# NoakLiu/FastFourierDiffusion

Measured on AMD Instinct MI355X. Metric: samples/sec at 1000 diffusion steps, ECG freq-domain, higher is better.
Workload: dtype f32; 1 GPU; ECG frequency-domain L=187 C=1, transformer d72/H12/NL10/F2048, VP beta[0.1,20], 1000-step sampler (BASELINE configs[1]); batch_per_gpu=512, global_batch=512, diffusion_steps=1000, cache=False, noise=philox on device

## Files before the change

### fastfourierdiffusion_amd/_native.py

```python
from __future__ import annotations

import ctypes as C
import os
from typing import Optional

_HERE = os.path.dirname(os.path.abspath(__file__))
LIB_PATH = os.path.join(_HERE, "libffd.so")

FFD_MODEL_TRANSFORMER, FFD_MODEL_LSTM, FFD_MODEL_MLP = 0, 1, 2
FFD_SDE_VP, FFD_SDE_VE = 0, 1
K_FFN, K_ATTN, K_OUTPROJ, K_LSTM_REC, K_LSTM_GATES, K_SDE, K_EMBED, K_UNEMBED = range(8)


class FFDError(RuntimeError):
    pass


class ModelDesc(C.Structure):
    _fields_ = [
        ("kind", C.c_int32), ("n_channels", C.c_int32), ("max_len", C.c_int32), ("d_model", C.c_int32),
        ("n_head", C.c_int32), ("num_layers", C.c_int32), ("dim_feedforward", C.c_int32), ("sde", C.c_int32),
        ("sde_a", C.c_double), ("sde_b", C.c_double), ("fourier_noise_scaling", C.c_int32), ("eps", C.c_double),
    ]


class SdeDesc(C.Structure):
    _fields_ = [("sde", C.c_int32), ("reserved", C.c_int32), ("a", C.c_double), ("b", C.c_double)]


class FrescaCfg(C.Structure):
    _fields_ = [("low_scale", C.c_float), ("high_scale", C.c_float), ("cutoff_ratio", C.c_double),
                ("strategy", C.c_int32), ("num_steps", C.c_int32)]


class CrfCaptureCfg(C.Structure):
    _fields_ = [("ring", C.c_void_p), ("n_slots", C.c_int32), ("every", C.c_int32), ("last", C.c_void_p),
                ("last_every", C.c_int32), ("reserved", C.c_int32)]


class CacheCfg(C.Structure):
    _fields_ = [("K", C.c_int32), ("R", C.c_int32)]


class CacheStats(C.Structure):
    _fields_ = [("recompute_count", C.c_int64), ("cache_hit_count", C.c_int64), ("current_step", C.c_int64),
                ("table_allocated", C.c_int32), ("reserved", C.c_int32)]


_P = C.c_void_p
_F = C.POINTER(C.c_float)

SIGNATURES = {
    "ffd_freq_decompose": (C.c_int, [_P, _P, _P, C.c_int, C.c_int, C.c_int, C.c_double, _P]),
    "ffd_hermite_predict": (C.c_int, [_P, C.POINTER(C.c_double), C.c_double, C.c_int, _P, C.c_int, C.c_size_t, _P]),
    "ffd_spectral_density": (C.c_int, [_P, _P, C.c_int, C.c_int, C.c_int, _P]),
    "ffd_w2_work_bytes": (C.c_size_t, [C.c_int, C.c_int, C.c_int, C.c_int, C.c_size_t]),
    "ffd_w2_sliced": (C.c_int, [_P, C.c_int, _P, C.c_int, C.c_int, _P, C.c_int, C.c_int, _P, _P, C.c_size_t, _P]),
    "ffd_w2_marginal": (C.c_int, [_P, C.c_int, _P, C.c_int, C.c_int, C.c_int, _P, _P, C.c_size_t, _P]),
    "ffd_w2_prepare": (C.c_int, [_P, C.c_int, C.c_int, _P, C.c_int, _P, _P, C.c_size_t, _P]),
    "ffd_w2_against_prepared": (C.c_int, [_P, C.c_int, _P, C.c_int, C.c_int, _P, C.c_int, C.c_int, _P, _P,
                                          C.c_size_t, _P]),
    "ffd_w2_summary": (C.c_int, [_P, C.c_int, _P, _P]),
    "ffd_col_mean_work_bytes": (C.c_size_t, [C.c_int, C.c_int]),
    "ffd_col_mean": (C.c_int, [_P, C.c_int, C.c_int, _P, _P, C.c_size_t, _P]),
    "ffd_w2_bench_kernels": (C.c_int, [_P, C.c_int, C.c_int, _P, C.c_int, _P, _P, _P, C.c_int, _P, C.c_int, _F, _P]),
    "ffd_sm_draw_times": (C.c_int, [_P, C.c_int, C.c_double, C.c_double, C.c_uint64, C.c_uint64, _P]),
    "ffd_sm_perturb": (C.c_int, [_P, _P, _P, _P, _P, _P, C.c_uint64, C.c_uint64, C.c_int, C.c_int, C.c_int, _P]),
    "ffd_sm_loss": (C.c_int, [_P, _P, _P, _P, C.c_uint64, C.c_uint64, C.c_int, C.c_int, _P, C.c_int, C.c_int, C.c_int, _P]),
    "ffd_sm_eval_batch": (C.c_int, [_P, _P, _P, _P, _P, _P, C.c_uint64, C.c_uint64, C.c_int, C.c_int, _P, C.c_int, _P]),
    "ffd_cache_crf_capture": (C.c_int, [_P, C.POINTER(CrfCaptureCfg)]),
    "ffd_create": (C.c_int, [C.POINTER(_P), C.POINTER(ModelDesc), C.c_int]),
    "ffd_destroy": (None, [_P]),
    "ffd_last_error": (C.c_char_p, [_P]),
    "ffd_version": (C.c_char_p, []),
    "ffd_load_weight": (C.c_int, [_P, C.c_char_p, _P, C.c_size_t]),
    "ffd_finalize_weights": (C.c_int, [_P]),
    "ffd_host_noise_scaling": (C.c_int, [C.c_int, C.c_int, _F]),
    "ffd_host_timesteps": (C.c_int, [C.c_int, C.c_double, _F, _F]),
    "ffd_host_gate": (C.c_int, [C.c_int, C.c_int, C.c_int, C.c_int]),
    "ffd_score_forward": (C.c_int, [_P, _P, C.c_float, _P, C.c_int, _P]),
    "ffd_score_forward_cached": (C.c_int, [_P, _P, C.c_float, _P, _P, C.c_int, C.c_int, _P]),
    "ffd_sde_step": (C.c_int, [C.POINTER(SdeDesc), _P, _P, _P, C.c_double, C.c_float, _P, C.c_uint64, C.c_uint64,
                               C.c_int, C.c_int, C.c_int, C.c_int, _P]),
    "ffd_prior": (C.c_int, [C.POINTER(SdeDesc), _P, _P, _P, C.c_uint64, C.c_uint64, C.c_int, C.c_int, C.c_int, _P]),
    "ffd_dft": (C.c_int, [_P, _P, C.c_int, C.c_int, C.c_int, _P]),
    "ffd_idft": (C.c_int, [_P, _P, C.c_int, C.c_int, C.c_int, _P]),
    "ffd_unstandardize_idft": (C.c_int, [_P, _P, _P, _P, C.c_int, C.c_int, C.c_int, _P]),
    "ffd_dft_standardize": (C.c_int, [_P, _P, _P, _P, C.c_int, C.c_int, C.c_int, _P]),
    "ffd_positional_encoding": (C.c_int, [_P, _P, _P, C.c_int, C.c_int, C.c_int, C.c_float, _P]),
    "ffd_time_encoding": (C.c_int, [_P, _P, _P, _P, _P, _P, _P, C.c_int, C.c_int, C.c_int, _P]),
    "ffd_fresca": (C.c_int, [_P, _P, _P, C.c_int, C.c_int, C.c_int, C.c_float, C.c_float, C.c_double, C.c_int, _P]),
    "ffd_lstm_trace": (C.c_int, [_P, C.POINTER(C.c_uint64), C.c_int, C.POINTER(C.c_int)]),
    "ffd_fresca2d": (C.c_int, [_P, _P, _P, C.c_int, C.c_int, C.c_int, C.c_int, C.c_float, C.c_float, C.c_double, C.c_int, _P]),
    "ffd_fresca_enable": (C.c_int, [_P, C.POINTER(FrescaCfg)]),
    "ffd_fresca_disable": (C.c_int, [_P]),
    "ffd_cache_enable": (C.c_int, [_P, C.POINTER(CacheCfg)]),
    "ffd_cache_disable": (C.c_int, [_P]),
    "ffd_cache_reset": (C.c_int, [_P]),
    "ffd_cache_stats_get": (C.c_int, [_P, C.POINTER(CacheStats)]),
    "ffd_cache_tables_read": (C.c_int, [_P, _P, _P, _P]),
    "ffd_sample_batch": (C.c_int, [_P, _P, C.c_int, _F, C.c_int, C.c_float, C.c_int, C.c_int, C.c_uint64,
                                   C.c_uint64, _P, C.c_int, C.c_int, _P]),
    "ffd_flops_per_sample_step": (C.c_double, [_P, C.c_int]),
    "ffd_ffn_flops_per_launch": (C.c_double, [_P, C.c_int]),
    "ffd_kernel_timing_begin": (C.c_int, [_P, C.c_uint32, C.c_int]),
    "ffd_kernel_timing_end": (C.c_int, [_P]),
    "ffd_kernel_timing_get": (C.c_int, [_P, C.c_int, _F, C.POINTER(C.c_int)]),
    "ffd_kernel_work": (C.c_char_p, [_P, C.c_int, C.c_int, C.c_int, C.POINTER(C.c_double), C.POINTER(C.c_double)]),
    "ffd_score_forward_ts": (C.c_int, [_P, _P, _P, _P, _P, C.c_int, C.c_int, _P]),
    "ffd_cache_configure": (C.c_int, [_P, C.POINTER(CacheCfg)]),
    "ffd_tune": (C.c_int, [C.c_char_p, C.c_int]),
    "ffd_tune_get": (C.c_int, [C.c_char_p, C.POINTER(C.c_int)]),
    "ffd_bench_ffn": (C.c_int, [_P, C.c_int, C.c_int, _F, _P]),
    "ffd_probe_ffn_clock": (C.c_int, [_P, C.c_int, C.c_double, C.POINTER(C.c_double), C.POINTER(C.c_double),
                                      C.POINTER(C.c_uint64), C.c_int, C.POINTER(C.c_int), _P]),
    "ffd_async_status": (C.c_int, [_P]),
    "ffd_probe_attn": (C.c_int, [_P, C.c_int, C.c_int, C.c_double, C.c_int, _F, C.POINTER(C.c_uint64), C.c_int,
                                 C.POINTER(C.c_int), _P]),
}

_lib: Optional[C.CDLL] = None


def lib() -> C.CDLL:
    global _lib
    if _lib is not None:
        return _lib
    if not os.path.exists(LIB_PATH):
        raise FFDError(
            f"{LIB_PATH} not found: build it with `python -c 'import __graft_entry__ as g; g.build()'` "
            "(or `make -C fastfourierdiffusion_amd/csrc`). There is no CPU / PyTorch fallback.")
    try:
        import torch
    except Exception:
        pass
    try:
        handle = C.CDLL(LIB_PATH, mode=C.RTLD_GLOBAL)
    except OSError as e:
        raise FFDError(f"failed to load {LIB_PATH}: {e}") from e
    for name, (res, args) in SIGNATURES.items():
        try:
            fn = getattr(handle, name)
        except AttributeError as e:
            raise FFDError(f"{LIB_PATH} does not export {name}") from e
        fn.restype = res
        fn.argtypes = args
    _lib = handle
    return handle


def check(rc: int, ctx=None, what: str = "") -> None:
    if rc == 0:
        return
    msg = ""
    if ctx:
        raw = lib().ffd_last_error(ctx)
        msg = raw.decode() if raw else ""
    exc = {-1: AssertionError, -2: NotImplementedError}.get(rc, FFDError)
    raise exc(f"libffd {what} failed (status {rc}): {msg}")


def current_stream_ptr(device) -> int:
    import torch

    return int(torch.cuda.current_stream(device).cuda_stream)


def require_gpu_tensor(t, name: str = "tensor"):
    import torch

    if not isinstance(t, torch.Tensor):
        raise TypeError(f"{name} must be a torch.Tensor")
    if t.device.type != "cuda":
        raise FFDError(
            f"{name} lives on {t.device}: fastfourierdiffusion_amd computes only on an MI355X (gfx950) device; "
            "move the model/tensors to cuda (there is no CPU fallback).")
    if t.dtype != torch.float32:
        raise AssertionError(f"{name} must be float32, got {t.dtype}")
    return t if t.is_contiguous() else t.contiguous()
```

### fastfourierdiffusion_amd/csrc/ffd_api.hip

```cpp
#include <math.h>
#include <stdarg.h>
#include <stdio.h>
#include <string.h>

#include <algorithm>
#include <string>
#include <vector>

#include "../../include/ffd.h"
#include "ffd_internal.h"

using namespace ffd;

namespace {

template <typename T>
struct Grow {
  T* p = nullptr;
  size_t cap = 0;
};

struct WeightSlot {
  std::string key;
  size_t n;
// ... 44 lines not shown
  std::vector<LstmLayer> lstm;
  std::vector<MlpLayer> mlp;
  float* G_dev = nullptr;
  std::vector<float> G_host;
  Grow<float> h0, h1, attn, score;
  Grow<float> qkv;
  Grow<float> temb_b;
  Grow<float> temb_tab, ts_dev;
  float* temb1 = nullptr;
  Grow<float> ffn_part;
  Grow<int> lstm_prog;
  Grow<float> lstm_state;
  std::vector<float> ts_host;
  long weight_epoch = 0, temb_epoch = -1;
  uint32_t time_mask = 0;
  std::vector<hipEvent_t> ev;
  std::vector<int> ev_cls;
  size_t ev_used = 0;
  float tm_ms[FFD_K_COUNT] = {0};
  int tm_n[FFD_K_COUNT] = {0};
  int* async_err = nullptr;
  unsigned long long* lstm_trace = nullptr;
  int lstm_trace_units = 0;
  bool fresca_on = false;
  bool crf_cap_on = false;
  ffd_crf_capture_cfg crf_cap{};
  ffd_fresca_cfg fcfg{};
  Grow<float> score2, fwork;
  Grow<float> sm_noisy;
  bool cache_enabled = false;
  ffd_cache_cfg ccfg{5, 10};
  float *kt = nullptr, *vt = nullptr;
  bool table_allocated = false;
  ffd_cache_stats stats{};

  int fail(int code, const char* fmt, ...) {
    char buf[512];
    va_list ap;
    va_start(ap, fmt);
    vsnprintf(buf, sizeof buf, fmt, ap);
    va_end(ap);
    err = buf;
    return code;
  }
  int d() const { return desc.d_model; }
  int hd() const { return desc.d_model / desc.n_head; }
  bool packs_made() const { return !layers.empty() && layers[0].in_wp != nullptr; }
  size_t table_floats() const { return (size_t)desc.num_layers * desc.n_head * desc.max_len * hd(); }
};

#define HIPCHECK(expr)                                                                          \
  do {                                                                                          \
    hipError_t e__ = (expr);                                                                    \
    if (e__ != hipSuccess)                                                                      \
      return ctx->fail(FFD_ERR_HIP, "%s failed: %s (%s:%d)", #expr, hipGetErrorString(e__), __FILE__, __LINE__); \
  } while (0)

namespace ffd {
#define FFD_KNOB_DEF(key, var, def, ...) thread_local int var = def;
FFD_KNOBS(FFD_KNOB_DEF, FFD_KNOB_DEF)
#undef FFD_KNOB_DEF
}

template <typename T>
static int dev_alloc(ffd_ctx* ctx, T** p, size_t n) {
  static_assert(sizeof(T) == sizeof(float), "the sizes in the messages are in floats");
  *p = nullptr;
  if (g_fail_alloc_after > 0 && --g_fail_alloc_after == 0)
    return ctx->fail(FFD_ERR_NOMEM, "hipMalloc(%zu floats) failed: injected by ffd_tune(\"fail_alloc_after\")", n);
  hipError_t e = hipMalloc((void**)p, n * sizeof(T) + 256);
  if (e != hipSuccess) return ctx->fail(FFD_ERR_NOMEM, "hipMalloc(%zu floats) failed: %s", n, hipGetErrorString(e));
  ctx->owned.push_back(*p);
  return FFD_OK;
}

template <typename T>
static int ensure(ffd_ctx* ctx, Grow<T>& b, size_t n) {
  if (n <= b.cap) return FFD_OK;
  T* old = b.p;
  b.cap = 0;
  b.p = nullptr;
  if (old) {
    (void)hipDeviceSynchronize();
    auto it = std::find(ctx->owned.begin(), ctx->owned.end(), (void*)old);
    if (it != ctx->owned.end()) ctx->owned.erase(it);
    (void)hipFree(old);
  }
  int rc = dev_alloc(ctx, &b.p, n);
  if (rc == FFD_OK) b.cap = n;
  return rc;
}

struct Timed {
  ffd_ctx* ctx;
  hipStream_t s;
  bool on;
  Timed(ffd_ctx* c, int cls, hipStream_t st) : ctx(c), s(st) {
    on = ((c->time_mask >> cls) & 1u) && c->ev_used + 2 <= c->ev.size();
    if (on) {
      (void)hipEventRecord(c->ev[c->ev_used], s);
      c->ev_cls.push_back(cls);
    }
  }
  ~Timed() {
    if (on) {
      (void)hipEventRecord(ctx->ev[ctx->ev_used + 1], s);
      ctx->ev_used += 2;
    }
  }
};
#define TIMED(cls, expr)      \
  do {                        \
    Timed tm__(ctx, cls, s);  \
    HIPCHECK(expr);           \
  } while (0)

static bool d_supported(int d) {
#define X(v) if (d == v) return true;
  FFD_D_LIST(X)
#undef X
  return false;
}
static bool hd_supported(int hd) {
#define X(v) if (hd == v) return true;
  FFD_HD_LIST(X)
#undef X
  return false;
}

namespace ffd {

CacheMode cache_mode(int n_rec, int L) {
  if (n_rec < 0) return CACHE_STD;
  if (n_rec == L) return CACHE_FULL;
  if ((double)n_rec > 0.8 * (double)L) return CACHE_STD;
  return n_rec == 0 ? CACHE_PURE : CACHE_MIXED;
}

LayerPlan plan_layer(const ffd_model_desc& m, int B, CacheMode mode, const PackSet& pk) {
  const int L = m.max_len, d = m.d_model, H = m.n_head, hd = d / H, F = m.dim_feedforward, M = B * L;
  LayerPlan p{};
  p.attn = g_attn_fused && pk.aw_full ? ATTN_FUSED : ATTN_TWO_KERNEL;
  p.hpw = 1;
  p.q_only = mode == CACHE_PURE;
  const int QT = cdiv(L, 32);
  if (p.attn == ATTN_FUSED) {
    p.kspl = qkv_attention_small_split(B, H, L);
    if (pk.aw_full2 && !p.kspl) p.hpw = qkv_attention_hpw(d, hd, L);
    if (g_attn_kvq && pk.aw_kvq && mode != CACHE_PURE && p.kspl) p.q_only = 2;
    p.qg = p.kspl                                               ? 1
           : p.hpw == 2                                         ? cdiv(QT, 2)
           : !p.q_only && (g_attn_qg == 1 || g_attn_qg == 2)    ? g_attn_qg
                                                                : attn_qg(QT, hd, true);
  } else {
    p.qg = QT == 1 ? 1 : g_attn_qg ? g_attn_qg : attn_qg(QT, hd, false);
  }
  const int hp = g_ffn_height && !g_ffn_split && !g_ffn_mb_override ? ffn_height_plan(M, d, F) : 0;
  int unf = 0;
  auto rows_nw = [&] { return g_ffn_rows_nw ? g_ffn_rows_nw : rows_waves(M); };
  if (g_ffn_split) {
    p.ffn = FFN_SPLIT;
  } else if (hp && g_ffn_height == 1) {
    p.ffn = FFN_LN_OPROJ, p.mb = hp;
  } else if (!(hp && g_small_wgs == 0) && (p.ns = small_path_splits(M, d, F))) {
    p.ffn = FFN_SMALL, p.part_floats = small_path_partial_floats(M, d, p.ns);
  } else if (pk.ring && !(hp && g_rows_slices == 0) && rows_slice_plan(M, d, F, &p.nw, &p.nslice, &unf)) {
    p.ffn = unf ? FFN_ROWS_SLICED : FFN_ROWS_SLICED_OPROJ, p.cps = 2, p.part_floats = rows_slice_floats(M, d, p.nslice);
  } else if ((p.nm = hp && g_mid_path == 1 ? 0 : mid_path_splits(M, d, F))) {
    p.ffn = FFN_MID, p.part_floats = small_path_partial_floats(cdiv(M, 64) * 64, d, p.nm);
  } else if (pk.ring && ffn_rows_fused_selected(M, d, F)) {
    p.ffn = FFN_ROWS_OPROJ, p.nw = rows_nw(), p.cps = 2;
  } else if (pk.ring && ffn_rows_selected(M, d, F)) {
    p.ffn = FFN_ROWS, p.nw = rows_nw(), p.cps = g_ffn_rows_cps == 1 && d == 72 ? 1 : 2;
  } else {
    p.ffn = FFN_LN;
    p.mb = g_ffn_mb_override >= 1 ? g_ffn_mb_override : cdiv(M, 64) >= 512 ? 4 : cdiv(M, 32) >= 512 ? 2 : 1;
    if (hp) p.mb = hp;
    p.persist = g_ffn_persist;
  }
  if (p.ffn == FFN_LN || p.ffn == FFN_LN_OPROJ) p.rem = g_ffn_rem && ffn_rem_rows(d, p.mb);
  p.oproj_separate = p.ffn >= FFN_ROWS_SLICED;
  p.swap = p.ffn == FFN_ROWS_SLICED_OPROJ || p.ffn == FFN_ROWS_OPROJ;
  return p;
}

LstmPlan plan_lstm(const ffd_model_desc& m, int B) {
  const int maxb = lstm_wave_max_batch(m.max_len, m.d_model);
  if (g_lstm_wave && m.d_model % 4 == 0 && m.d_model >= 16 && m.num_layers <= 64 && maxb >= 16)
    return {true, B < maxb ? B : maxb};
  return {false, B};
}

}

extern "C" {

int ffd_tune(const char* key, int value) {
  if (!key) return FFD_ERR_INVALID;
  if (!strcmp(key, "reset")) {
#define FFD_KNOB_RESET(k, var, def, ...) var = def;
    FFD_KNOBS(FFD_KNOB_RESET, FFD_KNOB_RESET)
#undef FFD_KNOB_RESET
    return FFD_OK;
  }
  const int v = value;
#define FFD_KNOB_SET(k, var, def, ok) \
  if (!strcmp(key, k)) {              \
    if (!(ok)) return FFD_ERR_INVALID; \
    var = v;                          \
    return FFD_OK;                    \
  }
#define FFD_KNOB_SET_BOOL(k, var, def) \
  if (!strcmp(key, k)) {               \
    var = v ? 1 : 0;                   \
    return FFD_OK;                     \
  }
  FFD_KNOBS(FFD_KNOB_SET, FFD_KNOB_SET_BOOL)
#undef FFD_KNOB_SET
#undef FFD_KNOB_SET_BOOL
  return FFD_ERR_INVALID;
}

int ffd_tune_get(const char* key, int* value) {
  if (!key || !value) return FFD_ERR_INVALID;
#define FFD_KNOB_GET(k, var, ...) \
  if (!strcmp(key, k)) {          \
    *value = var;                 \
    return FFD_OK;                \
  }
  FFD_KNOBS(FFD_KNOB_GET, FFD_KNOB_GET)
#undef FFD_KNOB_GET
  return FFD_ERR_INVALID;
}

const char* ffd_version(void) { return "libffd 0.1 (gfx950, fp32 MFMA 16x16x4, wave64)"; }

const char* ffd_last_error(const ffd_ctx* ctx) { return ctx ? ctx->err.c_str() : "null context"; }

int ffd_host_noise_scaling(int max_len, int fourier_noise_scaling, float* G) {
  if (max_len < 1 || !G) return FFD_ERR_INVALID;
  for (int i = 0; i < max_len; ++i) G[i] = 1.0f;
  if (fourier_noise_scaling) {
    const float c = (float)(1.0 / sqrt(2.0));
    const float s2 = (float)sqrt(2.0);
    for (int i = 0; i < max_len; ++i) G[i] = c * G[i];
    G[0] = G[0] * s2;
    if (max_len % 2 == 0) G[max_len / 2] = G[max_len / 2] * s2;
  }
  return FFD_OK;
}

int ffd_host_timesteps(int n, double eps, float* ts, float* step_size) {
  if (n < 2 || !ts) return FFD_ERR_INVALID;
  const float start = 1.0f, end = (float)eps;
  const float step = (end - start) / (float)(n - 1);
  const int half = n / 2;
  for (int i = 0; i < n; ++i) {
    volatile float prod = (i < half) ? step * (float)i : step * (float)(n - i - 1);
    ts[i] = (i < half) ? start + prod : end - prod;
  }
  if (step_size) *step_size = ts[0] - ts[1];
  return FFD_OK;
}

int ffd_host_gate(int step, int max_len, int K, int R) {
  if (step == 0) return max_len;
  const int interval = (R < 100) ? 500 : R;
  const int k_tokens = K < max_len ? K : max_len;
  if (step % interval == 0) {
    int n = 2 * k_tokens;
    if (n > max_len) n = max_len;
    return n < 0 ? 0 : n;
  }
  return 0;
}

static void bind_weights(ffd_ctx* ctx) {
  const ffd_model_desc& m = ctx->desc;
  const int NL = std::max(m.num_layers, 0);
  const size_t d = m.d_model, C = m.n_channels, L = m.max_len, F = m.dim_feedforward;
  auto bind = [&](const std::string& key, size_t n, const float** field) { ctx->weights.push_back({key, n, field}); };
  ModelWeights& w = ctx->model;
  if (m.kind == FFD_MODEL_TRANSFORMER) bind("pos_encoder.embedding.weight", L * d, &w.pos);
  bind("time_encoder.W", (d + 1) / 2, &w.time_W);
  bind("time_encoder.dense.weight", d * d, &w.time_dense_w);
  bind("time_encoder.dense.bias", d, &w.time_dense_b);
  const size_t io = m.kind == FFD_MODEL_MLP ? L * C : C;
  bind("embedder.weight", d * io, &w.embed_w);
  bind("embedder.bias", d, &w.embed_b);
  bind("unembedder.weight", io * d, &w.unembed_w);
  bind("unembedder.bias", io, &w.unembed_b);
  if (m.kind == FFD_MODEL_TRANSFORMER) ctx->layers.resize(NL);
  else if (m.kind == FFD_MODEL_MLP) ctx->mlp.resize(NL);
  else ctx->lstm.resize(NL);
  for (int i = 0; i < NL; ++i) {
    const std::string s = (m.kind == FFD_MODEL_TRANSFORMER ? "backbone.layers." : "backbone.") + std::to_string(i) + ".";
    if (m.kind == FFD_MODEL_TRANSFORMER) {
      LayerWeights& l = ctx->layers[i];
      bind(s + "self_attn.in_proj_weight", 3 * d * d, &l.in_w);
      bind(s + "self_attn.in_proj_bias", 3 * d, &l.in_b);
      bind(s + "self_attn.out_proj.weight", d * d, &l.out_w);
      bind(s + "self_attn.out_proj.bias", d, &l.out_b);
      bind(s + "linear1.weight", F * d, &l.w1);
      bind(s + "linear1.bias", F, &l.b1);
      bind(s + "linear2.weight", d * F, &l.w2);
      bind(s + "linear2.bias", d, &l.b2);
      bind(s + "norm1.weight", d, &l.n1w);
      bind(s + "norm1.bias", d, &l.n1b);
      bind(s + "norm2.weight", d, &l.n2w);
      bind(s + "norm2.bias", d, &l.n2b);
    } else if (m.kind == FFD_MODEL_MLP) {
      MlpLayer& l = ctx->mlp[i];
      bind(s + "0.weight", F * d, &l.w0);
      bind(s + "0.bias", F, &l.b0);
      bind(s + "3.weight", d * F, &l.w3);
      bind(s + "3.bias", d, &l.b3);
    } else {
      LstmLayer& l = ctx->lstm[i];
      bind(s + "weight_ih_l0", 4 * d * d, &l.wih);
      bind(s + "weight_hh_l0", 4 * d * d, &l.whh);
      bind(s + "bias_ih_l0", 4 * d, &l.bih);
      bind(s + "bias_hh_l0", 4 * d, &l.bhh);
    }
  }
}

int ffd_create(ffd_ctx** out, const ffd_model_desc* desc, int device) {
  if (!out || !desc) return FFD_ERR_INVALID;
  *out = nullptr;
  ffd_ctx* ctx = new ffd_ctx();
  ctx->desc = *desc;
  ctx->device = device;
  *out = ctx;
  const ffd_model_desc& m = ctx->desc;
  bind_weights(ctx);
  if (m.n_channels < 1 || m.max_len < 1 || m.num_layers < 1)
    return ctx->fail(FFD_ERR_INVALID, "bad shape: C=%d L=%d NL=%d", m.n_channels, m.max_len, m.num_layers);
  if (m.kind == FFD_MODEL_MLP) {
    if (m.d_model < 1 || m.dim_feedforward < 1)
      return ctx->fail(FFD_ERR_INVALID, "mlp: d_model=%d d_mlp=%d", m.d_model, m.dim_feedforward);
  } else if (!d_supported(m.d_model)) {
    return ctx->fail(FFD_ERR_UNSUPPORTED, "d_model=%d: this build has kernels for d_model in {8, 16, 24, 32, 48, 60, 64, 72}", m.d_model);
  }
  if (m.kind == FFD_MODEL_TRANSFORMER) {
    if (m.n_head < 1 || m.d_model % m.n_head != 0)
      return ctx->fail(FFD_ERR_INVALID, "d_model=%d not divisible by n_head=%d", m.d_model, m.n_head);
    if (!hd_supported(m.d_model / m.n_head))
      return ctx->fail(FFD_ERR_UNSUPPORTED, "head_dim=%d: supported head dims are 2, 3, 4, 5, 6, 8", m.d_model / m.n_head);
    if (m.dim_feedforward < 64 || m.dim_feedforward % 64 != 0)
      return ctx->fail(FFD_ERR_UNSUPPORTED, "dim_feedforward=%d must be a positive multiple of 64", m.dim_feedforward);
    if (m.max_len > 512) return ctx->fail(FFD_ERR_UNSUPPORTED, "max_len=%d > 512 (attention kernel limit)", m.max_len);
  } else if (m.kind != FFD_MODEL_LSTM && m.kind != FFD_MODEL_MLP) {
    return ctx->fail(FFD_ERR_UNSUPPORTED, "model kind %d", m.kind);
  }
  if (m.sde != FFD_SDE_VP && m.sde != FFD_SDE_VE) return ctx->fail(FFD_ERR_UNSUPPORTED, "sde kind %d", m.sde);
  int ndev = 0;
  hipError_t e = hipGetDeviceCount(&ndev);
  if (e != hipSuccess || ndev <= 0)
    return ctx->fail(FFD_ERR_HIP, "no HIP device available (%s): libffd has no CPU path",
                     e == hipSuccess ? "device count 0" : hipGetErrorString(e));
  if (device < 0 || device >= ndev) return ctx->fail(FFD_ERR_INVALID, "device %d out of range [0,%d)", device, ndev);
  HIPCHECK(hipSetDevice(device));
  hipDeviceProp_t prop;
  HIPCHECK(hipGetDeviceProperties(&prop, device));
  if (strncmp(prop.gcnArchName, "gfx950", 6) != 0)
    return ctx->fail(FFD_ERR_UNSUPPORTED, "device %d is %s; libffd is built for gfx950 only", device, prop.gcnArchName);
  ctx->G_host.resize(m.max_len);
  ffd_host_noise_scaling(m.max_len, m.fourier_noise_scaling, ctx->G_host.data());
  int rc = dev_alloc(ctx, &ctx->G_dev, m.max_len);
  if (rc) return rc;
  HIPCHECK(hipMemcpy(ctx->G_dev, ctx->G_host.data(), sizeof(float) * m.max_len, hipMemcpyHostToDevice));
  rc = dev_alloc(ctx, &ctx->temb1, m.d_model);
  if (rc) return rc;
  HIPCHECK(hipHostMalloc((void**)&ctx->async_err, 64, hipHostMallocMapped));
  memset(ctx->async_err, 0, 64);
  return FFD_OK;
}

void ffd_destroy(ffd_ctx* ctx) {
  if (!ctx) return;
  (void)hipSetDevice(ctx->device);
  for (WeightSlot& w : ctx->weights) (void)hipFree(w.dev);
  for (void* p : ctx->owned) (void)hipFree(p);
  for (hipEvent_t e : ctx->ev) (void)hipEventDestroy(e);
  if (ctx->async_err) (void)hipHostFree(ctx->async_err);
  delete ctx;
}

int ffd_load_weight(ffd_ctx* ctx, const char* name, const float* data, size_t n) {
  if (!ctx) return FFD_ERR_INVALID;
  if (!name || !data) return ctx->fail(FFD_ERR_INVALID, "ffd_load_weight: null argument");
  auto w = std::find_if(ctx->weights.begin(), ctx->weights.end(), [&](const WeightSlot& v) { return v.key == name; });
  if (w == ctx->weights.end()) return ctx->fail(FFD_ERR_INVALID, "unexpected parameter '%s' for this model", name);
  if (w->n != n) return ctx->fail(FFD_ERR_INVALID, "parameter '%s': got %zu floats, expected %zu", name, n, w->n);
  HIPCHECK(hipSetDevice(ctx->device));
  if (!w->dev) {
    hipError_t e = hipMalloc((void**)&w->dev, n * sizeof(float) + 256);
    if (e != hipSuccess) return ctx->fail(FFD_ERR_NOMEM, "hipMalloc for '%s' failed: %s", name, hipGetErrorString(e));
    *w->field = w->dev;
  }
  HIPCHECK(hipMemcpy(w->dev, data, n * sizeof(float), hipMemcpyDefault));
  ctx->finalized = false;
  return FFD_OK;
}

int ffd_finalize_weights(ffd_ctx* ctx) {
  if (!ctx) return FFD_ERR_INVALID;
  const ffd_model_desc& m = ctx->desc;
  for (const WeightSlot& w : ctx->weights)
    if (!w.dev) return ctx->fail(FFD_ERR_STATE, "missing parameter '%s'", w.key.c_str());
  HIPCHECK(hipSetDevice(ctx->device));
  const int d = m.d_model, F = m.dim_feedforward;
  hipStream_t s = nullptr;
  if (m.kind == FFD_MODEL_TRANSFORMER) {
    HIPCHECK(launch_renorm_rows(const_cast<float*>(ctx->model.pos), m.max_len, d, sqrtf((float)d), s));
    for (LayerWeights& l : ctx->layers) {
      if (!l.in_wp) {
        int rc;
        if ((rc = dev_alloc(ctx, &l.in_wp, dpack_floats(3 * d, d)))) return rc;
        if ((rc = dev_alloc(ctx, &l.q_wp, dpack_floats(d, d)))) return rc;
        if ((rc = dev_alloc(ctx, &l.kv_wp, dpack_floats(2 * d, d)))) return rc;
        if (qkv_attention_supported(d, d / m.n_head)) {
          if ((rc = dev_alloc(ctx, &l.aw_full, attn_pack_floats(d, m.n_head, 1, 0)))) return rc;
          if ((rc = dev_alloc(ctx, &l.aw_q, attn_pack_floats(d, m.n_head, 1, 1)))) return rc;
          if (attn_kvq_supported(d / m.n_head))
            if ((rc = dev_alloc(ctx, &l.aw_kvq, attn_pack_floats(d, m.n_head, 1, 2)))) return rc;
          if (m.n_head % 2 == 0) {
            if ((rc = dev_alloc(ctx, &l.aw_full2, attn_pack_floats(d, m.n_head, 2, 0)))) return rc;
            if ((rc = dev_alloc(ctx, &l.aw_q2, attn_pack_floats(d, m.n_head, 2, 1)))) return rc;
          }
        }
        if ((rc = dev_alloc(ctx, &l.out_wp, dpack_floats(d, d)))) return rc;
        if ((rc = dev_alloc(ctx, &l.w1p, dpack_floats(F, d)))) return rc;
        if ((rc = dev_alloc(ctx, &l.w2p, w2pack_floats(d, F)))) return rc;
        if ((rc = dev_alloc(ctx, &l.w2r, w2rem_floats(d, F)))) return rc;
        if (ffn_rows_supported(d, F)) {
          if ((rc = dev_alloc(ctx, &l.ring, ffn_ring_floats(d, F)))) return rc;
          if ((rc = dev_alloc(ctx, &l.ring_op, ffn_ring_oproj_floats(d)))) return rc;
        }
      }
      HIPCHECK(launch_pack_dweight(l.in_w, l.in_wp, 3 * d, d, s));
      HIPCHECK(launch_pack_dweight(l.in_w, l.q_wp, d, d, s));
      HIPCHECK(launch_pack_dweight(l.in_w + (size_t)d * d, l.kv_wp, 2 * d, d, s));
      if (l.aw_full) {
        HIPCHECK(launch_pack_attn(l.in_w, l.in_b, l.aw_full, d, m.n_head, 1, 0, s));
        HIPCHECK(launch_pack_attn(l.in_w, l.in_b, l.aw_q, d, m.n_head, 1, 1, s));
        if (l.aw_kvq) HIPCHECK(launch_pack_attn(l.in_w, l.in_b, l.aw_kvq, d, m.n_head, 1, 2, s));
        if (l.aw_full2) {
          HIPCHECK(launch_pack_attn(l.in_w, l.in_b, l.aw_full2, d, m.n_head, 2, 0, s));
          HIPCHECK(launch_pack_attn(l.in_w, l.in_b, l.aw_q2, d, m.n_head, 2, 1, s));
        }
      }
      HIPCHECK(launch_pack_dweight(l.out_w, l.out_wp, d, d, s));
      HIPCHECK(launch_pack_dweight(l.w1, l.w1p, F, d, s));
      HIPCHECK(launch_pack_w2(l.w2, l.w2p, d, F, s));
      HIPCHECK(launch_pack_w2rem(l.w2, l.w2r, d, F, s));
      if (l.ring) {
        HIPCHECK(launch_pack_ffn_ring(l.w1, l.b1, l.w2, l.ring, d, F, s));
        HIPCHECK(launch_pack_oproj_ring(l.out_w, l.ring_op, d, s));
      }
      if (l.w1s) HIPCHECK(launch_pack_ffn_split(l.w1, l.w2, l.w1s, l.w2s, d, F, s));
    }
  } else if (m.kind == FFD_MODEL_LSTM) {
    for (LstmLayer& l : ctx->lstm) {
      if (!l.wih_p) {
        int rc;
        if ((rc = dev_alloc(ctx, &l.wih_p, dpack_floats(4 * d, d)))) return rc;
        if ((rc = dev_alloc(ctx, &l.bsum, 4 * d))) return rc;
        if (d % 4 == 0 && d >= 16) {
          if ((rc = dev_alloc(ctx, &l.ih_wpk, lstm_wave_wpack_floats(d)))) return rc;
          if ((rc = dev_alloc(ctx, &l.hh_wpk, lstm_wave_wpack_floats(d)))) return rc;
          if ((rc = dev_alloc(ctx, &l.b_wpk, lstm_wave_bpack_floats(d)))) return rc;
        }
      }
      HIPCHECK(launch_pack_dweight(l.wih, l.wih_p, 4 * d, d, s));
      hipLaunchKernelGGL(k_add_vec, dim3(cdiv(4 * d, 256)), dim3(256), 0, s, l.bih, l.bhh, l.bsum, 4 * d);
      HIPCHECK(hipGetLastError());
      if (l.ih_wpk) HIPCHECK(launch_pack_lstm_wave(l.wih, l.whh, l.bsum, l.ih_wpk, l.hh_wpk, l.b_wpk, d, s));
    }
  }
  HIPCHECK(hipStreamSynchronize(s));
  ctx->weight_epoch++;
  ctx->finalized = true;
  return FFD_OK;
}

static int ensure_workspace(ffd_ctx* ctx, int B) {
  const ffd_model_desc& m = ctx->desc;
  const size_t M = (size_t)B * m.max_len, d = m.d_model;
  int rc;
  if ((rc = ensure(ctx, ctx->h0, M * d))) return rc;
  if ((rc = ensure(ctx, ctx->score, M * m.n_channels))) return rc;
  if ((rc = ensure(ctx, ctx->temb_b, (size_t)B * d))) return rc;
  if (m.kind == FFD_MODEL_MLP) {
    if ((rc = ensure(ctx, ctx->h1, (size_t)B * d))) return rc;
    if ((rc = ensure(ctx, ctx->qkv, (size_t)B * m.dim_feedforward))) return rc;
  } else if (m.kind == FFD_MODEL_TRANSFORMER) {
    if ((rc = ensure(ctx, ctx->h1, M * d))) return rc;
    if ((rc = ensure(ctx, ctx->attn, M * d))) return rc;
  }
  return FFD_OK;
}

static LayerPlan plan_of(const ffd_ctx* ctx, int B, CacheMode mode) {
  const LayerWeights& w = ctx->layers[0];
  return plan_layer(ctx->desc, B, mode,
                    PackSet{w.aw_full != nullptr, w.aw_full2 != nullptr, w.aw_kvq != nullptr, w.ring_op != nullptr});
}

struct CacheUse {
  int n_own;
  bool tables, store;
};
static CacheUse cache_use(CacheMode mode, int n_rec, int L) {
  return {mode == CACHE_PURE ? 0 : mode == CACHE_MIXED ? n_rec : L, mode == CACHE_PURE || mode == CACHE_MIXED,
          mode == CACHE_MIXED};
}

static hipError_t run_attention(const ffd_ctx* ctx, const LayerPlan& p, const LayerWeights& w, const float* x,
                                const float* kt, const float* vt, float* kt_out, float* vt_out, int B, int n_own,
                                hipStream_t s, unsigned long long* stamp = nullptr) {
  const ffd_model_desc& m = ctx->desc;
  const int L = m.max_len, d = m.d_model, H = m.n_head, hd = d / H;
  float* out = ctx->attn.p;
  if (p.attn == ATTN_FUSED) {
    const float* pack = p.q_only == 2 ? w.aw_kvq
                        : p.hpw == 2  ? (p.q_only ? w.aw_q2 : w.aw_full2)
                                      : (p.q_only ? w.aw_q : w.aw_full);
    return launch_qkv_attention(AttnArgs{x, pack, kt, vt, kt_out, vt_out, out, B, L, n_own, stamp}, d, hd, p.hpw, p.q_only,
                                p.kspl, p.qg, s);
  }
  if (stamp != nullptr) return hipErrorInvalidValue;
  const size_t M = (size_t)B * L;
  float *q = ctx->qkv.p, *k = q + M * d, *v = q + 2 * M * d;
  hipError_t e = launch_linear_hm(x, p.q_only ? w.q_wp : w.in_wp, w.in_b, q, k, v, (int)M, p.q_only ? 1 : 3, d, L, H, hd, s);
  if (e == hipSuccess) e = launch_attention(q, k, v, kt, vt, out, B, L, H, hd, n_own, p.qg, s);
  if (e == hipSuccess && kt_out)
    e = launch_kv_store(k, v, kt_out, vt_out, L, H, hd, n_own, s);
  return e;
}

static hipError_t run_ffn(const ffd_ctx* ctx, const LayerPlan& p, const LayerWeights& w, const float* attn, float* cur,
                          float* alt, int M, hipStream_t s, unsigned long long* stamp = nullptr) {
  const int d = ctx->desc.d_model, F = ctx->desc.dim_feedforward;
  float* P = ctx->ffn_part.p;
  const bool sliced = p.ffn == FFN_ROWS_SLICED_OPROJ || p.ffn == FFN_ROWS_SLICED;
  const bool fused = p.ffn == FFN_ROWS_SLICED_OPROJ || p.ffn == FFN_ROWS_OPROJ;
  float* const y = fused ? alt : cur;
  const RowsArgs rows{fused ? attn : alt, fused ? cur : nullptr, &w, sliced ? P : y, M, d, F, p.nw, p.cps, fused,
                      sliced ? p.nslice : 0, stamp};
  switch (p.ffn) {
    case FFN_LN_OPROJ:
      return stamp ? hipErrorInvalidValue : launch_oproj_ffn_ln(attn, cur, w, cur, M, d, F, p.mb, p.rem, s);
    case FFN_SMALL:
      return stamp ? hipErrorInvalidValue : launch_oproj_ffn_small(attn, cur, w, alt, P, cur, M, d, F, p.ns, s);
    case FFN_ROWS_SLICED_OPROJ:
    case FFN_ROWS_SLICED: {
      if (stamp || p.nslice < 2) return hipErrorInvalidValue;
      const hipError_t e = launch_ffn_rows(rows, s);
      return e != hipSuccess ? e : launch_rows_reduce_ln(P, w, y, M, d, p.nslice, s);
    }
    case FFN_ROWS_OPROJ:
    case FFN_ROWS: return launch_ffn_rows(rows, s);
    case FFN_MID:
      return stamp ? hipErrorInvalidValue : launch_ffn_mid(alt, w, P, cur, M, d, F, p.nm, s);
    case FFN_SPLIT: return launch_ffn_ln_split(alt, w, cur, M, d, F, s, stamp);
    case FFN_LN: return launch_ffn_ln(alt, w, cur, M, d, F, p.mb, p.rem, p.persist, s, stamp);
  }
  return hipErrorInvalidValue;
}

static const struct {
  const char* name;
  bool oproj;
} kFfnForms[] = {
    {"k_ffn_ln<oproj>", true},
    {"k_oproj_ffn_split + k_ffn_reduce_ln", true},
    {"k_ffn_rows<oproj, sliced> + k_rows_reduce_ln", true},
    {"k_ffn_rows<oproj>", true},
    {"k_ffn_rows<sliced> + k_rows_reduce_ln", false},
    {"k_ffn_part", false},
    {"k_ffn_ln_split", false},
    {"k_ffn_rows", false},
    {"k_ffn_ln", false},
};

static int forward_impl(ffd_ctx* ctx, const float* x, const float* temb, int temb_stride, float* score_out,
                        float* crf_out, int B, int n_rec, hipStream_t s, const float** hidden_out = nullptr) {
  const ffd_model_desc& m = ctx->desc;
  const int L = m.max_len, C = m.n_channels, d = m.d_model, M = B * L;
  const ModelWeights& mw = ctx->model;
  if (m.kind == FFD_MODEL_MLP) {
    const int io = L * C, F = m.dim_feedforward;
    HIPCHECK(launch_dense(x, mw.embed_w, mw.embed_b, temb_stride ? nullptr : temb, temb_stride ? temb : nullptr,
                          ctx->h0.p, B, d, io, 0, s));
    float* cur = ctx->h0.p;
    float* alt = ctx->h1.p;
    for (const MlpLayer& l : ctx->mlp) {
      HIPCHECK(launch_dense(cur, l.w0, l.b0, nullptr, nullptr, ctx->qkv.p, B, F, d, 1, s));
      HIPCHECK(launch_dense(ctx->qkv.p, l.w3, l.b3, nullptr, cur, alt, B, d, F, 0, s));
      std::swap(cur, alt);
    }
    HIPCHECK(launch_dense(cur, mw.unembed_w, mw.unembed_b, nullptr, nullptr, score_out, B, io, d, 0, s));
    return FFD_OK;
  }
  float* const h0 = ctx->h0.p;
  if (m.kind == FFD_MODEL_LSTM) {
    TIMED(FFD_K_EMBED, launch_embed(x, mw.embed_w, mw.embed_b, nullptr, temb, temb_stride, h0, B, L, C, d, s));
    if (const LstmPlan lp = plan_lstm(m, B); lp.wave) {
      const int Bw = lp.Bw;
      if (int rc = ensure(ctx, ctx->lstm_prog, (size_t)16 + 16 * cdiv(Bw, 16))) return rc;
      const float *wih[64], *whh[64], *bs[64];
      for (int i = 0; i < m.num_layers; ++i) wih[i] = ctx->lstm[i].ih_wpk, whh[i] = ctx->lstm[i].hh_wpk, bs[i] = ctx->lstm[i].b_wpk;
      if (int rc = ensure(ctx, ctx->lstm_state, lstm_wave_state_floats(Bw, d, m.num_layers))) return rc;
      for (int b0 = 0; b0 < B; b0 += Bw) {
        const int nb = B - b0 < Bw ? B - b0 : Bw;
        TIMED(FFD_K_LSTM_REC, launch_lstm_wave(h0 + (size_t)b0 * L * d, wih, whh, bs, m.num_layers, nb, L, d,
                                               ctx->lstm_prog.p, ctx->lstm_state.p, ctx->async_err, s,
                                               b0 == 0 ? ctx->lstm_trace : nullptr));
      }
    } else
    for (const LstmLayer& l : ctx->lstm) {
      if (int rc = ensure(ctx, ctx->qkv, (size_t)M * 4 * d)) return rc;
      TIMED(FFD_K_LSTM_GATES, launch_linear(h0, l.wih_p, l.bsum, ctx->qkv.p, M, 4 * d, d, 4 * d, s));
      TIMED(FFD_K_LSTM_REC, launch_lstm_layer(h0, ctx->qkv.p, l.whh, B, L, d, s));
    }
    if (hidden_out) {
      *hidden_out = h0;
      return FFD_OK;
    }
    TIMED(FFD_K_UNEMBED, launch_unembed(h0, mw.unembed_w, mw.unembed_b, score_out, M, C, d, s));
    return FFD_OK;
  }
  const int H = m.n_head, hd = d / H, F = m.dim_feedforward;
  TIMED(FFD_K_EMBED, launch_embed(x, mw.embed_w, mw.embed_b, mw.pos, temb, temb_stride, h0, B, L, C, d, s));
  const CacheMode mode = cache_mode(n_rec, L);
  const CacheUse cu = cache_use(mode, n_rec, L);
  const size_t lt = (size_t)H * L * hd;
  if (g_ffn_split && !ffn_split_supported(d, F))
    return ctx->fail(FFD_ERR_UNSUPPORTED, "ffn_split needs d_model %% 4 == 0, d_model <= 96, dim_feedforward %% 128 == 0");
  const LayerPlan plan = plan_of(ctx, B, mode);
  if (plan.attn == ATTN_TWO_KERNEL)
    if (int rc = ensure(ctx, ctx->qkv, (size_t)M * 3 * d)) return rc;
  if (int rc = ensure(ctx, ctx->ffn_part, plan.part_floats)) return rc;
  float* const attn = ctx->attn.p;
  float* cur = h0;
  float* alt = ctx->h1.p;
  for (int i = 0; i < m.num_layers; ++i) {
    LayerWeights& w = ctx->layers[i];
    float* kt = ctx->kt ? ctx->kt + i * lt : nullptr;
    float* vt = ctx->vt ? ctx->vt + i * lt : nullptr;
    TIMED(FFD_K_ATTN, run_attention(ctx, plan, w, cur, cu.tables ? kt : nullptr, cu.tables ? vt : nullptr,
                                    cu.store ? kt : nullptr, cu.store ? vt : nullptr, B, cu.n_own, s));
    if (plan.ffn == FFN_SPLIT && w.w1s == nullptr) {
      if (int rc = dev_alloc(ctx, &w.w1s, w1split_bytes(d, F) / sizeof(float))) return rc;
      if (int rc = dev_alloc(ctx, &w.w2s, w2split_bytes(d, F) / sizeof(float))) return rc;
      HIPCHECK(launch_pack_ffn_split(w.w1, w.w2, w.w1s, w.w2s, d, F, s));
    }
    if (plan.oproj_separate)
      TIMED(FFD_K_OUTPROJ, launch_linear_res_ln(attn, w.out_wp, w.out_b, cur, w.n1w, w.n1b, alt, M, d, s));
    TIMED(FFD_K_FFN, run_ffn(ctx, plan, w, attn, cur, alt, M, s));
    if (plan.swap) std::swap(cur, alt);
    if (mode == CACHE_FULL) {
      HIPCHECK(launch_linear_hm(cur, w.kv_wp, w.in_b + d, kt, vt, nullptr, L, 2, d, L, H, hd, s));
    }
    if (n_rec >= 0 && crf_out)
      HIPCHECK(hipMemcpyAsync(crf_out + (size_t)i * L * d, cur, sizeof(float) * L * d, hipMemcpyDeviceToDevice, s));
  }
  if (n_rec >= 0) {
    if (mode == CACHE_FULL) ctx->stats.recompute_count += (int64_t)L * m.num_layers, ctx->table_allocated = true;
    else if (mode == CACHE_PURE) ctx->stats.cache_hit_count += (int64_t)L * m.num_layers;
    else if (mode == CACHE_MIXED) {
      ctx->stats.cache_hit_count += (int64_t)(L - n_rec) * m.num_layers;
      ctx->stats.recompute_count += (int64_t)n_rec * m.num_layers;
      ctx->table_allocated = true;
    }
  }
  if (hidden_out) {
    *hidden_out = cur;
    return FFD_OK;
  }
  TIMED(FFD_K_UNEMBED, launch_unembed(cur, mw.unembed_w, mw.unembed_b, score_out, M, C, d, s));
  return FFD_OK;
// ... 236 lines not shown
    }
    float* crf_dst = nullptr;
    float* crf_copy = nullptr;
    if (use_cache && ctx->crf_cap_on) {
      const ffd_crf_capture_cfg& cc = ctx->crf_cap;
      const int gstep = global_step0 + j;
      const size_t crf_n = (size_t)m.num_layers * m.max_len * d;
      if (cc.ring && gstep % cc.every == 0) crf_dst = cc.ring + (size_t)((gstep / cc.every) % cc.n_slots) * crf_n;
      if (cc.last && gstep % cc.last_every == 0) {
        const int rest = n_run - 1 - j;
        const int to_next = cc.last_every - (gstep % cc.last_every);
        if (to_next > rest) {
          if (crf_dst) crf_copy = cc.last; else crf_dst = cc.last;
        }
      }
    }
    const float* hidden = nullptr;
    if ((rc = forward_impl(ctx, x, ctx->temb_tab.p + (size_t)i * d, 0, ctx->score.p, crf_dst, B, n_rec, s,
                           fuse_tail ? &hidden : nullptr)))
      return rc;
    if (crf_copy)
      HIPCHECK(hipMemcpyAsync(crf_copy, crf_dst, sizeof(float) * (size_t)m.num_layers * m.max_len * d,
                              hipMemcpyDeviceToDevice, s));
    if (use_cache) ctx->stats.current_step = i;
    const double t = (double)timesteps[i];
    const float* score = ctx->score.p;
    if (ctx->fresca_on) {
      const ffd_fresca_cfg& f = ctx->fcfg;
      double h = (double)f.high_scale;
      if (f.num_steps > 0 && h > 1.0) h = (1.0 - t / (double)f.num_steps) * (h - 1.0) + 1.0;
      if (!((double)f.low_scale == 1.0 && h == 1.0)) {
        HIPCHECK(launch_fresca(ctx->score.p, ctx->score2.p, ctx->fwork.p, B, m.max_len, m.n_channels, f.low_scale, (float)h,
                               f.cutoff_ratio, f.strategy, s));
        score = ctx->score2.p;
      }
    }
    if (hidden)
      TIMED(FFD_K_SDE, launch_unembed_sde(hidden, ctx->model.unembed_w, ctx->model.unembed_b, x,
                                          z_inject ? z_inject + (size_t)j * slab : nullptr, ctx->G_dev,
                                          sde_params(m.sde, m.sde_a, m.sde_b, t, step_size), seed, elem_off, (uint32_t)i,
                                          B, m.max_len, m.n_channels, d, s));
    else
      TIMED(FFD_K_SDE, launch_sde_step(x, score, z_inject ? z_inject + (size_t)j * slab : nullptr, ctx->G_dev,
                                       sde_params(m.sde, m.sde_a, m.sde_b, t, step_size), seed, elem_off, (uint32_t)i, B,
                                       m.max_len, m.n_channels, s));
  }
  return FFD_OK;
}

double ffd_flops_per_sample_step(const ffd_ctx* ctx, int cache_hit) {
  if (!ctx) return 0.0;
  const ffd_model_desc& m = ctx->desc;
  const double L = m.max_len, d = m.d_model, C = m.n_channels, NL = m.num_layers, F = m.dim_feedforward;
  if (m.kind == FFD_MODEL_LSTM) return NL * 2.0 * L * (2.0 * 4.0 * d * d) + 4.0 * L * C * d + 2.0 * d * d;
  if (m.kind == FFD_MODEL_MLP) return NL * 4.0 * d * F + 4.0 * L * C * d + 2.0 * d * d;
  double per_layer = 2.0 * L * d * 3.0 * d + 2.0 * L * L * d + 2.0 * L * L * d + 2.0 * L * d * d + 4.0 * L * d * F;
  if (cache_hit) per_layer -= 2.0 * L * d * 2.0 * d;
  return NL * per_layer + 4.0 * L * C * d + 2.0 * d * d;
}

double ffd_ffn_flops_per_launch(const ffd_ctx* ctx, int B) {
  if (!ctx) return 0.0;
  const ffd_model_desc& m = ctx->desc;
  return 4.0 * (double)B * m.max_len * m.d_model * m.dim_feedforward;
}

int ffd_lstm_trace(ffd_ctx* ctx, unsigned long long* host_out, int capacity_units, int* n_units_out) {
  if (!ctx || capacity_units < 1) return FFD_ERR_INVALID;
  HIPCHECK(hipSetDevice(ctx->device));
  if (host_out == nullptr) {
    if (ctx->lstm_trace) (void)hipFree(ctx->lstm_trace);
    ctx->lstm_trace = nullptr;
    HIPCHECK(hipMalloc(&ctx->lstm_trace, sizeof(unsigned long long) * 4 * (size_t)capacity_units));
    HIPCHECK(hipMemset(ctx->lstm_trace, 0, sizeof(unsigned long long) * 4 * (size_t)capacity_units));
    ctx->lstm_trace_units = capacity_units;
    return FFD_OK;
  }
  if (!ctx->lstm_trace) return ctx->fail(FFD_ERR_STATE, "ffd_lstm_trace: no trace begun");
  HIPCHECK(hipDeviceSynchronize());
  const int n = capacity_units < ctx->lstm_trace_units ? capacity_units : ctx->lstm_trace_units;
  HIPCHECK(hipMemcpy(host_out, ctx->lstm_trace, sizeof(unsigned long long) * 4 * (size_t)n, hipMemcpyDeviceToHost));
  (void)hipFree(ctx->lstm_trace);
  ctx->lstm_trace = nullptr;
  if (n_units_out) *n_units_out = n;
  return FFD_OK;
}

int ffd_kernel_timing_begin(ffd_ctx* ctx, uint32_t class_mask, int max_launches) {
  if (!ctx) return FFD_ERR_INVALID;
  if (max_launches < 1 || max_launches > 100000) return ctx->fail(FFD_ERR_INVALID, "max_launches=%d", max_launches);
  HIPCHECK(hipSetDevice(ctx->device));
  while (ctx->ev.size() < (size_t)2 * max_launches) {
    hipEvent_t e;
    HIPCHECK(hipEventCreate(&e));
    ctx->ev.push_back(e);
  }
  ctx->ev_used = 0;
  ctx->ev_cls.clear();
  ctx->time_mask = class_mask;
  return FFD_OK;
}

int ffd_kernel_timing_end(ffd_ctx* ctx) {
  if (!ctx) return FFD_ERR_INVALID;
  ctx->time_mask = 0;
  HIPCHECK(hipSetDevice(ctx->device));
  double tot[FFD_K_COUNT] = {0};
  for (int c = 0; c < FFD_K_COUNT; ++c) ctx->tm_n[c] = 0;
  const size_t n = ctx->ev_used / 2;
  for (size_t i = 0; i < n; ++i) {
    HIPCHECK(hipEventSynchronize(ctx->ev[2 * i + 1]));
    float ms = 0.f;
    HIPCHECK(hipEventElapsedTime(&ms, ctx->ev[2 * i], ctx->ev[2 * i + 1]));
    const int c = ctx->ev_cls[i];
    tot[c] += ms;
    ctx->tm_n[c]++;
  }
  for (int c = 0; c < FFD_K_COUNT; ++c) ctx->tm_ms[c] = ctx->tm_n[c] ? (float)(tot[c] / ctx->tm_n[c]) : 0.f;
  ctx->ev_used = 0;
  ctx->ev_cls.clear();
  return FFD_OK;
}

int ffd_kernel_timing_get(const ffd_ctx* ctx, int kernel_class, float* avg_ms_out, int* launches_out) {
  if (!ctx || kernel_class < 0 || kernel_class >= FFD_K_COUNT || !avg_ms_out || !launches_out) return FFD_ERR_INVALID;
  *avg_ms_out = ctx->tm_ms[kernel_class];
  *launches_out = ctx->tm_n[kernel_class];
  return FFD_OK;
}

const char* ffd_kernel_work(const ffd_ctx* ctx, int kernel_class, int B, int cache_hit, double* flops_out,
                            double* bytes_out) {
  if (!ctx || B < 1) return nullptr;
  const ffd_model_desc& m = ctx->desc;
  const double L = m.max_len, d = m.d_model, C = m.n_channels, F = m.dim_feedforward, M = (double)B * L;
  const bool tr = m.kind == FFD_MODEL_TRANSFORMER && ctx->packs_made(), ls = m.kind == FFD_MODEL_LSTM;
  const LayerPlan p = tr ? plan_of(ctx, B, cache_hit ? CACHE_PURE : CACHE_STD) : LayerPlan{};
  const LstmPlan lp = ls ? plan_lstm(m, B) : LstmPlan{};
  double fl = 0.0, by = 0.0;
  const char* name = nullptr;
  switch (kernel_class) {
    case FFD_K_FFN:
      if (tr) {
        const bool op = kFfnForms[p.ffn].oproj;
        name = kFfnForms[p.ffn].name;
        fl = 4.0 * M * d * F + (op ? (p.ffn == FFN_ROWS_SLICED_OPROJ ? p.nslice : 1) * 2.0 * M * d * d : 0.0);
        by = p.ffn == FFN_SPLIT ? 4.0 * (2.0 * M * d) + 6.0 * (2.0 * d * F)
             : op               ? 4.0 * (3.0 * M * d + 2.0 * d * F + d * d)
                                : 4.0 * (2.0 * M * d + 2.0 * d * F);
      }
      break;
    case FFD_K_ATTN:
      if (tr) {
        name = p.attn == ATTN_FUSED ? "k_qkv_attention" : "k_linear_hm + k_attention_mfma";
        fl = M * (2.0 * d * (cache_hit ? d : 3.0 * d) + 4.0 * L * d);
        by = 4.0 * (2.0 * M * d + 3.0 * d * d + (cache_hit ? 2.0 * L * d : 0.0));
        if (p.attn == ATTN_TWO_KERNEL) by += 4.0 * 2.0 * M * (cache_hit ? d : 3.0 * d);
      }
      break;
    case FFD_K_OUTPROJ:
      if (tr && p.oproj_separate) name = "k_linear_res_ln", fl = 2.0 * M * d * d, by = 4.0 * (3.0 * M * d + d * d);
      break;
    case FFD_K_LSTM_REC:
      if (ls && lp.wave) {
        const double Ml = (double)lp.Bw * L;
        name = "k_lstm_wave", fl = m.num_layers * 2.0 * Ml * 8.0 * d * d, by = m.num_layers * 4.0 * (2.0 * Ml * d + 8.0 * d * d);
      }
      else if (ls)
        name = "k_lstm_layer", fl = 2.0 * M * 4.0 * d * d, by = 4.0 * (M * 4.0 * d + 2.0 * M * d + 4.0 * d * d);
      break;
    case FFD_K_LSTM_GATES:
      if (ls && !lp.wave)
        name = "k_linear_rm", fl = 2.0 * M * 4.0 * d * d, by = 4.0 * (M * d + M * 4.0 * d + 4.0 * d * d);
      break;
    case FFD_K_SDE:
      if (tail_fusable(ctx))
        name = "k_unembed_mfma<sde>", fl = 2.0 * M * C * d, by = 4.0 * M * (d + 2.0 * C);
      else
        name = "k_sde_step", by = 12.0 * M * C;
      break;
    case FFD_K_EMBED:
      if (m.kind != FFD_MODEL_MLP) name = "k_embed", fl = 2.0 * M * C * d, by = 4.0 * M * (C + d);
      break;
    case FFD_K_UNEMBED:
      if (m.kind != FFD_MODEL_MLP) name = "k_unembed", fl = 2.0 * M * C * d, by = 4.0 * M * (C + d);
      break;
    default: break;
  }
  if (flops_out) *flops_out = fl;
  if (bytes_out) *bytes_out = by;
  return name;
}


}

template <typename Run>
static int time_launches(ffd_ctx* ctx, hipStream_t s, Run run, int batch, double warm_seconds, int iters, float* ms_out) {
  struct Events {
    hipEvent_t e0 = nullptr, e1 = nullptr;
    ~Events() {
      if (e0) (void)hipEventDestroy(e0);
      if (e1) (void)hipEventDestroy(e1);
    }
  } ev;
  HIPCHECK(hipEventCreate(&ev.e0));
  HIPCHECK(hipEventCreate(&ev.e1));
  HIPCHECK(hipEventRecord(ev.e0, s));
  float ms = 0.f;
  do {
    for (int i = 0; i < batch; ++i) HIPCHECK(run());
    HIPCHECK(hipEventRecord(ev.e1, s));
    HIPCHECK(hipEventSynchronize(ev.e1));
    HIPCHECK(hipEventElapsedTime(&ms, ev.e0, ev.e1));
  } while (ms * 1e-3 < warm_seconds);
  if (iters < 1) return FFD_OK;
  HIPCHECK(hipEventRecord(ev.e0, s));
  for (int i = 0; i < iters; ++i) HIPCHECK(run());
  HIPCHECK(hipEventRecord(ev.e1, s));
  HIPCHECK(hipEventSynchronize(ev.e1));
  HIPCHECK(hipEventElapsedTime(&ms, ev.e0, ev.e1));
  *ms_out = ms / iters;
  return FFD_OK;
}

extern "C" {

struct StampBuf {
  unsigned long long* p = nullptr;
  ~StampBuf() { (void)hipFree(p); }
};

static int ffn_probe_setup(ffd_ctx* ctx, int B, hipStream_t s, LayerPlan* plan) {
  if (int rc = check_ready(ctx, B)) return rc;
  if (ctx->desc.kind != FFD_MODEL_TRANSFORMER) return ctx->fail(FFD_ERR_UNSUPPORTED, "no FFN in this backbone");
  HIPCHECK(hipSetDevice(ctx->device));
  if (int rc = ensure_workspace(ctx, B)) return rc;
  *plan = plan_of(ctx, B, CACHE_STD);
  if (plan->ffn == FFN_SPLIT && ctx->layers[0].w1s == nullptr)
    return ctx->fail(FFD_ERR_STATE, "ffn_split: run one forward first (the packs are made on first use)");
  if (int rc = ensure(ctx, ctx->ffn_part, plan->part_floats)) return rc;
  const size_t n = (size_t)B * ctx->desc.max_len * ctx->desc.d_model;
  hipLaunchKernelGGL(k_fill_hash, dim3(1024), dim3(256), 0, s, ctx->h1.p, n, 0x9E3779B9u);
  hipLaunchKernelGGL(k_fill_hash, dim3(1024), dim3(256), 0, s, ctx->attn.p, n, 0x85EBCA6Bu);
  hipLaunchKernelGGL(k_fill_hash, dim3(1024), dim3(256), 0, s, ctx->h0.p, n, 0xC2B2AE35u);
  HIPCHECK(hipGetLastError());
  return FFD_OK;
}

int ffd_bench_ffn(ffd_ctx* ctx, int B, int iters, float* ms_out, void* stream) {
  if (!ctx) return FFD_ERR_INVALID;
  if (iters < 1 || !ms_out) return ctx->fail(FFD_ERR_INVALID, "bad argument to ffd_bench_ffn");
  hipStream_t s = (hipStream_t)stream;
  LayerPlan p;
  if (int rc = ffn_probe_setup(ctx, B, s, &p)) return rc;
  const int M = B * ctx->desc.max_len;
  auto run = [&]() { return run_ffn(ctx, p, ctx->layers[0], ctx->attn.p, ctx->h1.p, ctx->h0.p, M, s); };
  return time_launches(ctx, s, run, 3, 0.0, iters, ms_out);
}

int ffd_probe_ffn_clock(ffd_ctx* ctx, int B, double warm_seconds, double* ghz_out, double* loop_us_out,
                        unsigned long long* raw_out, int raw_capacity, int* nwg_out, void* stream) {
  if (!ctx) return FFD_ERR_INVALID;
  if (!ghz_out || !(warm_seconds >= 0.0) || warm_seconds > 30.0) return ctx->fail(FFD_ERR_INVALID, "bad argument");
  hipStream_t s = (hipStream_t)stream;
  LayerPlan p;
  if (int rc = ffn_probe_setup(ctx, B, s, &p)) return rc;
  const int M = B * ctx->desc.max_len;
  const int nwg = cdiv(M, 16);
  StampBuf stamps;
  HIPCHECK(hipMalloc((void**)&stamps.p, sizeof(unsigned long long) * 8 * nwg));
  HIPCHECK(hipMemsetAsync(stamps.p, 0, sizeof(unsigned long long) * 8 * nwg, s));
  auto launch = [&](unsigned long long* st) { return run_ffn(ctx, p, ctx->layers[0], ctx->attn.p, ctx->h1.p, ctx->h0.p, M, s, st); };
  float unused;
  if (int rc = time_launches(ctx, s, [&]() { return launch(nullptr); }, 50, warm_seconds, 0, &unused)) return rc;
  if (launch(stamps.p) != hipSuccess)
    return ctx->fail(FFD_ERR_UNSUPPORTED, "no stamped twin of the planned FFN form (%s)", kFfnForms[p.ffn].name);
  std::vector<unsigned long long> h(8 * (size_t)nwg);
  HIPCHECK(hipMemcpyAsync(h.data(), stamps.p, sizeof(unsigned long long) * 8 * nwg, hipMemcpyDeviceToHost, s));
  HIPCHECK(hipStreamSynchronize(s));
  std::vector<double> ghz, us;
  int used = 0;
  for (int i = 0; i < nwg; ++i)
    if (h[8 * i + 1] > 0) {
      ghz.push_back((double)h[8 * i] / (double)h[8 * i + 1] * 0.1);
      us.push_back((double)h[8 * i + 1] * 0.01);
      if (raw_out && used < raw_capacity) memcpy(raw_out + 8 * (size_t)used, &h[8 * i], sizeof(unsigned long long) * 8);
      ++used;
    }
  if (nwg_out) *nwg_out = used;
  if (ghz.empty()) return ctx->fail(FFD_ERR_STATE, "no stamps were written");
  std::sort(ghz.begin(), ghz.end());
  std::sort(us.begin(), us.end());
  *ghz_out = ghz[ghz.size() / 2];
  if (loop_us_out) *loop_us_out = us[us.size() / 2];
  return FFD_OK;
}

int ffd_async_status(ffd_ctx* ctx) {
  if (!ctx) return FFD_ERR_INVALID;
  return check_async(ctx);
}

int ffd_probe_attn(ffd_ctx* ctx, int B, int n_recompute, double warm_seconds, int iters, float* ms_out,
                   unsigned long long* raw_out, int raw_capacity, int* nrec_out, void* stream) {
  if (!ctx) return FFD_ERR_INVALID;
  int rc = check_ready(ctx, B);
  if (rc) return rc;
  const ffd_model_desc& m = ctx->desc;
  if (m.kind != FFD_MODEL_TRANSFORMER) return ctx->fail(FFD_ERR_UNSUPPORTED, "no attention in this backbone");
  if (!ms_out || iters < 1 || !(warm_seconds >= 0.0) || warm_seconds > 30.0) return ctx->fail(FFD_ERR_INVALID, "bad argument");
  const int L = m.max_len, d = m.d_model, H = m.n_head;
  if (n_recompute > L) return ctx->fail(FFD_ERR_INVALID, "n_recompute=%d outside [-1,%d]", n_recompute, L);
  const CacheMode mode = cache_mode(n_recompute, L);
  const CacheUse cu = cache_use(mode, n_recompute, L);
  if (cu.tables && !(ctx->cache_enabled && ctx->table_allocated))
    return ctx->fail(FFD_ERR_STATE, "cached modes need ffd_cache_enable and one full step (the tables)");
  HIPCHECK(hipSetDevice(ctx->device));
  if ((rc = ensure_workspace(ctx, B))) return rc;
  const LayerPlan p = plan_of(ctx, B, mode);
  if (p.attn == ATTN_TWO_KERNEL)
    if ((rc = ensure(ctx, ctx->qkv, (size_t)B * L * 3 * d))) return rc;
  hipStream_t s = (hipStream_t)stream;
  hipLaunchKernelGGL(k_fill_hash, dim3(1024), dim3(256), 0, s, ctx->h1.p, (size_t)B * L * d, 0x9E3779B9u);
  HIPCHECK(hipGetLastError());
  auto launch = [&](unsigned long long* st) {
    return run_attention(ctx, p, ctx->layers[0], ctx->h1.p, cu.tables ? ctx->kt : nullptr, cu.tables ? ctx->vt : nullptr,
                         nullptr, nullptr, B, cu.n_own, s, st);
  };
  if ((rc = time_launches(ctx, s, [&]() { return launch(nullptr); }, 20, warm_seconds, iters, ms_out))) return rc;
  if (nrec_out) *nrec_out = 0;
  if (raw_out && raw_capacity > 0) {
    const size_t nwave = (size_t)B * H * 4;
    StampBuf stamps;
    HIPCHECK(hipMalloc((void**)&stamps.p, sizeof(unsigned long long) * 16 * nwave));
    HIPCHECK(hipMemsetAsync(stamps.p, 0, sizeof(unsigned long long) * 16 * nwave, s));
    if (launch(stamps.p) != hipSuccess)
      return ctx->fail(FFD_ERR_UNSUPPORTED, "no stamped twin of the planned attention form (%s, %d head(s) per workgroup, "
                       "pack mode %d, %d key pieces) for this shape", p.attn == ATTN_FUSED ? "k_qkv_attention" : "two-kernel",
                       p.hpw, p.q_only, p.kspl);
    std::vector<unsigned long long> h(16 * nwave);
    HIPCHECK(hipMemcpyAsync(h.data(), stamps.p, sizeof(unsigned long long) * 16 * nwave, hipMemcpyDeviceToHost, s));
    HIPCHECK(hipStreamSynchronize(s));
    int used = 0;
    for (size_t i = 0; i < nwave && used < raw_capacity; ++i)
      if (h[16 * i + 1] != 0) memcpy(raw_out + 16 * (size_t)used++, &h[16 * i], sizeof(unsigned long long) * 16);
    if (nrec_out) *nrec_out = used;
  }
  return FFD_OK;
}

}
```

### fastfourierdiffusion_amd/csrc/ffd_ffn_rows.hip

```cpp
#include "ffd_internal.h"

namespace ffd {

typedef float f32x16 __attribute__((ext_vector_type(16)));
__device__ __forceinline__ f32x16 mfma32(float a, float b, f32x16 c) {
  return __builtin_amdgcn_mfma_f32_32x32x2f32(a, b, c, 0, 0, 0);
}

constexpr __host__ __device__ int ring_ct(int D) { return D / 32; }
constexpr __host__ __device__ int ring_ng(int D) { return (D % 32) / 4; }
constexpr __host__ __device__ int ring_ks2(int D) { return 16 * ring_ct(D) + 4 * ((ring_ng(D) + 1) / 2); }
constexpr __host__ __device__ int ring_nq1(int D) { return cdiv(ring_ks2(D), 4); }
constexpr __host__ __device__ int ring_kperm(int D, int s, int half) {
  return s < 16 * ring_ct(D) ? 32 * (s / 16) + 8 * ((s % 16) / 4) + 4 * half + s % 4
                             : 32 * ring_ct(D) + 4 * (2 * ((s - 16 * ring_ct(D)) / 4) + half) + (s - 16 * ring_ct(D)) % 4;
}
constexpr __host__ __device__ int ring_nmain(int D) { return ring_nq1(D) + 4 * ring_ct(D); }
constexpr __host__ __device__ int ring_nrem(int D) { return 4 * ring_ng(D); }
constexpr __host__ __device__ int ring_nfc(int D) { return ring_nmain(D) + ring_nrem(D); }
constexpr __host__ __device__ bool ring_compact(int D) { return D != 72; }
constexpr __host__ __device__ int ring_nfull(int D) { return ring_compact(D) ? ring_nmain(D) : ring_nfc(D); }
constexpr __host__ __device__ int ring_chunk_groups(int D) { return ring_nfull(D) + cdiv(ring_nfc(D) - ring_nfull(D), 8) + 1; }
constexpr __host__ __device__ int ring_frag_off(int nmain, int k, int lane) {
  return k < nmain ? k * 256 + lane * 4
// ... 170 lines not shown
    }
  ss += __shfl_xor(ss, 32);
  const float rstd = 1.0f / sqrtf(ss * (1.0f / D) + 1e-5f);
#pragma unroll
  for (int ct = 0; ct < CT; ++ct)
#pragma unroll
    for (int t = 0; t < 4; ++t) {
      const int c0 = 32 * ct + 8 * t + 4 * half;
      const float4 g4 = *reinterpret_cast<const float4*>(&p[D + c0]);
      const float4 e4 = *reinterpret_cast<const float4*>(&p[2 * D + c0]);
      v[ct][t] = float4{(v[ct][t].x - mean) * rstd * g4.x + e4.x, (v[ct][t].y - mean) * rstd * g4.y + e4.y,
                        (v[ct][t].z - mean) * rstd * g4.z + e4.z, (v[ct][t].w - mean) * rstd * g4.w + e4.w};
    }
#pragma unroll
  for (int i = 0; i < (NG + 1) / 2; ++i)
    if (2 * i + half < NG) {
      const int c0 = 32 * CT + 4 * (2 * i + half);
      const float4 g4 = *reinterpret_cast<const float4*>(&p[D + c0]);
      const float4 e4 = *reinterpret_cast<const float4*>(&p[2 * D + c0]);
      vr[i] = float4{(vr[i].x - mean) * rstd * g4.x + e4.x, (vr[i].y - mean) * rstd * g4.y + e4.y,
                     (vr[i].z - mean) * rstd * g4.z + e4.z, (vr[i].w - mean) * rstd * g4.w + e4.w};
    }
}

template <int D>
__device__ __forceinline__ void raw_rows(const f32x16* acc, const f32x4* rem, const float4 (*res)[4], const float4* resrem,
                                         const float* p, int half, bool first, float4 (*v)[4], float4* vr) {
  constexpr int CT = ring_ct(D), NG = ring_ng(D);
#pragma unroll
  for (int ct = 0; ct < CT; ++ct)
#pragma unroll
    for (int t = 0; t < 4; ++t) {
      v[ct][t] = float4{acc[ct][4 * t], acc[ct][4 * t + 1], acc[ct][4 * t + 2], acc[ct][4 * t + 3]};
      if (first) {
        const float4 bq = *reinterpret_cast<const float4*>(&p[32 * ct + 8 * t + 4 * half]);
        const float4 x4 = res[ct][t];
        v[ct][t] = float4{x4.x + (v[ct][t].x + bq.x), x4.y + (v[ct][t].y + bq.y), x4.z + (v[ct][t].z + bq.z),
                          x4.w + (v[ct][t].w + bq.w)};
      }
    }
#pragma unroll
  for (int i = 0; i < (NG + 1) / 2; ++i) {
    float a[4];
#pragma unroll
    for (int e = 0; e < 4; ++e) {
      float t0 = rem[2 * i][e];
      t0 += __shfl_xor(t0, 32);
      float t1 = 0.f;
      if (2 * i + 1 < NG) {
        t1 = rem[(2 * i + 1 < NG) ? 2 * i + 1 : 0][e];
        t1 += __shfl_xor(t1, 32);
      }
      a[e] = half ? t1 : t0;
    }
    vr[i] = float4{a[0], a[1], a[2], a[3]};
    if (first && 2 * i + half < NG) {
      const float4 bq = *reinterpret_cast<const float4*>(&p[32 * CT + 4 * (2 * i + half)]);
      const float4 x4 = resrem[i];
      vr[i] = float4{x4.x + (a[0] + bq.x), x4.y + (a[1] + bq.y), x4.z + (a[2] + bq.z), x4.w + (a[3] + bq.w)};
    }
  }
}

template <int D, int NW, int CPS, int NSLOT, int PR, bool OP, bool SL, bool ONE>
__global__ __launch_bounds__(64 * NW, 3) void k_ffn_rows(const float* __restrict__ X, const float* __restrict__ Rin,
                                                             const float* __restrict__ ring, const float* __restrict__ ringp,
                                                             const float* __restrict__ b2, const float* __restrict__ gam,
                                                             const float* __restrict__ bet, const float* __restrict__ bo,
                                                             const float* __restrict__ gam1, const float* __restrict__ bet1,
                                                             float* __restrict__ Y, int M, int F, int nslice,
                                                             unsigned long long* stamp) {
  using C = FfnRowsCfg<D, NW, CPS, NSLOT>;
  constexpr int KS2 = C::KS2, CT = C::CT, NG = C::NG, NQ1 = C::NQ1, SGC = C::SGC, NFC = C::NFC, PD = C::PD;
  constexpr int NGA = NG > 0 ? NG : 1, CTA = CT > 0 ? CT : 1;
  constexpr int NRH = (NG + 1) / 2;
  constexpr int NRA = NRH > 0 ? NRH : 1;
  constexpr int R = 32 * NW;
  constexpr int NFS = CPS * NFC;
  constexpr int RPG = cdiv(4, CTA);
  constexpr int NPM = C::NPM, NFP = C::NFP;
  static_assert(CT == 0 || 4 % CT == 0, "relu placement assumes CT in {1, 2, 4}");
  static_assert(!OP || (CPS == 2 && C::AHEAD == 2 && NFP + PD <= NFS + PD && C::NFPP <= C::SLOT_G && CT > 0),
                "the fused form: two-chunk slots, ring one slot ahead of the barrier");
  __shared__ __align__(16) float lds[C::LDS_FLOATS];

  const int lane = threadIdx.x & 63;
  const int wave = __builtin_amdgcn_readfirstlane(threadIdx.x >> 6);
  const int half = lane >> 5, m = lane & 31;
  float* const ringl = lds;
  float* const lnp = lds + NSLOT * C::SLOT_FLOATS;
  const unsigned ring_base = __builtin_amdgcn_readfirstlane(lds_addr(ringl));

  const int ntiles = (M + R - 1) / R;
  const int slice = SL ? (int)blockIdx.x % nslice : 0;
  const int slot_first = SL ? slice * (F / (32 * CPS)) / nslice : 0;
  const int nchunk_slots = SL ? (slice + 1) * (F / (32 * CPS)) / nslice - slot_first : F / (32 * CPS);
  const int NSL = nchunk_slots + (OP ? 1 : 0);
  const int tstride = SL ? (int)gridDim.x / nslice : (int)gridDim.x;
  const int my_tiles = SL ? ((int)blockIdx.x / nslice < ntiles ? (ntiles - 1 - (int)blockIdx.x / nslice) / tstride + 1 : 0)
                       : ONE ? ((int)blockIdx.x < ntiles ? 1 : 0)
                             : ((int)blockIdx.x < ntiles) ? (ntiles - 1 - (int)blockIdx.x) / (int)gridDim.x + 1 : 0;
  const int total = my_tiles * NSL;
  if (total == 0) return;

  const float* const ring_s = ring + (size_t)slot_first * C::SLOT_FLOATS;
  auto slot_src = [&](int wslot) -> const float* {
    return OP ? (wslot == 0 ? ringp : ring_s + (size_t)(wslot - 1) * C::SLOT_FLOATS) : ring_s + (size_t)wslot * C::SLOT_FLOATS;
  };

  float4 xv[CTA][4], xrem[NRA];
  f32x16 yacc[CTA];
  f32x4 yrem[NGA];
  int tile = SL ? (int)blockIdx.x / nslice : (int)blockIdx.x;
  int wnext = C::AHEAD % NSL;
  auto load_rows = [&](const float* src, float4 (*q)[4], float4* qrem) {
    const int row = min(tile * R + wave * 32 + m, M - 1);
    const float* xr = src + (size_t)row * D;
#pragma unroll
    for (int ct = 0; ct < CT; ++ct)
#pragma unroll
      for (int t = 0; t < 4; ++t) q[ct][t] = *reinterpret_cast<const float4*>(xr + 32 * ct + 8 * t + 4 * half);
#pragma unroll
    for (int i = 0; i < NRH; ++i) {
      qrem[i] = float4{0.f, 0.f, 0.f, 0.f};
      if (2 * i + half < NG) qrem[i] = *reinterpret_cast<const float4*>(xr + 32 * CT + 4 * (2 * i + half));
    }
  };
  auto retire_rows = [&](float4 (*q)[4], float4* qrem) {
#pragma unroll
    for (int ct = 0; ct < CT; ++ct)
#pragma unroll
      for (int t = 0; t < 4; ++t) asm volatile("" : "+v"(q[ct][t].x), "+v"(q[ct][t].y), "+v"(q[ct][t].z), "+v"(q[ct][t].w));
#pragma unroll
    for (int i = 0; i < NRH; ++i) asm volatile("" : "+v"(qrem[i].x), "+v"(qrem[i].y), "+v"(qrem[i].z), "+v"(qrem[i].w));
  };
  auto xb_of = [&](int s) -> float {
    return s < 16 * CT ? f4e(xv[s / 16 < CTA ? s / 16 : 0][(s % 16) / 4], s % 4)
                       : f4e(xrem[(s - 16 * CT) / 4 < NRH ? (s - 16 * CT) / 4 : 0], (s - 16 * CT) % 4);
  };
  auto zero_acc = [&]() {
#pragma unroll
    for (int ct = 0; ct < CTA; ++ct)
#pragma unroll
      for (int r = 0; r < 16; ++r) yacc[ct][r] = 0.f;
#pragma unroll
    for (int g = 0; g < NGA; ++g) yrem[g] = f32x4{0.f, 0.f, 0.f, 0.f};
  };

  static_assert(C::AHEAD == 2 || !OP, "prologue of the fused form");
  for (int i = threadIdx.x; i < (OP ? 6 : 3) * D; i += 64 * NW)
    lnp[i] = i < D ? b2[i] : i < 2 * D ? gam[i - D] : i < 3 * D ? bet[i - 2 * D]
           : i < 4 * D ? bo[i - 3 * D] : i < 5 * D ? gam1[i - 4 * D] : bet1[i - 5 * D];
  {
    const float* src = slot_src(0) + lane * 4;
    for (int g = wave; g < (OP ? C::NFPP : C::SLOT_G); g += NW) dma_piece(src + g * 256, ring_base + g * 1024);
  }
  float4 rin[CTA][4], rinrem[NRA];
  load_rows(X, xv, xrem);
  if (OP) load_rows(Rin, rin, rinrem);
  wait_vm<0>();
  retire_rows(xv, xrem);
  if (OP) retire_rows(rin, rinrem);
#pragma unroll
  for (int j = 1; j < C::AHEAD; ++j)
    if (j < total) {
      const float* src = slot_src(j % NSL) + lane * 4;
      const unsigned dst = ring_base + (unsigned)(j % NSLOT) * (C::SLOT_FLOATS * 4);
#pragma unroll
      for (int i = 0; i < C::NPW; ++i) {
        const int g0 = wave + i * NW, g = g0 < C::SLOT_G ? g0 : g0 - C::SLOT_G;
        dma_piece(src + g * 256, dst + g * 1024);
      }
    }
  asm volatile("s_waitcnt lgkmcnt(0)" ::: "memory");
  __builtin_amdgcn_s_barrier();

  float4 hb[4], f[NFS + PD];
  {
    const float* slot = ringl;
    if (!OP) {
#pragma unroll
      for (int t = 0; t < 4; ++t) hb[t] = *reinterpret_cast<const float4*>(slot + (SGC - 1) * 256 + 4 * (2 * t + half));
    }
#pragma unroll
    for (int k = 0; k < PD; ++k) f[k] = *reinterpret_cast<const float4*>(slot + k * 256 + lane * 4);
  }
  unsigned long long st_clk = 0, st_rt = 0, st_acc = 0, st_acc_rt = 0, st_first_b = 0, st_first_e = 0, st_epi = 0;
  const unsigned long long st_entry = stamp ? __builtin_amdgcn_s_memrealtime() : 0ull;
  int st_tiles = 0;


#define FFD_SLOT_PRELUDE                                                                                               \
  int lane_i;                                                                                                          \
  asm volatile("v_mbcnt_lo_u32_b32 %0, -1, 0\n\tv_mbcnt_hi_u32_b32 %0, -1, %0" : "=v"(lane_i));                       \
  const int half_i = lane_i >> 5;                                                                                      \
  const float* slot = ringl + (it % NSLOT) * C::SLOT_FLOATS;                                                           \
  const float* nslot = ringl + ((it + 1) % NSLOT) * C::SLOT_FLOATS;                                                    \
  const bool dma_on = it + C::AHEAD < total;                                                                           \
  const float* dma_src = slot_src(wnext) + lane_i * 4;                                                                 \
  const unsigned dma_dst = ring_base + (unsigned)((it + C::AHEAD) % NSLOT) * (C::SLOT_FLOATS * 4);                     \
  int dma_g = wave;                                                       \
  auto issue_piece = [&]() {          \
    if (dma_on) {                                                                                                      \
      const int g = dma_g < C::SLOT_G ? dma_g : dma_g - C::SLOT_G;                                                     \
      dma_piece(dma_src + g * 256, dma_dst + g * 1024);                                                                \
      dma_g += NW;                                                                                                     \
    }                                                                                                                  \
  }

  int it = 0;
  for (int tl = 0; tl < my_tiles; ++tl) {
    if (stamp) {
      st_clk = __builtin_amdgcn_s_memtime(), st_rt = __builtin_amdgcn_s_memrealtime();
      if (st_tiles == 0) st_first_b = st_rt;
    }
    if (OP) {
      FFD_SLOT_PRELUDE;
      if (it > 0) {
        wait_vm<0>();
        __builtin_amdgcn_s_barrier();
      }
#pragma unroll
      for (int i = 0; i < C::NPW; ++i) issue_piece();
      zero_acc();
#pragma unroll
      for (int K = 0; K < NFP; ++K) {
        const float4 w = f[K];
        if (PR) {
          if (K == 0) __builtin_amdgcn_s_setprio(3);
          else if (K == NFP / 4) __builtin_amdgcn_s_setprio(2);
          else if (K == NFP / 2) __builtin_amdgcn_s_setprio(1);
          else if (K == 3 * NFP / 4) __builtin_amdgcn_s_setprio(0);
        }
#pragma unroll
        for (int j = 0; j < 4; ++j) {
          if (K < NPM) {
            const int idx = 4 * K + j, s = idx / CTA, ct = idx % CTA;
            if (s < KS2) yacc[ct] = mfma32(f4e(w, j), xb_of(s), yacc[ct]);
          } else {
            const int idx = 4 * (K - NPM) + j, s = idx / NGA, g = idx % NGA;
            if (s < KS2) yrem[g] = __builtin_amdgcn_mfma_f32_4x4x1f32(f4e(w, j), xb_of(s), yrem[g], 0, 0, 0);
          }
          if (j == 1) {
            const int KP = K + PD;
            if (KP < NFP) f[KP] = *reinterpret_cast<const float4*>(slot + ring_frag_off(C::NPF, KP, lane_i));
            else f[KP] = *reinterpret_cast<const float4*>(nslot + ring_frag_off(C::NMAIN, KP - NFP, lane_i));
            if (K == NFP - 1) {
#pragma unroll
              for (int t = 0; t < 4; ++t) hb[t] = *reinterpret_cast<const float4*>(nslot + (SGC - 1) * 256 + 4 * (2 * t + half_i));
            }
          }
          __builtin_amdgcn_sched_barrier(0);
        }
        if (K == NPM - 1) {
          if (dma_on) wait_vm<C::NPW>(); else wait_vm<0>();
          __builtin_amdgcn_s_barrier();
          __builtin_amdgcn_sched_barrier(0);
        }
      }
#pragma unroll
      for (int k = 0; k < PD; ++k) f[k] = f[NFP + k];
      {
        float4 v[CTA][4], vr[NRA];
        ln_rows<D>(yacc, yrem, rin, rinrem, lnp + 3 * D, half, v, vr);
#pragma unroll
        for (int ct = 0; ct < CT; ++ct)
#pragma unroll
          for (int t = 0; t < 4; ++t) xv[ct][t] = v[ct][t];
#pragma unroll
        for (int i = 0; i < NRH; ++i) xrem[i] = (2 * i + half < NG) ? vr[i] : float4{0.f, 0.f, 0.f, 0.f};
      }
      if (dma_on && ++wnext == NSL) wnext = 0;
      ++it;
    }
    zero_acc();

    for (int sl = OP ? 1 : 0; sl < NSL; ++sl, ++it) {
      FFD_SLOT_PRELUDE;
      f32x16 h;
#pragma unroll
      for (int K = 0; K < NFS; ++K) {
        const int c = K / NFC, k = K % NFC;
        const float4 w = f[K];
        if (PR) {
          constexpr int KB = (CPS - 1) * NFC + NQ1;
          const int rel = (K - KB + NFS) % NFS;
          if (rel == 0 || (rel * 4) / NFS != ((rel - 1) * 4) / NFS) {
            const int lvl = 3 - (rel * 4) / NFS;
            if (lvl == 3) __builtin_amdgcn_s_setprio(3);
            else if (lvl == 2) __builtin_amdgcn_s_setprio(2);
            else if (lvl == 1) __builtin_amdgcn_s_setprio(1);
            else __builtin_amdgcn_s_setprio(0);
          }
        }
        if (k == 0) {
#pragma unroll
          for (int t = 0; t < 4; ++t) h[4 * t] = hb[t].x, h[4 * t + 1] = hb[t].y, h[4 * t + 2] = hb[t].z, h[4 * t + 3] = hb[t].w;
        }
#pragma unroll
        for (int j = 0; j < 4; ++j) {
          if (k < NQ1) {
            const int s = 4 * k + j;
            if (s < KS2) h = mfma32(f4e(w, j), xb_of(s), h);
          } else if (k < NQ1 + 4 * CT) {
            const int idx = 4 * (k - NQ1) + j, r = idx / CTA, ct = idx % CTA;
            yacc[ct] = mfma32(f4e(w, j), h[r], yacc[ct]);
            if (j == 0) {
#pragma unroll
              for (int rr = 0; rr < RPG; ++rr) {
                const int rn = (k - NQ1 + 1) * RPG + rr;
                if (rn < 16) h[rn] = relu_bits(h[rn]);
              }
            }
          } else {
            const int idx = 4 * (k - NQ1 - 4 * CT) + j, r = idx / NGA, g = idx % NGA;
            yrem[g] = __builtin_amdgcn_mfma_f32_4x4x1f32(f4e(w, j), h[r], yrem[g], 0, 0, 0);
          }
          if (j == 1) {
            const int KP = K + PD;
            const float* base = KP < NFS ? slot : nslot;
            const int kk = KP < NFS ? KP : KP - NFS;
            f[KP] = *reinterpret_cast<const float4*>(base + (kk / NFC) * SGC * 256 + ring_frag_off(C::NMAIN, kk % NFC, lane_i));
            if (k == NFC - 1) {
              const float* bsrc = (c + 1 < CPS) ? slot + ((c + 1) * SGC + SGC - 1) * 256 : nslot + (SGC - 1) * 256;
#pragma unroll
              for (int t = 0; t < 4; ++t) hb[t] = *reinterpret_cast<const float4*>(bsrc + 4 * (2 * t + half_i));
            }
          }
          {
            constexpr int KB0 = (CPS - 1) * NFC + NQ1, W = NFC - NQ1;
            if (j == 2 && K >= KB0 && K - KB0 < C::NPW) issue_piece();
            if (j == 3 && K >= KB0 && K - KB0 + W < C::NPW) issue_piece();
          }
          __builtin_amdgcn_sched_barrier(0);
        }
        if (k == NQ1 - 1) {
#pragma unroll
          for (int r = 0; r < RPG; ++r) h[r] = relu_bits(h[r]);
          if (c == CPS - 1) {
            if (C::AHEAD > 2 && it + C::AHEAD - 1 < total) {
              if (sl == 0 && it > 0) wait_vm<(C::AHEAD - 2) * C::NPW + C::NST>(); else wait_vm<(C::AHEAD - 2) * C::NPW>();
            } else {
              wait_vm<0>();
            }
            __builtin_amdgcn_s_barrier();
          }
          __builtin_amdgcn_sched_barrier(0);
        }
      }
#pragma unroll
      for (int k = 0; k < PD; ++k) f[k] = f[NFS + k];
      if (dma_on && ++wnext == NSL) wnext = 0;
    }

    if (stamp) {
      const unsigned long long rt = __builtin_amdgcn_s_memrealtime();
      st_acc += __builtin_amdgcn_s_memtime() - st_clk;
      st_acc_rt += rt - st_rt;
// ... 246 lines not shown
```

### fastfourierdiffusion_amd/csrc/ffd_internal.h

```cpp
#pragma once
#include <hip/hip_runtime.h>
#include <stdint.h>

#include "../../include/ffd.h"

namespace ffd {

constexpr int WAVE = 64;

#define FFD_D_LIST(X) X(8) X(16) X(24) X(32) X(48) X(60) X(64) X(72)
#define FFD_HD_LIST(X) X(2) X(3) X(4) X(5) X(6) X(8)

typedef float f32x4 __attribute__((ext_vector_type(4)));

__device__ __forceinline__ f32x4 mfma16(float a, float b, f32x4 c) {
  return __builtin_amdgcn_mfma_f32_16x16x4f32(a, b, c, 0, 0, 0);
}

constexpr __host__ __device__ int cdiv(int a, int b) { return (a + b - 1) / b; }

__device__ __forceinline__ float relu_bits(float x) {
  const int i = __builtin_bit_cast(int, x);
  return __builtin_bit_cast(float, i > 0 ? i : 0);
}

struct U4 {
  uint32_t x, y, z, w;
};

__device__ __forceinline__ U4 philox4x32_10(U4 c, uint32_t k0, uint32_t k1) {
  const uint32_t M0 = 0xD2511F53u, M1 = 0xCD9E8D57u, W0 = 0x9E3779B9u, W1 = 0xBB67AE85u;
#pragma unroll
  for (int i = 0; i < 10; ++i) {
    const uint64_t p0 = (uint64_t)M0 * c.x, p1 = (uint64_t)M1 * c.z;
    const uint32_t hi0 = (uint32_t)(p0 >> 32), lo0 = (uint32_t)p0, hi1 = (uint32_t)(p1 >> 32), lo1 = (uint32_t)p1;
    U4 n = {hi1 ^ c.y ^ k0, lo1, hi0 ^ c.w ^ k1, lo0};
    c = n;
    k0 += W0;
    k1 += W1;
  }
  return c;
}

__device__ __forceinline__ void box_muller(uint32_t a, uint32_t b, float& z0, float& z1) {
  const float u1 = ((float)(a >> 8) + 0.5f) * (1.0f / 16777216.0f);
  const float u2 = ((float)(b >> 8) + 0.5f) * (1.0f / 16777216.0f);
  const float r = __builtin_amdgcn_sqrtf(-1.3862943611198906f * __builtin_amdgcn_logf(u1));
  z0 = r * __builtin_amdgcn_cosf(u2);
  z1 = r * __builtin_amdgcn_sinf(u2);
}

__device__ __forceinline__ void normal4(uint64_t g4, uint64_t seed, uint32_t step, float out[4]) {
  U4 c = {(uint32_t)g4, (uint32_t)(g4 >> 32), step, 0x46464446u };
  U4 r = philox4x32_10(c, (uint32_t)seed, (uint32_t)(seed >> 32));
  box_muller(r.x, r.y, out[0], out[1]);
  box_muller(r.z, r.w, out[2], out[3]);
}

__device__ __forceinline__ void load_normals(const float* z, size_t i0, int n, uint64_t seed, uint64_t elem_offset,
                                             uint32_t step, float zz[4]) {
  if (z) {
    for (int j = 0; j < n; ++j) zz[j] = z[i0 + j];
    return;
  }
  uint64_t g0 = elem_offset + i0;
  float a[4], b[4] = {0.f, 0.f, 0.f, 0.f};
  normal4(g0 >> 2, seed, step, a);
  const int sh = (int)(g0 & 3);
  if (sh) normal4((g0 >> 2) + 1, seed, step, b);
  const float c[7] = {a[0], a[1], a[2], a[3], b[0], b[1], b[2]};
#pragma unroll
  for (int j = 0; j < 4; ++j) zz[j] = sh == 0 ? c[j] : sh == 1 ? c[j + 1] : sh == 2 ? c[j + 2] : c[j + 3];
}

__device__ __forceinline__ double block_sum(double v, double* red) {
  __syncthreads();
  red[threadIdx.x] = v;
  __syncthreads();
  for (int s = 128; s > 0; s >>= 1) {
    if ((int)threadIdx.x < s) red[threadIdx.x] += red[threadIdx.x + s];
    __syncthreads();
  }
  return red[0];
}

#define FFD_KNOBS(I, B)                                                                                                 \
  I("ffn_mb", g_ffn_mb_override, 0, v >= 0 && v <= 4)      \
  I("ffn_height", g_ffn_height, 1, v >= 0 && v <= 2)       \
  I("ffn_persist", g_ffn_persist, 1, v >= 0 && v <= 8)     \
  B("ffn_rem", g_ffn_rem, 1)                               \
  B("ffn_split", g_ffn_split, 0)                           \
  I("ffn_rows", g_ffn_rows, 1, v >= 0 && v <= 2)           \
  I("ffn_rows_nw", g_ffn_rows_nw, 0, v == 0 || v == 4 || v == 8 || v == 12)   \
  I("ffn_rows_cps", g_ffn_rows_cps, 0, v >= 0 && v <= 2)   \
  B("ffn_rows_fuse", g_ffn_rows_fuse, 1)                   \
  I("rows_slices", g_rows_slices, 0, v >= -1 && v != 1 && v <= 32)   \
  I("rows_slices_fuse", g_rows_slices_fuse, 0, v >= 0 && v <= 2)   \
  I("mid_path", g_mid_path, 1, v == 0 || v == 1 || v == 2 || v == 4 || v == 8)   \
  B("small_path", g_small_path, 1)                         \
  I("small_wgs", g_small_wgs, 0, v >= 0)                   \
  I("attn_small", g_attn_small, 1, v == 0 || v == 1 || v == 2 || v == 4)   \
  I("attn_fused", g_attn_fused, 1, v >= 0 && v <= 1)       \
  I("attn_hpw", g_attn_hpw, 0, v >= 0 && v <= 2)           \
  I("attn_qg", g_attn_qg, 0, v >= 0 && v <= 3)             \
  B("attn_kvq", g_attn_kvq, 1)                             \
  B("embed_ldsx", g_embed_ldsx, 1)                         \
  I("embed_threads", g_embed_threads, 262144, v >= 256)    \
  I("lstm_wave", g_lstm_wave, 1, v >= 0 && v <= 2)         \
  B("lstm_wave_persist", g_lstm_wave_persist, 1)           \
  I("lstm_wave_per", g_lstm_wave_per, 0, v >= 0 && v <= 16)   \
  I("lstm_wave_chunk", g_lstm_wave_chunk, 0, v >= 0 && !(v > 1 && (v & 1)) && v <= 1024)   \
  I("lstm_wave_fault", g_lstm_wave_fault, 0, v >= 0)       \
  I("lstm_wave_spin_ms", g_lstm_wave_spin_ms, 2000, v >= 1 && v <= 20000)   \
  B("fuse_tail", g_fuse_tail, 1)                           \
  I("fail_alloc_after", g_fail_alloc_after, 0, v >= 0)

#define FFD_KNOB_DECL(key, var, ...) extern thread_local int var;
FFD_KNOBS(FFD_KNOB_DECL, FFD_KNOB_DECL)
#undef FFD_KNOB_DECL

template <int N>
__device__ __forceinline__ void wait_vm() {
  asm volatile("s_waitcnt vmcnt(%0)" ::"n"(N) : "memory");
}

__device__ __forceinline__ void dma_piece(const float* g, unsigned lds_byte) {
  asm volatile("s_mov_b32 m0, %0\n\ts_nop 0\n\tglobal_load_lds_dwordx4 %1, off" ::"s"(lds_byte), "v"(g)
               : "memory");
}
__device__ __forceinline__ unsigned lds_addr(const float* p) {
  return (unsigned)(unsigned long)((const __attribute__((address_space(3))) float*)p);
}


constexpr __host__ __device__ int lds_stride(int D) { return D + ((6 - D % 4) % 4); }

constexpr __host__ __device__ int dpack_groups(int D) { return cdiv(cdiv(D, 4), 4); }
constexpr __host__ __device__ size_t dpack_floats(int N, int D) {
  return (size_t)cdiv(N, 16) * dpack_groups(D) * 64 * 4;
}
constexpr __host__ __device__ size_t w2pack_floats(int D, int F) { return (size_t)(F / 16) * cdiv(D, 16) * 64 * 4; }


struct LayerWeights {
  const float *in_w, *in_b, *out_w, *out_b, *w1, *b1, *w2, *b2, *n1w, *n1b, *n2w, *n2b;
  float *in_wp = nullptr, *q_wp = nullptr, *kv_wp = nullptr;
  float* out_wp = nullptr;
  float* w1p = nullptr;
  float* w2p = nullptr;
  float* w2r = nullptr;
  float* ring = nullptr;
  float* ring_op = nullptr;
  float *w1s = nullptr, *w2s = nullptr;
  float *aw_full = nullptr, *aw_q = nullptr;
  float *aw_full2 = nullptr, *aw_q2 = nullptr;
  float* aw_kvq = nullptr;
};

hipError_t launch_pack_dweight(const float* W, float* Wp, int N, int D, hipStream_t s);
hipError_t launch_pack_w2(const float* W2, float* W2p, int D, int F, hipStream_t s);
constexpr __host__ __device__ int w2rem_groups(int D) { return (D % 16) / 4; }
constexpr __host__ __device__ size_t w2rem_floats(int D, int F) { return (size_t)(F / 16) * (w2rem_groups(D) ? w2rem_groups(D) : 1) * 64 * 4; }
hipError_t launch_pack_w2rem(const float* W2, float* W2r, int D, int F, hipStream_t s);
hipError_t launch_renorm_rows(float* W, int rows, int D, float max_norm, hipStream_t s);

hipError_t launch_time_embed(const float* ts, float t_imm, int n, const float* W, const float* dense_w,
                             const float* dense_b, float* temb, int D, hipStream_t s);
hipError_t launch_embed(const float* X, const float* We, const float* be, const float* pos, const float* temb,
                        int temb_stride, float* h, int B, int L, int C, int D, hipStream_t s);
hipError_t launch_unembed(const float* h, const float* Wu, const float* bu, float* score, int M, int C, int D,
                          hipStream_t s);

struct SdeParams {
  int sde;
  float a;
  float cs;
  float dt, sqdt;
};
SdeParams sde_params(int sde, double a, double b, double t, float step_size);
hipError_t launch_sde_step(float* x, const float* score, const float* z, const float* G, SdeParams p, uint64_t seed,
                           uint64_t elem_offset, uint32_t step, int B, int L, int C, hipStream_t s);
bool unembed_sde_supported(int C, int D);
hipError_t launch_unembed_sde(const float* h, const float* Wu, const float* bu, float* x, const float* z, const float* G,
                              SdeParams p, uint64_t seed, uint64_t elem_offset, uint32_t step, int B, int L, int C,
                              int D, hipStream_t s);

constexpr uint32_t SM_TAG_NOISE = 0xFFFFFFFEu, SM_TAG_TIMES = 0xFFFFFFFDu;
hipError_t launch_sm_perturb(const float* x0, float* x_noisy, const float* mean_coeff, const float* sigma, const float* G,
                             const float* z, uint64_t seed, uint64_t sample_offset, int B, int L, int C, hipStream_t s);
hipError_t launch_sm_loss(const float* score, const float* sigma, const float* G, const float* z, uint64_t seed,
                          uint64_t sample_offset, int likelihood_weighting, int reduce_mean, double* out, int B, int L,
                          int C, hipStream_t s);

hipError_t launch_linear(const float* X, const float* Wp, const float* bias, float* Y, int M, int N, int D, int ldy,
                         hipStream_t s);
hipError_t launch_linear_res_ln(const float* X, const float* Wp, const float* bias, const float* R, const float* g,
                                const float* beta, float* Y, int M, int D, hipStream_t s);
bool ffn_rem_rows(int D, int mb);
hipError_t launch_ffn_ln(const float* X, const LayerWeights& w, float* Y, int M, int D, int F, int mb, bool rem, int persist,
                         hipStream_t s, unsigned long long* stamp = nullptr);
int ffn_height_plan(int M, int D, int F);
hipError_t launch_oproj_ffn_ln(const float* attn, const float* Rres, const LayerWeights& w, float* Y, int M, int D, int F,
                               int mb, bool rem, hipStream_t s);
bool ffn_rows_supported(int D, int F);
bool ffn_rows_selected(int M, int D, int F);
size_t ffn_ring_floats(int D, int F);
hipError_t launch_pack_ffn_ring(const float* W1, const float* b1, const float* W2, float* out, int D, int F, hipStream_t s);
struct RowsArgs {
  const float *X, *Rin;
  const LayerWeights* w;
  float* Y;
  int M, D, F;
  int nw, cps;
  bool fused;
  int nslice;
  unsigned long long* stamp;
};
int rows_waves(int M);
hipError_t launch_ffn_rows(const RowsArgs& a, hipStream_t s);
bool ffn_rows_fused_selected(int M, int D, int F);
size_t ffn_ring_oproj_floats(int D);
hipError_t launch_pack_oproj_ring(const float* Wo, float* out, int D, hipStream_t s);
bool rows_slice_plan(int M, int D, int F, int* nw_out, int* nslice_out, int* unfused_out);
size_t rows_slice_floats(int M, int D, int nslice);
hipError_t launch_rows_reduce_ln(const float* P, const LayerWeights& w, float* Y, int M, int D, int nslice, hipStream_t s);
int small_path_splits(int M, int D, int F);
size_t small_path_partial_floats(int M, int D, int NS);
hipError_t launch_oproj_ffn_small(const float* attn, const float* xres, const LayerWeights& w, float* x1, float* P,
                                  float* Y, int M, int D, int F, int NS, hipStream_t s);
int mid_path_splits(int M, int D, int F);
hipError_t launch_ffn_mid(const float* x1, const LayerWeights& w, float* P, float* Y, int M, int D, int F, int NS, hipStream_t s);
bool ffn_split_supported(int D, int F);
size_t w1split_bytes(int D, int F);
size_t w2split_bytes(int D, int F);
hipError_t launch_pack_ffn_split(const float* W1, const float* W2, void* w1s, void* w2s, int D, int F, hipStream_t s);
hipError_t launch_ffn_ln_split(const float* X, const LayerWeights& w, float* Y, int M, int D, int F, hipStream_t s,
                               unsigned long long* stamp = nullptr);
size_t attn_pack_floats(int D, int H, int hpw, int q_only);
bool attn_kvq_supported(int hd);
hipError_t launch_pack_attn(const float* in_w, const float* in_b, float* pack, int D, int H, int hpw, int q_only,
                            hipStream_t s);
bool qkv_attention_supported(int D, int hd);
int qkv_attention_hpw(int D, int hd, int L);
int qkv_attention_small_split(int B, int H, int L);
int attn_qg(int QT, int hd, bool fused);
int num_cus();
struct AttnArgs {
  const float *x, *pack;
  const float *kt, *vt;
  float *kt_out, *vt_out;
  float* out;
  int B, L, n_own;
  unsigned long long* stamp;
};
hipError_t launch_qkv_attention(const AttnArgs& a, int D, int hd, int hpw, int q_only, int kspl, int qg, hipStream_t s);

hipError_t launch_linear_hm(const float* X, const float* Wp, const float* bias, float* out0, float* out1, float* out2,
                            int M, int nreg, int D, int L, int H, int hd, hipStream_t s);
hipError_t launch_attention(const float* q, const float* k, const float* v, const float* kt, const float* vt,
                            float* out, int B, int L, int H, int hd, int n_own, int qg, hipStream_t s);
hipError_t launch_kv_store(const float* k, const float* v, float* kt, float* vt, int L, int H, int hd, int n,
                           hipStream_t s);

hipError_t launch_lstm_layer(float* x, const float* gx, const float* whh, int B, int L, int D, hipStream_t s);
int lstm_wave_max_batch(int L, int D);
hipError_t launch_lstm_wave(float* x, const float* const* wih_pk, const float* const* whh_pk, const float* const* bias_pk, int NL,
                            int B, int L, int D, int* prog, float* state, int* err, hipStream_t s,
                            unsigned long long* trace = nullptr);
size_t lstm_wave_state_floats(int B, int D, int NL);
size_t lstm_wave_wpack_floats(int D);
size_t lstm_wave_bpack_floats(int D);
hipError_t launch_pack_lstm_wave(const float* wih, const float* whh, const float* bsum, float* ih_out, float* hh_out,
                                 float* b_out, int D, hipStream_t s);

hipError_t launch_dense(const float* X, const float* W, const float* b, const float* b2, const float* R, float* Y,
                        int M, int N, int K, int relu, hipStream_t s);
hipError_t launch_fresca(const float* in, float* out, float* work, int B, int L, int C, float low, float high,
                         double cutoff_ratio, int strategy, hipStream_t s);

enum CacheMode { CACHE_STD, CACHE_FULL, CACHE_PURE, CACHE_MIXED };
CacheMode cache_mode(int n_rec, int L);
enum AttnForm { ATTN_FUSED, ATTN_TWO_KERNEL };
enum FfnForm { FFN_LN_OPROJ, FFN_SMALL, FFN_ROWS_SLICED_OPROJ, FFN_ROWS_OPROJ, FFN_ROWS_SLICED, FFN_MID, FFN_SPLIT, FFN_ROWS,
               FFN_LN };
struct PackSet {
  bool aw_full, aw_full2, aw_kvq;
  bool ring;
};
struct LayerPlan {
  AttnForm attn;
  int hpw;
  int q_only;
  int kspl;
  int qg;
  FfnForm ffn;
  int mb;
  bool rem;
  int persist;
  int ns;
  int nw, cps;
  int nslice;
  int nm;
  bool oproj_separate;
  bool swap;
  size_t part_floats;
};
LayerPlan plan_layer(const ffd_model_desc& m, int B, CacheMode mode, const PackSet& packs);
struct LstmPlan {
  bool wave;
  int Bw;
};
LstmPlan plan_lstm(const ffd_model_desc& m, int B);

}
```

### fastfourierdiffusion_amd/csrc/ffd_qkvattn.hip

```cpp
#include <type_traits>

#include "ffd_internal.h"

namespace ffd {

typedef float f32x2 __attribute__((ext_vector_type(2)));
typedef float f32x16 __attribute__((ext_vector_type(16)));

__device__ __forceinline__ f32x2 pk_fma_lo(f32x2 p, f32x2 v, f32x2 acc) {
  asm("v_pk_fma_f32 %0, %1, %2, %0 op_sel_hi:[0,1,1]" : "+v"(acc) : "v"(p), "v"(v));
  return acc;
}
__device__ __forceinline__ f32x2 pk_fma_hi(f32x2 p, f32x2 v, f32x2 acc) {
  asm("v_pk_fma_f32 %0, %1, %2, %0 op_sel:[1,0,0] op_sel_hi:[1,1,1]" : "+v"(acc) : "v"(p), "v"(v));
  return acc;
}

#define FFD_STAMP_T() ((unsigned long long)__builtin_amdgcn_s_memtime())
struct WaveStamps {
  unsigned long long t[7] = {0, 0, 0, 0, 0, 0, 0}, qk = 0, sm = 0, pv = 0, n = 0;
  __device__ __forceinline__ void begin() { t[0] = __builtin_amdgcn_s_memrealtime(), t[1] = FFD_STAMP_T(); }
  __device__ __forceinline__ void write(unsigned long long* stamp, int nwaves) {
    if ((threadIdx.x & 63) == 0 && stamp != nullptr) {
      unsigned long long* r = stamp + ((size_t)blockIdx.x * nwaves + (threadIdx.x >> 6)) * 16;
      t[6] = FFD_STAMP_T();
#pragma unroll
      for (int i = 0; i < 7; ++i) r[i] = t[i];
      r[7] = qk, r[8] = sm, r[9] = pv, r[10] = n, r[11] = __builtin_amdgcn_s_getreg(4 | (0 << 6) | (31 << 11));
      r[12] = __builtin_amdgcn_s_memrealtime();
    }
  }
};

__global__ void k_pack_attn(const float* __restrict__ W, const float* __restrict__ b, float* __restrict__ awp,
                            float* __restrict__ abp, int D, int H, int hd, int hpw, int nct, int q_only, float qscale) {
  const int steps4 = (D + 15) / 16;
  const int NG = H / hpw;
  const bool kvq = q_only == 2;
  const int fph = q_only == 1 ? hd : 3 * hd;
  const int nf = kvq ? 32 : hpw * fph;
  const int total = NG * nct * steps4 * 64 * 4;
  for (int idx = blockIdx.x * blockDim.x + threadIdx.x; idx < total; idx += gridDim.x * blockDim.x) {
    const int i = idx & 3, lane = (idx >> 2) & 63;
    int rest = idx >> 8;
    const int j = rest % steps4;
    rest /= steps4;
    const int ct = rest % nct, hg = rest / nct;
    const int n = lane & 15, q = lane >> 4;
    const int fi = 16 * ct + n;
    int k;
    if (16 * j + 16 <= D) k = 16 * j + 4 * q + i;
    else k = (4 * i < D - 16 * j) ? 16 * j + 4 * i + q : -1;
    float v = 0.f;
    if (fi < nf && k >= 0 && k < D) {
      int hh = fi / fph, f = fi - hh * fph;
      int reg = f / hd, e = f - reg * hd;
      bool on = true;
      if (kvq) {
        hh = 0, on = n < (ct == 0 ? 2 * hd : hd) && ct < 2;
        reg = ct == 0 ? (n < hd ? 1 : 2) : 0, e = ct == 0 ? (n < hd ? n : n - hd) : n;
      }
      if (on) v = W[(size_t)(reg * D + (hg * hpw + hh) * hd + e) * D + k] * (reg == 0 ? qscale : 1.f);
    }
    awp[idx] = v;
  }
  const int nb = NG * nct * 16;
  for (int idx = blockIdx.x * blockDim.x + threadIdx.x; idx < nb; idx += gridDim.x * blockDim.x) {
    const int n = idx & 15, ct = (idx >> 4) % nct, hg = (idx >> 4) / nct;
    const int fi = 16 * ct + n;
    float v = 0.f;
    if (fi < nf) {
      int hh = fi / fph, f = fi - hh * fph;
      int reg = f / hd, e = f - reg * hd;
      bool on = true;
      if (kvq) {
        hh = 0, on = n < (ct == 0 ? 2 * hd : hd) && ct < 2;
        reg = ct == 0 ? (n < hd ? 1 : 2) : 0, e = ct == 0 ? (n < hd ? n : n - hd) : n;
      }
      if (on) v = b[reg * D + (hg * hpw + hh) * hd + e] * (reg == 0 ? qscale : 1.f);
    }
    abp[idx] = v;
  }
}

static int attn_nct(int hd, int hpw, int q_only) { return q_only == 2 ? 2 : cdiv(hpw * (q_only ? hd : 3 * hd), 16); }
bool attn_kvq_supported(int hd) { return 2 * hd <= 16 && 3 * hd > 16; }

size_t attn_pack_floats(int D, int H, int hpw, int q_only) {
  const int nct = attn_nct(D / H, hpw, q_only);
  return (size_t)(H / hpw) * nct * ((D + 15) / 16) * 256 + (size_t)(H / hpw) * nct * 16;
}

hipError_t launch_pack_attn(const float* in_w, const float* in_b, float* pack, int D, int H, int hpw, int q_only,
                            hipStream_t s) {
  const int hd = D / H;
  const int nct = attn_nct(hd, hpw, q_only);
  float* abp = pack + (size_t)(H / hpw) * nct * ((D + 15) / 16) * 256;
  const float qscale = 1.4426950408889634f / sqrtf((float)hd);
  hipLaunchKernelGGL(k_pack_attn, dim3(64), dim3(256), 0, s, in_w, in_b, pack, abp, D, H, hd, hpw, nct, q_only, qscale);
  return hipGetLastError();
}

__device__ __forceinline__ float wave_max_nonneg(float v) {
#define FFD_DPP_MAX(ctrl) \
  v = fmaxf(v, __builtin_bit_cast(float, __builtin_amdgcn_update_dpp(0, __builtin_bit_cast(int, v), ctrl, 0xF, 0xF, true)))
  FFD_DPP_MAX(0xB1);
  FFD_DPP_MAX(0x4E);
  FFD_DPP_MAX(0x141);
  FFD_DPP_MAX(0x140);
#undef FFD_DPP_MAX
  v = fmaxf(v, __shfl_xor(v, 16));
  return fmaxf(v, __shfl_xor(v, 32));
}

template <int HD>
__device__ __forceinline__ void head_norms(const float* kts, const float* qts, unsigned* nrm, int Lp, int LS, int tid, int nthreads,
                                           int jq0 = 0, int jq1 = 1 << 30) {
  float km = 0.f, qm = 0.f;
  for (int j = tid; j < Lp; j += nthreads) {
    float k2 = 0.f, q2 = 0.f;
    const bool qon = j >= jq0 && j < jq1;
#pragma unroll
    for (int e = 0; e < HD; ++e) {
      const float kv = kts[e * LS + j], qv = qon ? qts[e * LS + j] : 0.f;
      k2 = fmaf(kv, kv, k2), q2 = fmaf(qv, qv, q2);
    }
    km = fmaxf(km, k2), qm = fmaxf(qm, q2);
  }
  km = wave_max_nonneg(km), qm = wave_max_nonneg(qm);
  if ((threadIdx.x & 63) == 0) {
    atomicMax(nrm, __float_as_uint(km));
    atomicMax(nrm + 1, __float_as_uint(qm));
  }
}

template <int HD>
struct HeadDims {
  static constexpr int KST = (HD + 1) / 2;
  static constexpr int KSX = (HD + 2) / 2;
  static constexpr int SX = HD / 2;
  static constexpr int HX = HD & 1;
  static constexpr int HP = (HD + 1) / 2;
  static constexpr float T = 64.0f;
  static constexpr size_t floats(int LS) { return (size_t)LS * (8 + 4 * KST); }
};

template <int HD>
__device__ __forceinline__ bool head_bounded(const unsigned* nrm) {
  constexpr float T = HeadDims<HD>::T;
  return __builtin_amdgcn_ballot_w64(__uint_as_float(nrm[1]) * __uint_as_float(nrm[0]) <= T * T) != 0;
}

__device__ __forceinline__ void xcd_sample_group(int pair, int B, int NG, int& b, int& g) {
  const int nmain = (B >> 3) * 8 * NG;
  if (pair < nmain) {
    const int xcd = pair & 7, slot = pair >> 3;
    const int sb = slot / NG;
    b = sb * 8 + xcd, g = slot - sb * NG;
  } else {
    b = pair / NG, g = pair - b * NG;
  }
}

template <int HD, typename I>
__device__ __forceinline__ void fill_from_tables(float* vs, float* kts, int LS, const float* kt, const float* vt, int h,
                                                 int L, int Lp, int n_own, int q_only, I tid, I nthreads) {
  if (!q_only && n_own > 0) __syncthreads();
  const float* ktab = kt + (size_t)h * L * HD;
  const float* vtab = vt + (size_t)h * L * HD;
  for (int j = n_own + tid; j < L; j += nthreads) {
    float kx[HD], vx[8];
#pragma unroll
    for (int e = 0; e < 8; ++e) vx[e] = 0.f;
    const float* kp = ktab + (size_t)j * HD;
    const float* vp = vtab + (size_t)j * HD;
    if constexpr (HD % 2 == 0) {
#pragma unroll
      for (int e = 0; e < HD; e += 2) {
        const float2 a = *reinterpret_cast<const float2*>(kp + e);
        const float2 c2 = *reinterpret_cast<const float2*>(vp + e);
        kx[e] = a.x, kx[e + 1] = a.y, vx[e] = c2.x, vx[e + 1] = c2.y;
      }
    } else {
#pragma unroll
      for (int e = 0; e < HD; ++e) kx[e] = kp[e], vx[e] = vp[e];
    }
#pragma unroll
    for (int e = 0; e < HD; ++e) kts[e * LS + j] = kx[e];
    *reinterpret_cast<float4*>(vs + (size_t)j * 8) = float4{vx[0], vx[1], vx[2], vx[3]};
    *reinterpret_cast<float4*>(vs + (size_t)j * 8 + 4) = float4{vx[4], vx[5], vx[6], vx[7]};
  }
  if (q_only) {
    for (int j = L + tid; j < Lp; j += nthreads) {
#pragma unroll
      for (int e = 0; e < HD; ++e) kts[e * LS + j] = 0.f;
      *reinterpret_cast<float4*>(vs + (size_t)j * 8) = float4{0.f, 0.f, 0.f, 0.f};
      *reinterpret_cast<float4*>(vs + (size_t)j * 8 + 4) = float4{0.f, 0.f, 0.f, 0.f};
    }
  }
}

template <int HD, typename I>
__device__ __forceinline__ void publish_kv(const float* vs, const float* kts, int LS, float* kt_out, float* vt_out, int h,
                                           int L, int n_own, I tid, I nthreads) {
  for (int idx = tid; idx < n_own * HD; idx += nthreads) {
    const int j = idx / HD, e = idx - j * HD;
    kt_out[(size_t)h * L * HD + idx] = kts[e * LS + j];
    vt_out[(size_t)h * L * HD + idx] = vs[(size_t)j * 8 + e];
  }
}

template <int HD, int QG>
struct QRows {
  float mref[QG];
  f32x2 lsum[QG], acc[QG][HeadDims<HD>::HP];
};

#if defined(__HIP_DEVICE_COMPILE__)
typedef __attribute__((address_space(3))) const float lds_f32;
typedef __attribute__((address_space(3))) const float4 lds_f32x4;
#else
typedef const float lds_f32;
typedef const float4 lds_f32x4;
#endif

template <int HD, int QG, bool STAMP, bool STORE, int LSC>
__device__ __forceinline__ QRows<HD, QG> attend_qtiles(lds_f32* vs, lds_f32* kts, lds_f32* qts, int LSR,
                                                       int q_first, int q_step, int q_end, int t_lo, int t_hi,
                                                       bool head_bounded, int L, float* orow0, int ostride,
                                                       WaveStamps& st) {
  constexpr int KST = HeadDims<HD>::KST, KSX = HeadDims<HD>::KSX, SX = HeadDims<HD>::SX, HX = HeadDims<HD>::HX;
  constexpr int HP = HeadDims<HD>::HP;
  constexpr float T = HeadDims<HD>::T;
  const int lane = threadIdx.x & 63;
  const int half = lane >> 5, l31 = lane & 31;
  const int QT = (L + 31) >> 5;
  const int LS = LSC ? LSC : LSR;
  const bool xlane = half == HX;
  constexpr int PF = 4;
  auto load_v = [&](int r, int kbase, f32x2(&dst)[4]) {
    lds_f32* vr = vs + (size_t)(kbase + (r & 3) + 8 * (r >> 2)) * 8;
    const float4 v0 = *reinterpret_cast<lds_f32x4*>(vr);
    dst[0] = f32x2{v0.x, v0.y}, dst[1] = f32x2{v0.z, v0.w};
    if (HD > 4) {
      const float4 v1 = *reinterpret_cast<lds_f32x4*>(vr + 4);
      dst[2] = f32x2{v1.x, v1.y}, dst[3] = f32x2{v1.z, v1.w};
    } else {
      dst[2] = f32x2{0.f, 0.f}, dst[3] = f32x2{0.f, 0.f};
    }
  };
  QRows<HD, QG> rows;
  for (int qt0 = q_first; qt0 < q_end; qt0 += q_step) {
    float qf[QG][KSX], mref[QG];
    f32x2 lsum[QG], acc[QG][HP];
    bool ref_on = false;
    bool acc_empty[QG];
#pragma unroll
    for (int g = 0; g < QG; ++g) acc_empty[g] = true;
#pragma unroll
    for (int g = 0; g < QG; ++g) {
      const int qtile = (qt0 + g < QT) ? qt0 + g : QT - 1;
#pragma unroll
      for (int s = 0; s < KSX; ++s) {
        const int e = 2 * s + half;
        qf[g][s] = (e < HD) ? qts[e * LS + 32 * qtile + l31] : 0.f;
      }
      mref[g] = 0.f;
      lsum[g] = f32x2{0.f, 0.f};
#pragma unroll
      for (int e = 0; e < HP; ++e) acc[g][e] = f32x2{0.f, 0.f};
    }
#pragma unroll 1
    for (int t = t_lo; t < t_hi; ++t) {
      unsigned long long st_a = 0;
      if constexpr (STAMP) st_a = FFD_STAMP_T();
      float kf[KSX];
#pragma unroll
      for (int s = 0; s < KSX; ++s) {
        const int e = 2 * s + half;
        kf[s] = (s < KST && (2 * s + 1 < HD || half == 0)) ? kts[e * LS + 32 * t + l31] : 0.f;
      }
      if (xlane) kf[SX] = 1.0f;
      f32x16 sc[QG];
#pragma unroll
      for (int g = 0; g < QG; ++g) {
        f32x16 z = {0, 0, 0, 0, 0, 0, 0, 0, 0, 0, 0, 0, 0, 0, 0, 0};
#pragma unroll
        for (int s = 0; s < KSX; ++s) {
          if (HD % 2 == 0 && s == SX && !ref_on) continue;
          z = __builtin_amdgcn_mfma_f32_32x32x2f32(kf[s], qf[g][s], z, 0, 0, 0);
        }
        sc[g] = z;
      }
      const int kbase = 32 * t + 4 * half;
      f32x2 vb[PF][4];
#pragma unroll
      for (int r = 0; r < PF; ++r) load_v(r, kbase, vb[r]);
      __builtin_amdgcn_sched_barrier(0);
      if constexpr (STAMP) {
        asm volatile("v_mov_b32 %0, %0" : "+v"(sc[QG - 1][15]));
        const unsigned long long n = FFD_STAMP_T();
        st.qk += n - st_a, st_a = n, ++st.n;
        __builtin_amdgcn_sched_barrier(0);
      }
      if (32 * t + 32 > L) {
#pragma unroll
        for (int r4 = 0; r4 < 4; ++r4) {
          if (32 * t + 8 * r4 + 8 > L) {
#pragma unroll
            for (int rr = 0; rr < 4; ++rr) {
              const bool dead = kbase + rr + 8 * r4 >= L;
#pragma unroll
              for (int g = 0; g < QG; ++g) sc[g][4 * r4 + rr] = dead ? -INFINITY : sc[g][4 * r4 + rr];
            }
          }
        }
      }
#pragma unroll
      for (int g = 0; g < QG; ++g) {
        if (ref_on || !head_bounded) {
        float bm = __builtin_fmaxf(__builtin_fmaxf(sc[g][0], sc[g][1]), sc[g][2]);
#pragma unroll
        for (int r = 3; r < 15; r += 2) bm = __builtin_fmaxf(__builtin_fmaxf(bm, sc[g][r]), sc[g][r + 1]);
        bm = __builtin_fmaxf(bm, sc[g][15]);
        const float bmx = fmaxf(bm, __shfl_xor(bm, 32));
        const bool first = acc_empty[g];
        const bool refresh = first ? (fabsf(bmx) > T) : (bmx > T);
        if (__builtin_amdgcn_ballot_w64(refresh) != 0) ref_on = true;
        if (refresh) {
          const float delta = bmx;
          mref[g] += delta;
          if (!first) {
            const float corr = __builtin_amdgcn_exp2f(-delta);
            lsum[g] *= corr;
#pragma unroll
            for (int e = 0; e < HP; ++e) acc[g][e] *= corr;
          }
#pragma unroll
          for (int r = 0; r < 16; ++r) sc[g][r] -= delta;
          if (xlane) qf[g][SX] = -mref[g];
        }
        }
        acc_empty[g] = false;
#pragma unroll
        for (int r = 0; r < 16; r += 2) {
          const float p0 = __builtin_amdgcn_exp2f(sc[g][r]);
          const float p1 = __builtin_amdgcn_exp2f(sc[g][r + 1]);
          sc[g][r] = p0;
          sc[g][r + 1] = p1;
          lsum[g] += f32x2{p0, p1};
        }
      }
      if constexpr (STAMP) {
        __builtin_amdgcn_sched_barrier(0);
        const unsigned long long n = FFD_STAMP_T();
        st.sm += n - st_a, st_a = n;
        __builtin_amdgcn_sched_barrier(0);
      }
#pragma unroll
      for (int r = 0; r < 16; ++r) {
        f32x2 vv[4];
#pragma unroll
        for (int e = 0; e < 4; ++e) vv[e] = vb[r % PF][e];
#pragma unroll
        for (int g = 0; g < QG; ++g) {
          const f32x2 pp = f32x2{sc[g][r & ~1], sc[g][(r & ~1) + 1]};
#pragma unroll
          for (int e = 0; e < HP; ++e) acc[g][e] = (r & 1) ? pk_fma_hi(pp, vv[e], acc[g][e]) : pk_fma_lo(pp, vv[e], acc[g][e]);
        }
        if (r + PF < 16) {
          load_v(r + PF, kbase, vb[r % PF]);
          __builtin_amdgcn_sched_barrier(0);
        }
      }
      if constexpr (STAMP) {
        __builtin_amdgcn_sched_barrier(0);
        st.pv += FFD_STAMP_T() - st_a;
        __builtin_amdgcn_sched_barrier(0);
      }
    }
    if constexpr (STAMP) st.t[5] = FFD_STAMP_T();
    if constexpr (STORE) {
#pragma unroll
      for (int g = 0; g < QG; ++g) {
        float l = lsum[g].x + lsum[g].y;
        l += __shfl_xor(l, 32);
        const float inv = __builtin_amdgcn_rcpf(l);
        const int q = 32 * (qt0 + g) + l31;
        float o[2 * HP];
#pragma unroll
        for (int e = 0; e < HP; ++e) {
          float a0 = acc[g][e].x, a1 = acc[g][e].y;
          a0 += __shfl_xor(a0, 32);
          a1 += __shfl_xor(a1, 32);
          o[2 * e] = a0 * inv, o[2 * e + 1] = a1 * inv;
        }
        if (half == 0 && q < L && qt0 + g < QT) {
          float* orow = orow0 + (size_t)q * ostride;
#pragma unroll
          for (int e = 0; e < HD; ++e) orow[e] = o[e];
        }
      }
    } else {
#pragma unroll
      for (int g = 0; g < QG; ++g) {
        rows.mref[g] = mref[g], rows.lsum[g] = lsum[g];
#pragma unroll
        for (int e = 0; e < HP; ++e) rows.acc[g][e] = acc[g][e];
      }
    }
  }
  return rows;
}

template <int D, int HD, int QG, int NCT, bool SPLIT = false, bool STAMP = false, bool KVQ = false>
__global__ __launch_bounds__(256, (SPLIT && NCT >= 2 ? 2 : QG <= 2 ? 4 : 3)) void k_qkv_attention(
    const float* __restrict__ x, const float* __restrict__ awp, const float* __restrict__ kt,
    const float* __restrict__ vt, float* __restrict__ kt_out, float* __restrict__ vt_out, float* __restrict__ out,
    int B, int L, int n_own, int q_only, int qsplit, int kspl, unsigned long long* __restrict__ stamp) {
  WaveStamps st;
  if constexpr (STAMP) st.begin();
  constexpr int H = D / HD;
  constexpr int KST = HeadDims<HD>::KST;
  constexpr int C16 = D / 16;
  constexpr int REM = (D % 16) / 4;
  constexpr int S4 = (D + 15) / 16;
  extern __shared__ __align__(16) float lds[];
  const int lane = threadIdx.x & 63, wave = threadIdx.x >> 6;
  const int nwaves = blockDim.x >> 6;
  int b, h, qs = 0;
  {
    int pair = blockIdx.x;
    if constexpr (SPLIT) qs = pair % qsplit, pair /= qsplit;
    xcd_sample_group(pair, B, H, b, h);
  }
  const int KT = (L + 31) >> 5;
  const int Lp = KT * 32;
  constexpr int LSC = (QG == 4 && !SPLIT) ? 516 : 0;
  const int LS = LSC ? LSC : Lp + 4;
  float* vs = lds;
  float* kts = vs + (size_t)LS * 8;
  float* qts = kts + (size_t)2 * KST * LS;
  constexpr int PS = 2 + 2 * HeadDims<HD>::HP;
  unsigned* nrm = reinterpret_cast<unsigned*>(lds + HeadDims<HD>::floats(LS) + (SPLIT ? 4 * 32 * PS : 0));
  if (threadIdx.x < 2) nrm[threadIdx.x] = 0u;

  if constexpr (HD % 2 == 1) {
    for (int idx = threadIdx.x; idx < LS * (8 + 4 * KST); idx += blockDim.x) vs[idx] = 0.f;
    __syncthreads();
  }

  {
    const int n = lane & 15, qq = lane >> 4;
    constexpr bool VREM = HD == 6 && NCT == 2 && QG >= 3;
    constexpr int NCTM = VREM ? 1 : NCT;
    float4 wf[NCTM][S4];
    const float4* Wq = reinterpret_cast<const float4*>(awp) + (size_t)h * NCT * S4 * 64;
#pragma unroll
    for (int ct = 0; ct < NCTM; ++ct)
#pragma unroll
      for (int j = 0; j < S4; ++j) wf[ct][j] = Wq[((size_t)ct * S4 + j) * 64 + lane];
    float4 w16[VREM ? C16 : 1], w17[VREM ? C16 : 1];
    float2 w16r = {0.f, 0.f}, w17r = {0.f, 0.f};
    const float* abp = awp + (size_t)H * NCT * S4 * 256 + (size_t)h * NCT * 16;
    float b16 = 0.f, b17 = 0.f;
    if constexpr (VREM) {
#pragma unroll
      for (int j = 0; j < C16; ++j) w16[j] = Wq[((size_t)S4 + j) * 64 + 16 * qq], w17[j] = Wq[((size_t)S4 + j) * 64 + 16 * qq + 1];
      static_assert(!VREM || REM <= 2, "remainder k-steps of the two vector-ALU columns");
      if constexpr (REM > 0) {
        w16r = *reinterpret_cast<const float2*>(&Wq[((size_t)S4 + S4 - 1) * 64 + 16 * qq]);
        w17r = *reinterpret_cast<const float2*>(&Wq[((size_t)S4 + S4 - 1) * 64 + 16 * qq + 1]);
      }
      b16 = abp[16], b17 = abp[17];
    }
    float bias[NCTM];
    int sbase[NCTM];
    bool sv[NCTM];
#pragma unroll
    for (int ct = 0; ct < NCTM; ++ct) {
      bias[ct] = abp[ct * 16 + n];
      const int fi = 16 * ct + n;
      int reg = fi / HD, e = fi - reg * HD;
      int kind = q_only ? (fi < HD ? 0 : 3) : (reg > 2 ? 3 : reg);
      if constexpr (KVQ) {
        static_assert(!KVQ || (SPLIT && NCT == 2 && 2 * HD <= 16), "kv | q pack");
        kind = ct == 0 ? (n < HD ? 1 : n < 2 * HD ? 2 : 3) : (n < HD ? 0 : 3);
        e = ct == 0 ? (n < HD ? n : n - HD) : n;
      }
      sv[ct] = kind == 2;
      sbase[ct] = kind == 3 ? -1 : kind == 0 ? LS * 8 + 2 * KST * LS + e * LS : kind == 1 ? LS * 8 + e * LS : e;
    }
    const float* xb = x + (size_t)b * L * D;
    const int TT = Lp >> 4;
    int tt0 = 0, tt1 = TT;
    int ot0 = 0, ot1 = TT;
    if constexpr (SPLIT) {
      const int qpw = nwaves / kspl;
      ot0 = min(2 * qs * qpw, TT), ot1 = min(ot0 + 2 * qpw, TT);
      if (q_only) tt0 = ot0, tt1 = ot1;
    }
    auto load_x = [&](int tt, float4(&xa)[C16 > 0 ? C16 : 1], float(&xr)[REM > 0 ? REM : 1]) {
      int tok = 16 * tt + n;
      if (tok >= L) tok = L - 1;
      const float* xp = xb + (size_t)tok * D;
#pragma unroll
      for (int j = 0; j < C16; ++j) xa[j] = *reinterpret_cast<const float4*>(xp + 16 * j + 4 * qq);
#pragma unroll
      for (int i = 0; i < REM; ++i) xr[i] = xp[16 * C16 + 4 * i + qq];
    };
    constexpr int PFX = VREM ? 3 : 4;
    float4 xa[PFX][C16 > 0 ? C16 : 1];
    float xr[PFX][REM > 0 ? REM : 1];
#pragma unroll
    for (int u = 0; u < PFX; ++u)
      load_x(min(tt0 + wave + u * nwaves, TT - 1), xa[u], xr[u]);
    __builtin_amdgcn_sched_barrier(0);
    if constexpr (STAMP) st.t[2] = FFD_STAMP_T();
    constexpr int MAXT = 8;
#pragma unroll
    for (int it = 0; it < MAXT; ++it) {
      const int u = it % PFX;
      const int tt = tt0 + wave + it * nwaves;
      if (tt >= tt1) break;
      f32x4 acc[NCTM];
#pragma unroll
      for (int ct = 0; ct < NCTM; ++ct) acc[ct] = f32x4{0.f, 0.f, 0.f, 0.f};
      const bool own = !KVQ || (tt >= ot0 && tt < ot1);
      auto tile_mfmas = [&](auto CTC) {
        constexpr int ct = decltype(CTC)::value;
#pragma unroll
        for (int j = 0; j < C16; ++j) {
          acc[ct] = mfma16(xa[u][j].x, wf[ct][j].x, acc[ct]);
          acc[ct] = mfma16(xa[u][j].y, wf[ct][j].y, acc[ct]);
          acc[ct] = mfma16(xa[u][j].z, wf[ct][j].z, acc[ct]);
          acc[ct] = mfma16(xa[u][j].w, wf[ct][j].w, acc[ct]);
        }
#pragma unroll
        for (int i = 0; i < REM; ++i) {
          const float4 w4 = wf[ct][S4 - 1];
          const float wv = i == 0 ? w4.x : i == 1 ? w4.y : i == 2 ? w4.z : w4.w;
          acc[ct] = mfma16(xr[u][i], wv, acc[ct]);
        }
      };
      if constexpr (KVQ) {
        tile_mfmas(std::integral_constant<int, 0>{});
        if (own) tile_mfmas(std::integral_constant<int, 1>{});
      } else {
#pragma unroll
        for (int j = 0; j < C16; ++j) {
#pragma unroll
          for (int ct = 0; ct < NCTM; ++ct) {
            acc[ct] = mfma16(xa[u][j].x, wf[ct][j].x, acc[ct]);
            acc[ct] = mfma16(xa[u][j].y, wf[ct][j].y, acc[ct]);
            acc[ct] = mfma16(xa[u][j].z, wf[ct][j].z, acc[ct]);
            acc[ct] = mfma16(xa[u][j].w, wf[ct][j].w, acc[ct]);
          }
        }
#pragma unroll
        for (int i = 0; i < REM; ++i) {
#pragma unroll
          for (int ct = 0; ct < NCTM; ++ct) {
            const float4 w4 = wf[ct][S4 - 1];
            const float wv = i == 0 ? w4.x : i == 1 ? w4.y : i == 2 ? w4.z : w4.w;
            acc[ct] = mfma16(xr[u][i], wv, acc[ct]);
          }
        }
      }
      float p16 = 0.f, p17 = 0.f;
      if constexpr (VREM) {
#pragma unroll
        for (int j = 0; j < C16; ++j) {
          p16 = fmaf(xa[u][j].x, w16[j].x, p16), p17 = fmaf(xa[u][j].x, w17[j].x, p17);
          p16 = fmaf(xa[u][j].y, w16[j].y, p16), p17 = fmaf(xa[u][j].y, w17[j].y, p17);
          p16 = fmaf(xa[u][j].z, w16[j].z, p16), p17 = fmaf(xa[u][j].z, w17[j].z, p17);
          p16 = fmaf(xa[u][j].w, w16[j].w, p16), p17 = fmaf(xa[u][j].w, w17[j].w, p17);
        }
#pragma unroll
        for (int i = 0; i < REM; ++i) {
          p16 = fmaf(xr[u][i], i == 0 ? w16r.x : w16r.y, p16), p17 = fmaf(xr[u][i], i == 0 ? w17r.x : w17r.y, p17);
        }
      }
      if (it + PFX < MAXT) load_x(min(tt + PFX * nwaves, TT - 1), xa[u], xr[u]);
      __builtin_amdgcn_sched_barrier(0);
      if constexpr (VREM) {
        p16 += __shfl_xor(p16, 16), p17 += __shfl_xor(p17, 16);
        p16 += __shfl_xor(p16, 32), p17 += __shfl_xor(p17, 32);
        if (qq == 0) *reinterpret_cast<float2*>(vs + (size_t)(16 * tt + n) * 8 + 4) = float2{p16 + b16, p17 + b17};
      }
      const int t0 = 16 * tt + 4 * qq;
#pragma unroll
      for (int ct = 0; ct < NCTM; ++ct) {
        const float4 o = float4{acc[ct][0] + bias[ct], acc[ct][1] + bias[ct], acc[ct][2] + bias[ct],
                                acc[ct][3] + bias[ct]};
        if (sbase[ct] >= 0 && (ct == 0 || own)) {
          if (!sv[ct]) {
            *reinterpret_cast<float4*>(lds + sbase[ct] + t0) = o;
          } else {
            float* vp = lds + sbase[ct] + t0 * 8;
            vp[0] = o.x, vp[8] = o.y, vp[16] = o.z, vp[24] = o.w;
          }
        }
      }
    }
  }
  if constexpr (STAMP) st.t[3] = FFD_STAMP_T();
  if (kt != nullptr) fill_from_tables<HD>(vs, kts, LS, kt, vt, h, L, Lp, n_own, q_only, threadIdx.x, blockDim.x);
  __syncthreads();
  {
    int jq0 = 0, jq1 = Lp;
    if constexpr (SPLIT) {
      if (q_only || KVQ) {
        const int qpw = nwaves / kspl;
        jq0 = min(32 * qs * qpw, Lp), jq1 = min(jq0 + 32 * qpw, Lp);
      }
    }
    head_norms<HD>(kts, qts, nrm, Lp, LS, threadIdx.x, blockDim.x, jq0, jq1);
  }
  if (kt_out != nullptr && b == 0 && qs == 0)
    publish_kv<HD>(vs, kts, LS, kt_out, vt_out, h, L, n_own, threadIdx.x, blockDim.x);

  __syncthreads();
  if constexpr (STAMP) st.t[4] = FFD_STAMP_T();
  const bool bounded = head_bounded<HD>(nrm);
  float* orow0 = out + (size_t)b * L * D + h * HD;
  if constexpr (SPLIT) {
    const int qpw = nwaves / kspl, kps = (KT + kspl - 1) / kspl;
    const int qt = qs * qpw + wave / kspl, t_lo = (wave % kspl) * kps;
    int t_hi = min(KT, t_lo + kps);
    if (qt >= KT) t_hi = t_lo;
    const QRows<HD, 1> r = attend_qtiles<HD, 1, STAMP, false, 0>((lds_f32*)vs, (lds_f32*)kts, (lds_f32*)qts, LS, qt, 1,
                                                                 qt + 1, t_lo, t_hi, bounded, L, orow0, D, st);
    const int half = lane >> 5, l31 = lane & 31;
    float* part = lds + HeadDims<HD>::floats(LS);
    float l = r.lsum[0].x + r.lsum[0].y;
    l += __shfl_xor(l, 32);
    float o[PS - 2];
#pragma unroll
    for (int e = 0; e < HeadDims<HD>::HP; ++e) {
      float a0 = r.acc[0][e].x, a1 = r.acc[0][e].y;
      o[2 * e] = a0 + __shfl_xor(a0, 32), o[2 * e + 1] = a1 + __shfl_xor(a1, 32);
    }
    if (half == 0) {
      float* pw = part + (size_t)(wave * 32 + l31) * PS;
      pw[0] = (t_lo < t_hi) ? r.mref[0] : -INFINITY;
      pw[1] = l;
#pragma unroll
      for (int e = 0; e < PS - 2; ++e) pw[2 + e] = o[e];
    }
    __syncthreads();
    for (int idx = threadIdx.x; idx < qpw * 32 * HD; idx += blockDim.x) {
      const int e = idx % HD, ql = (idx / HD) & 31, qi = idx / (HD * 32);
      const int qtile = qs * qpw + qi, q = 32 * qtile + ql;
      if (qtile >= KT || q >= L) continue;
      const float* p0 = part + (size_t)(qi * kspl * 32 + ql) * PS;
      float mx = -INFINITY;
      for (int sp = 0; sp < kspl; ++sp) mx = fmaxf(mx, p0[(size_t)sp * 32 * PS]);
      float lt = 0.f, ot = 0.f;
      for (int sp = 0; sp < kspl; ++sp) {
        const float* pp = p0 + (size_t)sp * 32 * PS;
        const float wgt = __builtin_amdgcn_exp2f(pp[0] - mx);
        lt = fmaf(pp[1], wgt, lt), ot = fmaf(pp[2 + e], wgt, ot);
      }
      orow0[(size_t)q * D + e] = ot / lt;
    }
  } else {
    attend_qtiles<HD, QG, STAMP, true, LSC>((lds_f32*)vs, (lds_f32*)kts, (lds_f32*)qts, LS, wave * QG, nwaves * QG, KT,
                                            0, KT, bounded, L, orow0, D, st);
  }
  if constexpr (STAMP) st.write(stamp, nwaves);
}

template <int D, int HD, int HPW, int QG, int NCT, bool QO, bool STAMP = false>
__global__ __launch_bounds__(128 * HPW, 3) void k_qkv_attention_mh(
    const float* __restrict__ x, const float* __restrict__ awp, const float* __restrict__ kt,
    const float* __restrict__ vt, float* __restrict__ kt_out, float* __restrict__ vt_out, float* __restrict__ out,
    int B, int L, int n_own, int q_only, unsigned long long* __restrict__ stamp) {
  WaveStamps st;
  if constexpr (STAMP) st.begin();
  constexpr int H = D / HD;
  constexpr int NG = H / HPW;
  constexpr int KST = HeadDims<HD>::KST;
  constexpr int C16 = D / 16;
  constexpr int REM = (D % 16) / 4;
  constexpr int S4 = (D + 15) / 16;
  constexpr int NW = 2 * HPW;
  constexpr int MAXT = 3;
  constexpr bool REMV = HD == 6 && HPW == 2 && NCT == 3;
  constexpr int NCTM = REMV ? 2 : NCT;
  extern __shared__ __align__(16) float lds[];
  const int lane = threadIdx.x & 63, wave = threadIdx.x >> 6;
  int b, hg;
  xcd_sample_group(blockIdx.x, B, NG, b, hg);
  const int KT = (L + 31) >> 5;
  const int Lp = KT * 32;
  constexpr int LS = 64 * QG + 4;
  constexpr int RS = HeadDims<HD>::floats(LS);
  float4* wl = reinterpret_cast<float4*>(lds + (size_t)HPW * RS);
  constexpr int fph = QO ? HD : 3 * HD;
  if (threadIdx.x < 2 * HPW)
    reinterpret_cast<unsigned*>(lds + (size_t)HPW * RS + (size_t)NCT * S4 * 256)[threadIdx.x] = 0u;

  {
    const int n = lane & 15, qq = lane >> 4;
    const float* xb = x + (size_t)b * L * D;
    const int TT = Lp >> 4;
    auto load_x = [&](int tt, float4(&xa)[C16 > 0 ? C16 : 1], float(&xr)[REM > 0 ? REM : 1]) {
      int tok = 16 * tt + n;
      if (tok >= L) tok = L - 1;
      const float* xp = xb + (size_t)tok * D;
#pragma unroll
      for (int j = 0; j < C16; ++j) xa[j] = *reinterpret_cast<const float4*>(xp + 16 * j + 4 * qq);
#pragma unroll
      for (int i = 0; i < REM; ++i) xr[i] = xp[16 * C16 + 4 * i + qq];
    };
    float4 xa[MAXT][C16 > 0 ? C16 : 1];
    float xr[MAXT][REM > 0 ? REM : 1];
#pragma unroll
    for (int u = 0; u < MAXT; ++u) load_x(min(wave + u * NW, TT - 1), xa[u], xr[u]);
    {
      const float4* Wq = reinterpret_cast<const float4*>(awp) + (size_t)hg * NCT * S4 * 64;
      for (int i = threadIdx.x; i < NCT * S4 * 64; i += 64 * NW) wl[i] = Wq[i];
      if constexpr (HD % 2 == 1) {
        for (int idx = threadIdx.x; idx < HPW * RS; idx += 64 * NW) lds[idx] = 0.f;
      }
    }
    const float* abp = awp + (size_t)NG * NCT * S4 * 256 + (size_t)hg * NCT * 16;
    float bias[NCTM];
    int sbase[NCTM];
    bool sv[NCTM];
#pragma unroll
    for (int ct = 0; ct < NCTM; ++ct) {
      bias[ct] = abp[ct * 16 + n];
      const int fi = 16 * ct + n;
      const int hh = fi / fph, f = fi - hh * fph;
      const int reg = f / HD, e = f - reg * HD;
      sv[ct] = reg == 2;
      sbase[ct] = hh >= HPW ? -1
                  : hh * RS + (reg == 0 ? LS * 8 + 2 * KST * LS + e * LS : reg == 1 ? LS * 8 + e * LS : e);
    }
    __syncthreads();
    if constexpr (STAMP) st.t[2] = FFD_STAMP_T();
    float wrem[REMV ? 4 * C16 + REM : 1];
    float bvv[REMV ? 4 : 1];
    if constexpr (REMV) {
      static_assert(!REMV || REM <= 4, "remainder k-steps come from one staged float4");
#pragma unroll
      for (int j = 0; j < C16; ++j) {
        const float4 w4 = wl[(2 * S4 + j) * 64 + 16 * qq + (lane & 3)];
        wrem[4 * j] = w4.x, wrem[4 * j + 1] = w4.y, wrem[4 * j + 2] = w4.z, wrem[4 * j + 3] = w4.w;
      }
      if constexpr (REM > 0) {
        const float4 r4 = wl[(2 * S4 + S4 - 1) * 64 + 16 * qq + (lane & 3)];
#pragma unroll
        for (int i = 0; i < REM; ++i) wrem[4 * C16 + i] = i == 0 ? r4.x : i == 1 ? r4.y : i == 2 ? r4.z : r4.w;
      }
#pragma unroll
      for (int f = 0; f < 4; ++f) bvv[f] = abp[2 * 16 + f];
    }
#pragma unroll
    for (int it = 0; it < MAXT; ++it) {
      const int tt = wave + it * NW;
      if (tt >= TT) break;
      if constexpr (REMV) {
        f32x4 pr = f32x4{0.f, 0.f, 0.f, 0.f};
#pragma unroll
        for (int j = 0; j < C16; ++j) {
          pr = __builtin_amdgcn_mfma_f32_4x4x1f32(wrem[4 * j], xa[it][j].x, pr, 0, 0, 0);
          pr = __builtin_amdgcn_mfma_f32_4x4x1f32(wrem[4 * j + 1], xa[it][j].y, pr, 0, 0, 0);
          pr = __builtin_amdgcn_mfma_f32_4x4x1f32(wrem[4 * j + 2], xa[it][j].z, pr, 0, 0, 0);
          pr = __builtin_amdgcn_mfma_f32_4x4x1f32(wrem[4 * j + 3], xa[it][j].w, pr, 0, 0, 0);
        }
#pragma unroll
        for (int i = 0; i < REM; ++i) pr = __builtin_amdgcn_mfma_f32_4x4x1f32(wrem[4 * C16 + i], xr[it][i], pr, 0, 0, 0);
        float pv[4];
#pragma unroll
        for (int f = 0; f < 4; ++f) {
          float p = pr[f];
          p += __shfl_xor(p, 16);
          p += __shfl_xor(p, 32);
          pv[f] = p + bvv[f];
        }
        if (qq == 0) {
          float* vp = lds + RS + (16 * tt + n) * 8 + 2;
          *reinterpret_cast<float2*>(vp) = float2{pv[0], pv[1]};
          *reinterpret_cast<float2*>(vp + 2) = float2{pv[2], pv[3]};
        }
      }
      f32x4 acc[NCTM];
#pragma unroll
      for (int ct = 0; ct < NCTM; ++ct) acc[ct] = f32x4{0.f, 0.f, 0.f, 0.f};
#pragma unroll
      for (int j = 0; j < C16; ++j) {
#pragma unroll
        for (int ct = 0; ct < NCTM; ++ct) {
          const float4 w4 = wl[(ct * S4 + j) * 64 + lane];
          acc[ct] = mfma16(xa[it][j].x, w4.x, acc[ct]);
          acc[ct] = mfma16(xa[it][j].y, w4.y, acc[ct]);
          acc[ct] = mfma16(xa[it][j].z, w4.z, acc[ct]);
          acc[ct] = mfma16(xa[it][j].w, w4.w, acc[ct]);
        }
      }
      if constexpr (REM > 0) {
#pragma unroll
        for (int ct = 0; ct < NCTM; ++ct) {
          const float4 w4 = wl[(ct * S4 + S4 - 1) * 64 + lane];
#pragma unroll
          for (int i = 0; i < REM; ++i) {
            const float wv = i == 0 ? w4.x : i == 1 ? w4.y : i == 2 ? w4.z : w4.w;
            acc[ct] = mfma16(xr[it][i], wv, acc[ct]);
          }
        }
      }
      const int t0 = 16 * tt + 4 * qq;
#pragma unroll
      for (int ct = 0; ct < NCTM; ++ct) {
        const float4 o = float4{acc[ct][0] + bias[ct], acc[ct][1] + bias[ct], acc[ct][2] + bias[ct],
                                acc[ct][3] + bias[ct]};
        if (sbase[ct] >= 0) {
          if (!sv[ct]) {
            *reinterpret_cast<float4*>(lds + sbase[ct] + t0) = o;
          } else {
            float* vp = lds + sbase[ct] + t0 * 8;
            vp[0] = o.x, vp[8] = o.y, vp[16] = o.z, vp[24] = o.w;
          }
        }
      }
    }
  }
  if constexpr (STAMP) st.t[3] = FFD_STAMP_T();
  const int hh = wave >> 1, gw = wave & 1;
  const int h = hg * HPW + hh;
  float* vs = lds + (size_t)hh * RS;
  float* kts = vs + LS * 8;
  float* qts = kts + 2 * KST * LS;
  if (kt != nullptr) fill_from_tables<HD>(vs, kts, LS, kt, vt, h, L, Lp, n_own, q_only, gw * 64 + lane, 128);
  __syncthreads();
  unsigned* nrm = reinterpret_cast<unsigned*>(lds + (size_t)HPW * RS + (size_t)NCT * S4 * 256) + 2 * hh;
  head_norms<HD>(kts, qts, nrm, Lp, LS, gw * 64 + lane, 128);
  if (kt_out != nullptr && b == 0) publish_kv<HD>(vs, kts, LS, kt_out, vt_out, h, L, n_own, gw * 64 + lane, 128);

  __syncthreads();
  if constexpr (STAMP) st.t[4] = FFD_STAMP_T();
  attend_qtiles<HD, QG, STAMP, true, LS>((lds_f32*)vs, (lds_f32*)kts, (lds_f32*)qts, LS, gw * QG, 2 * QG, KT, 0, KT,
                                         head_bounded<HD>(nrm), L, out + (size_t)b * L * D + h * HD, D, st);
  if constexpr (STAMP) st.write(stamp, NW);
}

template <int D, int HD, int HPW, int QG, int NCT, bool QO>
static hipError_t launch_mh_t(const AttnArgs& a, int q_only, hipStream_t s) {
  constexpr int S4 = (D + 15) / 16;
  const int KT = (a.L + 31) / 32;
  const size_t lds = (HPW * HeadDims<HD>::floats(64 * QG + 4) + (size_t)NCT * S4 * 256 + (size_t)HPW * 2) * sizeof(float);
  if (cdiv(2 * KT, 2 * HPW) > 3 || cdiv(KT, 2) > QG) return hipErrorInvalidValue;
  if constexpr (D == 72 && HD == 6) {
    if (a.stamp != nullptr) {
      hipLaunchKernelGGL((k_qkv_attention_mh<D, HD, HPW, QG, NCT, QO, true>), dim3(a.B * (D / HD / HPW)), dim3(128 * HPW), lds,
                         s, a.x, a.pack, a.kt, a.vt, a.kt_out, a.vt_out, a.out, a.B, a.L, a.n_own, q_only, a.stamp);
      return hipGetLastError();
    }
  }
  if (a.stamp != nullptr) return hipErrorInvalidValue;
  if (q_only != (QO ? 1 : 0)) return hipErrorInvalidValue;
  auto kern = k_qkv_attention_mh<D, HD, HPW, QG, NCT, QO>;
  hipLaunchKernelGGL(kern, dim3(a.B * (D / HD / HPW)), dim3(128 * HPW), lds, s, a.x, a.pack, a.kt, a.vt, a.kt_out, a.vt_out,
                     a.out, a.B, a.L, a.n_own, q_only, (unsigned long long*)nullptr);
  return hipGetLastError();
}

template <int D, int HD>
static hipError_t launch_mh2(const AttnArgs& a, int q_only, int qg, hipStream_t s) {
  constexpr int NF = (2 * 3 * HD + 15) / 16, NQ = (2 * HD + 15) / 16;
#define FFD_MH(g) \
  if (qg == g) return q_only ? launch_mh_t<D, HD, 2, g, NQ, true>(a, 1, s) : launch_mh_t<D, HD, 2, g, NF, false>(a, 0, s);
  FFD_MH(1) FFD_MH(2) FFD_MH(3)
#undef FFD_MH
  return hipErrorInvalidValue;
}

template <int D, int HD, int QG, int NCT>
static hipError_t launch_t(const AttnArgs& a, int q_only, hipStream_t s) {
  const int KT = (a.L + 31) / 32;
  const size_t lds = (HeadDims<HD>::floats(KT * 32 + 4) + (size_t)2 * KT) * sizeof(float);
  int nwaves = cdiv(KT, QG);
  if (nwaves > 4) nwaves = 4;
  if (cdiv(2 * KT, nwaves) > 8) return hipErrorInvalidValue;
  if constexpr (D == 72 && HD == 6 && NCT == 2) {
    if (a.stamp != nullptr) {
      hipLaunchKernelGGL((k_qkv_attention<D, HD, QG, NCT, false, true>), dim3(a.B * (D / HD)), dim3(64 * nwaves), lds, s, a.x,
                         a.pack, a.kt, a.vt, a.kt_out, a.vt_out, a.out, a.B, a.L, a.n_own, q_only, 1, 1, a.stamp);
      return hipGetLastError();
    }
  }
  if (a.stamp != nullptr) return hipErrorInvalidValue;
  hipLaunchKernelGGL((k_qkv_attention<D, HD, QG, NCT>), dim3(a.B * (D / HD)), dim3(64 * nwaves), lds, s, a.x, a.pack, a.kt,
                     a.vt, a.kt_out, a.vt_out, a.out, a.B, a.L, a.n_own, q_only, 1, 1, (unsigned long long*)nullptr);
  return hipGetLastError();
}

template <int D, int HD, int NCT, bool KVQ = false>
static hipError_t launch_split_t(const AttnArgs& a, int q_only, int kspl, hipStream_t s) {
  const int KT = (a.L + 31) / 32;
  if (cdiv(2 * KT, 4) > 8 || (kspl != 1 && kspl != 2 && kspl != 4)) return hipErrorInvalidValue;
  const int qsplit = cdiv(KT, 4 / kspl);
  const size_t lds =
      (HeadDims<HD>::floats(KT * 32 + 4) + (size_t)4 * 32 * (2 + 2 * HeadDims<HD>::HP) + (size_t)2 * KT) * sizeof(float);
  hipLaunchKernelGGL((k_qkv_attention<D, HD, 1, NCT, true, false, KVQ>), dim3(a.B * (D / HD) * qsplit), dim3(256), lds, s, a.x,
                     a.pack, a.kt, a.vt, a.kt_out, a.vt_out, a.out, a.B, a.L, a.n_own, q_only, qsplit, kspl,
                     (unsigned long long*)nullptr);
  return hipGetLastError();
}

int qkv_attention_small_split(int B, int H, int L) {
  if (g_attn_small == 0 || L > 512) return 0;
  if (g_attn_small == 2 || g_attn_small == 4) return g_attn_small;
  const int QT = (L + 31) / 32;
  if (8L * B * H * QT <= 5L * num_cus()) return 4;
  if (4L * B * H * cdiv(QT, 2) <= 5L * num_cus()) return 2;
  return 0;
}

int attn_qg(int QT, int hd, bool fused) {
  if (QT == 1) return 1;
  if (QT % 3 == 0) return 3;
  if (fused && hd <= 6 && QT % 4 == 0 && QT >= 16) return 4;
  return 2;
}

template <int D, int HD>
static hipError_t launch_dh(const AttnArgs& a, int q_only, int kspl, int qg, hipStream_t s) {
  constexpr int NCTF = (3 * HD + 15) / 16;
  if (kspl) {
    if (a.stamp != nullptr) return hipErrorInvalidValue;
    if constexpr (2 * HD <= 16 && 3 * HD > 16) {
      if (q_only == 2) return launch_split_t<D, HD, 2, true>(a, 0, kspl, s);
    }
    if (q_only == 2) return hipErrorInvalidValue;
    return q_only ? launch_split_t<D, HD, 1>(a, 1, kspl, s) : launch_split_t<D, HD, NCTF>(a, 0, kspl, s);
  }
  if (q_only == 2) return hipErrorInvalidValue;
  if (q_only && a.stamp != nullptr) return hipErrorInvalidValue;
#define FFD_QG(g, nct) if (qg == g) return launch_t<D, HD, g, nct>(a, q_only, s);
  if (q_only) {
    FFD_QG(1, 1) FFD_QG(3, 1)
    if constexpr (HD <= 6) {
      FFD_QG(4, 1)
    }
    FFD_QG(2, 1)
    return hipErrorInvalidValue;
  }
  FFD_QG(2, NCTF) FFD_QG(1, NCTF) FFD_QG(3, NCTF)
  if constexpr (HD <= 6) {
    FFD_QG(4, NCTF)
  }
#undef FFD_QG
  return hipErrorInvalidValue;
}

#define FFD_QKV_LIST(X, X2) X2(72, 6) X2(60, 5) X(24, 6) X(8, 2) X(64, 8) X2(48, 4) X(32, 8) X(16, 4) X(24, 3)
#define FFD_QKV_IS(dd, hh) if (D == dd && hd == hh) return true;
#define FFD_QKV_SKIP(dd, hh)

bool qkv_attention_supported(int D, int hd) {
  FFD_QKV_LIST(FFD_QKV_IS, FFD_QKV_IS)
  return false;
}
static bool qkv_attention_two_heads(int D, int hd) {
  FFD_QKV_LIST(FFD_QKV_SKIP, FFD_QKV_IS)
  return false;
}

int qkv_attention_hpw(int D, int hd, int L) {
  return (g_attn_hpw == 1 || !qkv_attention_two_heads(D, hd) || L > 192) ? 1 : 2;
}

hipError_t launch_qkv_attention(const AttnArgs& a, int D, int hd, int hpw, int q_only, int kspl, int qg, hipStream_t s) {
  if (a.B <= 0) return hipSuccess;
  if (hpw == 2) {
#define FFD_QA2(dd, hh) if (D == dd && hd == hh) return launch_mh2<dd, hh>(a, q_only, qg, s);
    FFD_QKV_LIST(FFD_QKV_SKIP, FFD_QA2)
#undef FFD_QA2
    return hipErrorInvalidValue;
  }
#define FFD_QA(dd, hh) if (D == dd && hd == hh) return launch_dh<dd, hh>(a, q_only, kspl, qg, s);
  FFD_QKV_LIST(FFD_QA, FFD_QA)
#undef FFD_QA
  return hipErrorInvalidValue;
}

}
```

### include/ffd.h

```cpp
#ifndef FFD_H
#define FFD_H

#include <stddef.h>
#include <stdint.h>

#ifdef __cplusplus
extern "C" {
#endif

typedef struct ffd_ctx ffd_ctx;

typedef enum {
  FFD_OK = 0,
  FFD_ERR_INVALID = -1,
  FFD_ERR_UNSUPPORTED = -2,
  FFD_ERR_STATE = -3,
  FFD_ERR_HIP = -4,
  FFD_ERR_NOMEM = -5
} ffd_status;

enum { FFD_MODEL_TRANSFORMER = 0, FFD_MODEL_LSTM = 1, FFD_MODEL_MLP = 2 };
enum { FFD_SDE_VP = 0, FFD_SDE_VE = 1 };

typedef struct {
  int32_t kind;
  int32_t n_channels;
  int32_t max_len;
  int32_t d_model;
  int32_t n_head;
  int32_t num_layers;
  int32_t dim_feedforward;
  int32_t sde;
  double sde_a;
  double sde_b;
  int32_t fourier_noise_scaling;
  double eps;
} ffd_model_desc;

typedef struct {
  int32_t K;
  int32_t R;
} ffd_cache_cfg;

typedef struct {
  int64_t recompute_count;
  int64_t cache_hit_count;
  int64_t current_step;
  int32_t table_allocated;
  int32_t reserved;
} ffd_cache_stats;


int ffd_create(ffd_ctx** out, const ffd_model_desc* desc, int device);
void ffd_destroy(ffd_ctx* ctx);
const char* ffd_last_error(const ffd_ctx* ctx);
const char* ffd_version(void);


int ffd_load_weight(ffd_ctx* ctx, const char* name, const float* data, size_t n);
int ffd_finalize_weights(ffd_ctx* ctx);


int ffd_host_noise_scaling(int max_len, int fourier_noise_scaling, float* G_out);
int ffd_host_timesteps(int n, double eps, float* ts_out, float* step_size_out);
int ffd_host_gate(int step, int max_len, int K, int R);


int ffd_score_forward(ffd_ctx* ctx, const float* x, float t, float* score_out, int B, void* stream);

int ffd_score_forward_cached(ffd_ctx* ctx, const float* x, float t, float* score_out, float* crf_out,
                             int B, int n_recompute, void* stream);

int ffd_score_forward_ts(ffd_ctx* ctx, const float* x, const float* timesteps, float* score_out, float* crf_out,
                         int B, int n_recompute, void* stream);

typedef struct {
  int32_t sde;
  int32_t reserved;
  double a;
  double b;
} ffd_sde_desc;

int ffd_sde_step(const ffd_sde_desc* sde, float* x, const float* score, const float* G, double t,
                 float step_size, const float* z, uint64_t seed, uint64_t sample_offset, int step, int B,
                 int L, int C, void* stream);

int ffd_prior(const ffd_sde_desc* sde, float* x, const float* z, const float* G, uint64_t seed,
              uint64_t sample_offset, int B, int L, int C, void* stream);

int ffd_dft(const float* in, float* out, int B, int L, int C, void* stream);
int ffd_idft(const float* in, float* out, int B, int L, int C, void* stream);
int ffd_unstandardize_idft(const float* in, float* out, const float* mean, const float* std, int B, int L, int C,
                           void* stream);
int ffd_dft_standardize(const float* in, float* out, const float* mean, const float* std, int B, int L, int C,
                        void* stream);

int ffd_positional_encoding(const float* x, float* weight, float* out, int B, int L, int D, float max_norm,
                            void* stream);
int ffd_time_encoding(const float* x, const float* timesteps, const float* W, const float* dense_w,
                      const float* dense_b, float* temb_work, float* out, int B, int L, int D, void* stream);

enum { FFD_FRESCA_SPATIAL = 0, FFD_FRESCA_ENERGY = 1 };
int ffd_fresca(const float* in, float* out, float* work, int B, int L, int C, float low_scale, float high_scale,
               double cutoff_ratio, int strategy, void* stream);

int ffd_fresca2d(const float* in, float* out, float* work, int B, int H, int W, int C, float low_scale,
                 float high_scale, double cutoff_ratio, int strategy, void* stream);

typedef struct {
  float low_scale, high_scale;
  double cutoff_ratio;
  int32_t strategy;
  int32_t num_steps;
} ffd_fresca_cfg;
int ffd_fresca_enable(ffd_ctx* ctx, const ffd_fresca_cfg* cfg);
int ffd_fresca_disable(ffd_ctx* ctx);


int ffd_freq_decompose(const float* x, float* low, float* high, int B, int L, int D, double low_freq_ratio,
                       void* stream);

int ffd_hermite_predict(const float* history, const double* timesteps, double target, int order, float* out, int K,
                        size_t n, void* stream);

int ffd_spectral_density(const float* xf, float* out, int B, int L, int C, void* stream);

size_t ffd_w2_work_bytes(int n, int m, int D, int K, size_t budget_bytes);
int ffd_w2_sliced(const float* orig, int n, const float* other, int m, int D, const float* dirs, int K,
                  int standardise, double* dist_out, void* work, size_t work_bytes, void* stream);
int ffd_w2_marginal(const float* orig, int n, const float* other, int m, int D, int standardise, double* dist_out,
                    void* work, size_t work_bytes, void* stream);
int ffd_w2_prepare(const float* x, int n, int D, const float* dirs, int K, float* prepared_out, void* work,
                   size_t work_bytes, void* stream);
int ffd_w2_against_prepared(const float* prepared, int n, const float* other, int m, int D, const float* dirs, int K,
                            int standardise, double* dist_out, void* work, size_t work_bytes, void* stream);
int ffd_w2_summary(const double* dist, int K, double* mean_max_out, void* stream);
size_t ffd_col_mean_work_bytes(int n, int D);
int ffd_col_mean(const float* x, int n, int D, float* mean_out, void* work, size_t work_bytes, void* stream);

int ffd_w2_bench_kernels(const float* x, int n, int D, const float* dirs, int K, float* rows, float* scratch,
                         const float* other_rows, int m, double* dist, int iters, float* ms_out, void* stream);


int ffd_sm_draw_times(float* t_out, int B, double eps, double T, uint64_t seed, uint64_t sample_offset, void* stream);
int ffd_sm_perturb(const float* x0, float* x_noisy, const float* mean_coeff, const float* sigma, const float* G,
                   const float* z, uint64_t seed, uint64_t sample_offset, int B, int L, int C, void* stream);
int ffd_sm_loss(const float* score, const float* sigma, const float* G, const float* z, uint64_t seed,
                uint64_t sample_offset, int likelihood_weighting, int reduce_mean, double* per_sample_out, int B, int L,
                int C, void* stream);
int ffd_sm_eval_batch(ffd_ctx* ctx, const float* x0, const float* timesteps, const float* mean_coeff, const float* sigma,
                      const float* z, uint64_t seed, uint64_t sample_offset, int likelihood_weighting, int reduce_mean,
                      double* per_sample_out, int B, void* stream);

typedef struct {
  float* ring;
  int32_t n_slots;
  int32_t every;
  float* last;
  int32_t last_every;
  int32_t reserved;
} ffd_crf_capture_cfg;
int ffd_cache_crf_capture(ffd_ctx* ctx, const ffd_crf_capture_cfg* cfg);


int ffd_cache_enable(ffd_ctx* ctx, const ffd_cache_cfg* cfg);
int ffd_cache_disable(ffd_ctx* ctx);
int ffd_cache_reset(ffd_ctx* ctx);
int ffd_cache_configure(ffd_ctx* ctx, const ffd_cache_cfg* cfg);
int ffd_cache_stats_get(const ffd_ctx* ctx, ffd_cache_stats* out);
int ffd_cache_tables_read(ffd_ctx* ctx, float* k_out, float* v_out, void* stream);

int ffd_sample_batch(ffd_ctx* ctx, float* x, int B, const float* timesteps, int n_steps, float step_size,
                     int first_step, int n_run, uint64_t seed, uint64_t sample_offset, const float* z_inject,
                     int use_cache, int global_step0, void* stream);

int ffd_tune(const char* key, int value);
int ffd_tune_get(const char* key, int* value);


double ffd_flops_per_sample_step(const ffd_ctx* ctx, int cache_hit);
double ffd_ffn_flops_per_launch(const ffd_ctx* ctx, int B);
enum {
  FFD_K_FFN = 0,
  FFD_K_ATTN = 1,
  FFD_K_OUTPROJ = 2,
  FFD_K_LSTM_REC = 3,
  FFD_K_LSTM_GATES = 4,
  FFD_K_SDE = 5,
  FFD_K_EMBED = 6,
  FFD_K_UNEMBED = 7,
  FFD_K_COUNT = 8
};
int ffd_lstm_trace(ffd_ctx* ctx, unsigned long long* host_out, int capacity_units, int* n_units_out);

int ffd_kernel_timing_begin(ffd_ctx* ctx, uint32_t class_mask, int max_launches);
int ffd_kernel_timing_end(ffd_ctx* ctx);
int ffd_kernel_timing_get(const ffd_ctx* ctx, int kernel_class, float* avg_ms_out, int* launches_out);
const char* ffd_kernel_work(const ffd_ctx* ctx, int kernel_class, int B, int cache_hit, double* flops_out,
                            double* bytes_out);
int ffd_bench_ffn(ffd_ctx* ctx, int B, int iters, float* ms_out, void* stream);

int ffd_probe_ffn_clock(ffd_ctx* ctx, int B, double warm_seconds, double* ghz_out, double* loop_us_out,
                        unsigned long long* raw_out, int raw_capacity, int* nwg_out, void* stream);

int ffd_async_status(ffd_ctx* ctx);

int ffd_probe_attn(ffd_ctx* ctx, int B, int n_recompute, double warm_seconds, int iters, float* ms_out,
                   unsigned long long* raw_out, int raw_capacity, int* nrec_out, void* stream);

#ifdef __cplusplus
}
#endif
#endif
```

Before: 99.47 samples/s.

## Skip runtime attention max/norm pass using static weight-derived score bound

Measured after the change: 100.8 samples/s (median of 6 runs). 1.4% higher.

```diff
diff --git a/fastfourierdiffusion_amd/_native.py b/fastfourierdiffusion_amd/_native.py
--- a/fastfourierdiffusion_amd/_native.py
+++ b/fastfourierdiffusion_amd/_native.py
@@ -78,6 +78,7 @@
     "ffd_host_noise_scaling": (C.c_int, [C.c_int, C.c_int, _F]),
     "ffd_host_timesteps": (C.c_int, [C.c_int, C.c_double, _F, _F]),
     "ffd_host_gate": (C.c_int, [C.c_int, C.c_int, C.c_int, C.c_int]),
+    "ffd_host_attn_score_bound": (C.c_int, [_F, _F, _F, _F, C.c_int, C.c_int, C.c_double, C.POINTER(C.c_double)]),
     "ffd_score_forward": (C.c_int, [_P, _P, C.c_float, _P, C.c_int, _P]),
     "ffd_score_forward_cached": (C.c_int, [_P, _P, C.c_float, _P, _P, C.c_int, C.c_int, _P]),
     "ffd_sde_step": (C.c_int, [C.POINTER(SdeDesc), _P, _P, _P, C.c_double, C.c_float, _P, C.c_uint64, C.c_uint64,
diff --git a/fastfourierdiffusion_amd/csrc/ffd_api.hip b/fastfourierdiffusion_amd/csrc/ffd_api.hip
--- a/fastfourierdiffusion_amd/csrc/ffd_api.hip
+++ b/fastfourierdiffusion_amd/csrc/ffd_api.hip
@@ -220,6 +220,7 @@
            : p.hpw == 2                                         ? cdiv(QT, 2)
            : !p.q_only && (g_attn_qg == 1 || g_attn_qg == 2)    ? g_attn_qg
                                                                 : attn_qg(QT, hd, true);
+    p.attn_static = g_attn_static_bound && (mode == CACHE_STD || mode == CACHE_FULL);
   } else {
     p.qg = QT == 1 ? 1 : g_attn_qg ? g_attn_qg : attn_qg(QT, hd, false);
   }
@@ -341,6 +342,62 @@
     return n < 0 ? 0 : n;
   }
   return 0;
+}
+
+static double sym_eig_max_upper(std::vector<double>& a, int n) {
+  for (int sweep = 0; sweep < 64; ++sweep) {
+    double off = 0.0, diag = 0.0;
+    for (int i = 0; i < n; ++i)
+      for (int j = 0; j < n; ++j) (i == j ? diag : off) += a[i * n + j] * a[i * n + j];
+    if (off <= 1e-30 * diag) break;
+    for (int p = 0; p < n; ++p)
+      for (int q = p + 1; q < n; ++q) {
+        const double apq = a[p * n + q];
+        if (apq == 0.0) continue;
+        const double theta = (a[q * n + q] - a[p * n + p]) / (2.0 * apq);
+        const double t = (theta >= 0.0 ? 1.0 : -1.0) / (fabs(theta) + sqrt(theta * theta + 1.0));
+        const double c = 1.0 / sqrt(t * t + 1.0), sn = t * c;
+        for (int k = 0; k < n; ++k) {
+          const double akp = a[k * n + p], akq = a[k * n + q];
+          a[k * n + p] = c * akp - sn * akq, a[k * n + q] = sn * akp + c * akq;
+        }
+        for (int k = 0; k < n; ++k) {
+          const double apk = a[p * n + k], aqk = a[q * n + k];
+          a[p * n + k] = c * apk - sn * aqk, a[q * n + k] = sn * apk + c * aqk;
+        }
+      }
+  }
+  double best = 0.0;
+  for (int i = 0; i < n; ++i) {
+    double r = a[i * n + i];
+    for (int j = 0; j < n; ++j)
+      if (j != i) r += fabs(a[i * n + j]);
+    best = std::max(best, r);
+  }
+  return best * (1.0 + 1e-12);
+}
+
+int ffd_host_attn_score_bound(const float* in_w, const float* in_b, const float* ln_w, const float* ln_b, int d, int hd,
+                              double q_scale, double* bound_out) {
+  if (!in_w || !in_b || !ln_w || !ln_b || !bound_out || d < 1 || hd < 1 || d % hd != 0) return FFD_ERR_INVALID;
+  constexpr double kLnSlack = 1e-4;
+  double gmax = 0.0, b2 = 0.0;
+  for (int i = 0; i < d; ++i) gmax = std::max(gmax, fabs((double)ln_w[i])), b2 += (double)ln_b[i] * ln_b[i];
+  const double R = (sqrt((double)d) * gmax + sqrt(b2)) * (1.0 + kLnSlack);
+  std::vector<double> gram((size_t)hd * hd);
+  auto reach = [&](int row0) {
+    for (int i = 0; i < hd; ++i)
+      for (int j = 0; j < hd; ++j) {
+        double acc = 0.0;
+        for (int k = 0; k < d; ++k) acc += (double)in_w[(size_t)(row0 + i) * d + k] * in_w[(size_t)(row0 + j) * d + k];
+        gram[(size_t)i * hd + j] = acc;
+      }
+    double bb = 0.0;
+    for (int i = 0; i < hd; ++i) bb += (double)in_b[row0 + i] * in_b[row0 + i];
+    return sqrt(sym_eig_max_upper(gram, hd)) * R + sqrt(bb);
+  };
+  for (int h = 0; h < d / hd; ++h) bound_out[h] = q_scale * reach(h * hd) * reach(d + h * hd);
+  return FFD_OK;
 }
 
 static void bind_weights(ffd_ctx* ctx) {
@@ -529,6 +586,22 @@
       }
       if (l.w1s) HIPCHECK(launch_pack_ffn_split(l.w1, l.w2, l.w1s, l.w2s, d, F, s));
     }
+    const int hd = d / m.n_head;
+    std::vector<float> in_w((size_t)3 * d * d), in_b(3 * d), g(d), be(d);
+    std::vector<double> bound(m.n_head);
+    for (size_t i = 0; i < ctx->layers.size(); ++i) {
+      LayerWeights& l = ctx->layers[i];
+      l.attn_bounded = false;
+      if (i == 0 || !l.aw_full) continue;
+      HIPCHECK(hipMemcpy(in_w.data(), l.in_w, in_w.size() * sizeof(float), hipMemcpyDeviceToHost));
+      HIPCHECK(hipMemcpy(in_b.data(), l.in_b, in_b.size() * sizeof(float), hipMemcpyDeviceToHost));
+      HIPCHECK(hipMemcpy(g.data(), ctx->layers[i - 1].n2w, d * sizeof(float), hipMemcpyDeviceToHost));
+      HIPCHECK(hipMemcpy(be.data(), ctx->layers[i - 1].n2b, d * sizeof(float), hipMemcpyDeviceToHost));
+      if (ffd_host_attn_score_bound(in_w.data(), in_b.data(), g.data(), be.data(), d, hd, attn_q_scale(hd), bound.data()))
+        continue;
+      l.attn_bounded = true;
+      for (double v : bound) l.attn_bounded = l.attn_bounded && v <= (double)ATTN_SCORE_T;
+    }
   } else if (m.kind == FFD_MODEL_LSTM) {
     for (LstmLayer& l : ctx->lstm) {
       if (!l.wih_p) {
@@ -595,8 +668,9 @@
     const float* pack = p.q_only == 2 ? w.aw_kvq
                         : p.hpw == 2  ? (p.q_only ? w.aw_q2 : w.aw_full2)
                                       : (p.q_only ? w.aw_q : w.aw_full);
-    return launch_qkv_attention(AttnArgs{x, pack, kt, vt, kt_out, vt_out, out, B, L, n_own, stamp}, d, hd, p.hpw, p.q_only,
-                                p.kspl, p.qg, s);
+    return launch_qkv_attention(AttnArgs{x, pack, kt, vt, kt_out, vt_out, out, B, L, n_own, stamp,
+                                         p.attn_static && w.attn_bounded && kt == nullptr},
+                                d, hd, p.hpw, p.q_only, p.kspl, p.qg, s);
   }
   if (stamp != nullptr) return hipErrorInvalidValue;
   const size_t M = (size_t)B * L;
@@ -1139,7 +1213,11 @@
       break;
     case FFD_K_ATTN:
       if (tr) {
-        name = p.attn == ATTN_FUSED ? "k_qkv_attention" : "k_linear_hm + k_attention_mfma";
+        bool any_static = false;
+        for (const LayerWeights& l : ctx->layers) any_static = any_static || (p.attn_static && l.attn_bounded);
+        name = p.attn != ATTN_FUSED ? "k_linear_hm + k_attention_mfma"
+               : any_static         ? "k_qkv_attention<static bound>"
+                                    : "k_qkv_attention";
         fl = M * (2.0 * d * (cache_hit ? d : 3.0 * d) + 4.0 * L * d);
         by = 4.0 * (2.0 * M * d + 3.0 * d * d + (cache_hit ? 2.0 * L * d : 0.0));
         if (p.attn == ATTN_TWO_KERNEL) by += 4.0 * 2.0 * M * (cache_hit ? d : 3.0 * d);
@@ -1312,7 +1390,7 @@
   hipLaunchKernelGGL(k_fill_hash, dim3(1024), dim3(256), 0, s, ctx->h1.p, (size_t)B * L * d, 0x9E3779B9u);
   HIPCHECK(hipGetLastError());
   auto launch = [&](unsigned long long* st) {
-    return run_attention(ctx, p, ctx->layers[0], ctx->h1.p, cu.tables ? ctx->kt : nullptr, cu.tables ? ctx->vt : nullptr,
+    return run_attention(ctx, p, ctx->layers[m.num_layers > 1 ? 1 : 0], ctx->h1.p, cu.tables ? ctx->kt : nullptr, cu.tables ? ctx->vt : nullptr,
                          nullptr, nullptr, B, cu.n_own, s, st);
   };
   if ((rc = time_launches(ctx, s, [&]() { return launch(nullptr); }, 20, warm_seconds, iters, ms_out))) return rc;
diff --git a/fastfourierdiffusion_amd/csrc/ffd_ffn_rows.hip b/fastfourierdiffusion_amd/csrc/ffd_ffn_rows.hip
--- a/fastfourierdiffusion_amd/csrc/ffd_ffn_rows.hip
+++ b/fastfourierdiffusion_amd/csrc/ffd_ffn_rows.hip
@@ -346,8 +346,8 @@
     lnp[i] = i < D ? b2[i] : i < 2 * D ? gam[i - D] : i < 3 * D ? bet[i - 2 * D]
            : i < 4 * D ? bo[i - 3 * D] : i < 5 * D ? gam1[i - 4 * D] : bet1[i - 5 * D];
   {
-    const float* src = slot_src(0) + lane * 4;
-    for (int g = wave; g < (OP ? C::NFPP : C::SLOT_G); g += NW) dma_piece(src + g * 256, ring_base + g * 1024);
+    const float* src = slot_src(0);
+    for (int g = wave; g < (OP ? C::NFPP : C::SLOT_G); g += NW) dma_piece_sbase(src + g * 256, lane * 16, ring_base + g * 1024);
   }
   float4 rin[CTA][4], rinrem[NRA];
   load_rows(X, xv, xrem);
@@ -358,12 +358,12 @@
 #pragma unroll
   for (int j = 1; j < C::AHEAD; ++j)
     if (j < total) {
-      const float* src = slot_src(j % NSL) + lane * 4;
+      const float* src = slot_src(j % NSL);
       const unsigned dst = ring_base + (unsigned)(j % NSLOT) * (C::SLOT_FLOATS * 4);
 #pragma unroll
       for (int i = 0; i < C::NPW; ++i) {
         const int g0 = wave + i * NW, g = g0 < C::SLOT_G ? g0 : g0 - C::SLOT_G;
-        dma_piece(src + g * 256, dst + g * 1024);
+        dma_piece_sbase(src + g * 256, lane * 16, dst + g * 1024);
       }
     }
   asm volatile("s_waitcnt lgkmcnt(0)" ::: "memory");
@@ -391,13 +391,14 @@
   const float* slot = ringl + (it % NSLOT) * C::SLOT_FLOATS;                                                           \
   const float* nslot = ringl + ((it + 1) % NSLOT) * C::SLOT_FLOATS;                                                    \
   const bool dma_on = it + C::AHEAD < total;                                                                           \
-  const float* dma_src = slot_src(wnext) + lane_i * 4;                                                                 \
+  const float* dma_src = slot_src(wnext);               \
+  const unsigned dma_lane = (unsigned)lane_i * 16u;                                                                    \
   const unsigned dma_dst = ring_base + (unsigned)((it + C::AHEAD) % NSLOT) * (C::SLOT_FLOATS * 4);                     \
   int dma_g = wave;                                                       \
   auto issue_piece = [&]() {          \
     if (dma_on) {                                                                                                      \
       const int g = dma_g < C::SLOT_G ? dma_g : dma_g - C::SLOT_G;                                                     \
-      dma_piece(dma_src + g * 256, dma_dst + g * 1024);                                                                \
+      dma_piece_sbase(dma_src + g * 256, dma_lane, dma_dst + g * 1024);                                                \
       dma_g += NW;                                                                                                     \
     }                                                                                                                  \
   }
diff --git a/fastfourierdiffusion_amd/csrc/ffd_internal.h b/fastfourierdiffusion_amd/csrc/ffd_internal.h
--- a/fastfourierdiffusion_amd/csrc/ffd_internal.h
+++ b/fastfourierdiffusion_amd/csrc/ffd_internal.h
@@ -104,6 +104,7 @@
   I("attn_hpw", g_attn_hpw, 0, v >= 0 && v <= 2)           \
   I("attn_qg", g_attn_qg, 0, v >= 0 && v <= 3)             \
   B("attn_kvq", g_attn_kvq, 1)                             \
+  B("attn_static_bound", g_attn_static_bound, 1)           \
   B("embed_ldsx", g_embed_ldsx, 1)                         \
   I("embed_threads", g_embed_threads, 262144, v >= 256)    \
   I("lstm_wave", g_lstm_wave, 1, v >= 0 && v <= 2)         \
@@ -126,6 +127,10 @@
 
 __device__ __forceinline__ void dma_piece(const float* g, unsigned lds_byte) {
   asm volatile("s_mov_b32 m0, %0\n\ts_nop 0\n\tglobal_load_lds_dwordx4 %1, off" ::"s"(lds_byte), "v"(g)
+               : "memory");
+}
+__device__ __forceinline__ void dma_piece_sbase(const float* base, unsigned lane_byte, unsigned lds_byte) {
+  asm volatile("s_mov_b32 m0, %0\n\ts_nop 0\n\tglobal_load_lds_dwordx4 %1, %2" ::"s"(lds_byte), "v"(lane_byte), "s"(base)
                : "memory");
 }
 __device__ __forceinline__ unsigned lds_addr(const float* p) {
@@ -155,6 +160,7 @@
   float *aw_full = nullptr, *aw_q = nullptr;
   float *aw_full2 = nullptr, *aw_q2 = nullptr;
   float* aw_kvq = nullptr;
+  bool attn_bounded = false;
 };
 
 hipError_t launch_pack_dweight(const float* W, float* Wp, int N, int D, hipStream_t s);
@@ -236,6 +242,8 @@
 hipError_t launch_pack_ffn_split(const float* W1, const float* W2, void* w1s, void* w2s, int D, int F, hipStream_t s);
 hipError_t launch_ffn_ln_split(const float* X, const LayerWeights& w, float* Y, int M, int D, int F, hipStream_t s,
                                unsigned long long* stamp = nullptr);
+constexpr float ATTN_SCORE_T = 64.0f;
+float attn_q_scale(int hd);
 size_t attn_pack_floats(int D, int H, int hpw, int q_only);
 bool attn_kvq_supported(int hd);
 hipError_t launch_pack_attn(const float* in_w, const float* in_b, float* pack, int D, int H, int hpw, int q_only,
@@ -252,6 +260,7 @@
   float* out;
   int B, L, n_own;
   unsigned long long* stamp;
+  bool static_bound = false;
 };
 hipError_t launch_qkv_attention(const AttnArgs& a, int D, int hd, int hpw, int q_only, int kspl, int qg, hipStream_t s);
 
@@ -293,6 +302,7 @@
   int q_only;
   int kspl;
   int qg;
+  bool attn_static;
   FfnForm ffn;
   int mb;
   bool rem;
diff --git a/fastfourierdiffusion_amd/csrc/ffd_qkvattn.hip b/fastfourierdiffusion_amd/csrc/ffd_qkvattn.hip
--- a/fastfourierdiffusion_amd/csrc/ffd_qkvattn.hip
+++ b/fastfourierdiffusion_amd/csrc/ffd_qkvattn.hip
@@ -91,12 +91,14 @@
   return (size_t)(H / hpw) * nct * ((D + 15) / 16) * 256 + (size_t)(H / hpw) * nct * 16;
 }
 
+float attn_q_scale(int hd) { return 1.4426950408889634f / sqrtf((float)hd); }
+
 hipError_t launch_pack_attn(const float* in_w, const float* in_b, float* pack, int D, int H, int hpw, int q_only,
                             hipStream_t s) {
   const int hd = D / H;
   const int nct = attn_nct(hd, hpw, q_only);
   float* abp = pack + (size_t)(H / hpw) * nct * ((D + 15) / 16) * 256;
-  const float qscale = 1.4426950408889634f / sqrtf((float)hd);
+  const float qscale = attn_q_scale(hd);
   hipLaunchKernelGGL(k_pack_attn, dim3(64), dim3(256), 0, s, in_w, in_b, pack, abp, D, H, hd, hpw, nct, q_only, qscale);
   return hipGetLastError();
 }
@@ -141,7 +143,7 @@
   static constexpr int SX = HD / 2;
   static constexpr int HX = HD & 1;
   static constexpr int HP = (HD + 1) / 2;
-  static constexpr float T = 64.0f;
+  static constexpr float T = ATTN_SCORE_T;
   static constexpr size_t floats(int LS) { return (size_t)LS * (8 + 4 * KST); }
 };
 
@@ -224,7 +226,25 @@
 typedef const float4 lds_f32x4;
 #endif
 
-template <int HD, int QG, bool STAMP, bool STORE, int LSC>
+struct StorePlan {
+  unsigned a, s1, s2, s3, step;
+  __device__ __forceinline__ void init(const float* lds0, int image_float, bool vrow, int tok, int tile_tokens) {
+    unsigned s = vrow ? 32u : 4u;
+    asm("" : "+v"(s));
+    a = lds_addr(lds0) + 4u * (unsigned)image_float + (unsigned)tok * s;
+    s1 = s, s2 = s + s, s3 = s2 + s, step = (unsigned)tile_tokens * s;
+    asm("" : "+v"(a), "+v"(s1), "+v"(s2), "+v"(s3), "+v"(step));
+  }
+  __device__ __forceinline__ void store(float x, float y, float z, float w) const {
+#if defined(__HIP_DEVICE_COMPILE__)
+    typedef __attribute__((address_space(3))) float lds_w32;
+    *(lds_w32*)(a) = x, *(lds_w32*)(a + s1) = y, *(lds_w32*)(a + s2) = z, *(lds_w32*)(a + s3) = w;
+#endif
+  }
+  __device__ __forceinline__ void next_tile() { a += step; }
+};
+
+template <int HD, int QG, bool STAMP, bool STORE, int LSC, bool BOUNDED = false>
 __device__ __forceinline__ QRows<HD, QG> attend_qtiles(lds_f32* vs, lds_f32* kts, lds_f32* qts, int LSR,
                                                        int q_first, int q_step, int q_end, int t_lo, int t_hi,
                                                        bool head_bounded, int L, float* orow0, int ostride,
@@ -318,7 +338,7 @@
       }
 #pragma unroll
       for (int g = 0; g < QG; ++g) {
-        if (ref_on || !head_bounded) {
+        if (!BOUNDED && (ref_on || !head_bounded)) {
         float bm = __builtin_fmaxf(__builtin_fmaxf(sc[g][0], sc[g][1]), sc[g][2]);
 #pragma unroll
         for (int r = 3; r < 15; r += 2) bm = __builtin_fmaxf(__builtin_fmaxf(bm, sc[g][r]), sc[g][r + 1]);
@@ -413,7 +433,7 @@
   return rows;
 }
 
-template <int D, int HD, int QG, int NCT, bool SPLIT = false, bool STAMP = false, bool KVQ = false>
+template <int D, int HD, int QG, int NCT, bool SPLIT = false, bool STAMP = false, bool KVQ = false, bool SB = false>
 __global__ __launch_bounds__(256, (SPLIT && NCT >= 2 ? 2 : QG <= 2 ? 4 : 3)) void k_qkv_attention(
     const float* __restrict__ x, const float* __restrict__ awp, const float* __restrict__ kt,
     const float* __restrict__ vt, float* __restrict__ kt_out, float* __restrict__ vt_out, float* __restrict__ out,
@@ -443,7 +463,9 @@
   float* qts = kts + (size_t)2 * KST * LS;
   constexpr int PS = 2 + 2 * HeadDims<HD>::HP;
   unsigned* nrm = reinterpret_cast<unsigned*>(lds + HeadDims<HD>::floats(LS) + (SPLIT ? 4 * 32 * PS : 0));
-  if (threadIdx.x < 2) nrm[threadIdx.x] = 0u;
+  if constexpr (!SB) {
+    if (threadIdx.x < 2) nrm[threadIdx.x] = 0u;
+  }
 
   if constexpr (HD % 2 == 1) {
     for (int idx = threadIdx.x; idx < LS * (8 + 4 * KST); idx += blockDim.x) vs[idx] = 0.f;
@@ -605,31 +627,36 @@
     }
   }
   if constexpr (STAMP) st.t[3] = FFD_STAMP_T();
-  if (kt != nullptr) fill_from_tables<HD>(vs, kts, LS, kt, vt, h, L, Lp, n_own, q_only, threadIdx.x, blockDim.x);
+  if constexpr (!SB) {
+    if (kt != nullptr) fill_from_tables<HD>(vs, kts, LS, kt, vt, h, L, Lp, n_own, q_only, threadIdx.x, blockDim.x);
+  }
   __syncthreads();
-  {
-    int jq0 = 0, jq1 = Lp;
-    if constexpr (SPLIT) {
-      if (q_only || KVQ) {
-        const int qpw = nwaves / kspl;
-        jq0 = min(32 * qs * qpw, Lp), jq1 = min(jq0 + 32 * qpw, Lp);
-      }
-    }
-    head_norms<HD>(kts, qts, nrm, Lp, LS, threadIdx.x, blockDim.x, jq0, jq1);
-  }
-  if (kt_out != nullptr && b == 0 && qs == 0)
-    publish_kv<HD>(vs, kts, LS, kt_out, vt_out, h, L, n_own, threadIdx.x, blockDim.x);
-
-  __syncthreads();
+  bool bounded = true;
+  if constexpr (!SB) {
+    {
+      int jq0 = 0, jq1 = Lp;
+      if constexpr (SPLIT) {
+        if (q_only || KVQ) {
+          const int qpw = nwaves / kspl;
+          jq0 = min(32 * qs * qpw, Lp), jq1 = min(jq0 + 32 * qpw, Lp);
+        }
+      }
+      head_norms<HD>(kts, qts, nrm, Lp, LS, threadIdx.x, blockDim.x, jq0, jq1);
+    }
+    if (kt_out != nullptr && b == 0 && qs == 0)
+      publish_kv<HD>(vs, kts, LS, kt_out, vt_out, h, L, n_own, threadIdx.x, blockDim.x);
+
+    __syncthreads();
+    bounded = head_bounded<HD>(nrm);
+  }
   if constexpr (STAMP) st.t[4] = FFD_STAMP_T();
-  const bool bounded = head_bounded<HD>(nrm);
   float* orow0 = out + (size_t)b * L * D + h * HD;
   if constexpr (SPLIT) {
     const int qpw = nwaves / kspl, kps = (KT + kspl - 1) / kspl;
     const int qt = qs * qpw + wave / kspl, t_lo = (wave % kspl) * kps;
     int t_hi = min(KT, t_lo + kps);
     if (qt >= KT) t_hi = t_lo;
-    const QRows<HD, 1> r = attend_qtiles<HD, 1, STAMP, false, 0>((lds_f32*)vs, (lds_f32*)kts, (lds_f32*)qts, LS, qt, 1,
+    const QRows<HD, 1> r = attend_qtiles<HD, 1, STAMP, false, 0, SB>((lds_f32*)vs, (lds_f32*)kts, (lds_f32*)qts, LS, qt, 1,
                                                                  qt + 1, t_lo, t_hi, bounded, L, orow0, D, st);
     const int half = lane >> 5, l31 = lane & 31;
     float* part = lds + HeadDims<HD>::floats(LS);
@@ -665,13 +692,13 @@
       orow0[(size_t)q * D + e] = ot / lt;
     }
   } else {
-    attend_qtiles<HD, QG, STAMP, true, LSC>((lds_f32*)vs, (lds_f32*)kts, (lds_f32*)qts, LS, wave * QG, nwaves * QG, KT,
+    attend_qtiles<HD, QG, STAMP, true, LSC, SB>((lds_f32*)vs, (lds_f32*)kts, (lds_f32*)qts, LS, wave * QG, nwaves * QG, KT,
                                             0, KT, bounded, L, orow0, D, st);
   }
   if constexpr (STAMP) st.write(stamp, nwaves);
 }
 
-template <int D, int HD, int HPW, int QG, int NCT, bool QO, bool STAMP = false>
+template <int D, int HD, int HPW, int QG, int NCT, bool QO, bool STAMP = false, bool SB = false>
 __global__ __launch_bounds__(128 * HPW, 3) void k_qkv_attention_mh(
     const float* __restrict__ x, const float* __restrict__ awp, const float* __restrict__ kt,
     const float* __restrict__ vt, float* __restrict__ kt_out, float* __restrict__ vt_out, float* __restrict__ out,
@@ -698,8 +725,10 @@
   constexpr int RS = HeadDims<HD>::floats(LS);
   float4* wl = reinterpret_cast<float4*>(lds + (size_t)HPW * RS);
   constexpr int fph = QO ? HD : 3 * HD;
-  if (threadIdx.x < 2 * HPW)
-    reinterpret_cast<unsigned*>(lds + (size_t)HPW * RS + (size_t)NCT * S4 * 256)[threadIdx.x] = 0u;
+  if constexpr (!SB) {
+    if (threadIdx.x < 2 * HPW)
+      reinterpret_cast<unsigned*>(lds + (size_t)HPW * RS + (size_t)NCT * S4 * 256)[threadIdx.x] = 0u;
+  }
 
   {
     const int n = lane & 15, qq = lane >> 4;
@@ -728,16 +757,16 @@
     const float* abp = awp + (size_t)NG * NCT * S4 * 256 + (size_t)hg * NCT * 16;
     float bias[NCTM];
     int sbase[NCTM];
-    bool sv[NCTM];
+    StorePlan sp[NCTM];
 #pragma unroll
     for (int ct = 0; ct < NCTM; ++ct) {
       bias[ct] = abp[ct * 16 + n];
       const int fi = 16 * ct + n;
       const int hh = fi / fph, f = fi - hh * fph;
       const int reg = f / HD, e = f - reg * HD;
-      sv[ct] = reg == 2;
       sbase[ct] = hh >= HPW ? -1
                   : hh * RS + (reg == 0 ? LS * 8 + 2 * KST * LS + e * LS : reg == 1 ? LS * 8 + e * LS : e);
+      sp[ct].init(lds, sbase[ct], reg == 2, 16 * wave + 4 * qq, 16 * NW);
     }
     __syncthreads();
     if constexpr (STAMP) st.t[2] = FFD_STAMP_T();
@@ -812,19 +841,11 @@
           }
         }
       }
-      const int t0 = 16 * tt + 4 * qq;
 #pragma unroll
       for (int ct = 0; ct < NCTM; ++ct) {
-        const float4 o = float4{acc[ct][0] + bias[ct], acc[ct][1] + bias[ct], acc[ct][2] + bias[ct],
-                                acc[ct][3] + bias[ct]};
-        if (sbase[ct] >= 0) {
-          if (!sv[ct]) {
-            *reinterpret_cast<float4*>(lds + sbase[ct] + t0) = o;
-          } else {
-            float* vp = lds + sbase[ct] + t0 * 8;
-            vp[0] = o.x, vp[8] = o.y, vp[16] = o.z, vp[24] = o.w;
-          }
-        }
+        if (sbase[ct] >= 0)
+          sp[ct].store(acc[ct][0] + bias[ct], acc[ct][1] + bias[ct], acc[ct][2] + bias[ct], acc[ct][3] + bias[ct]);
+        sp[ct].next_tile();
       }
     }
   }
@@ -834,16 +855,22 @@
   float* vs = lds + (size_t)hh * RS;
   float* kts = vs + LS * 8;
   float* qts = kts + 2 * KST * LS;
-  if (kt != nullptr) fill_from_tables<HD>(vs, kts, LS, kt, vt, h, L, Lp, n_own, q_only, gw * 64 + lane, 128);
+  if constexpr (!SB) {
+    if (kt != nullptr) fill_from_tables<HD>(vs, kts, LS, kt, vt, h, L, Lp, n_own, q_only, gw * 64 + lane, 128);
+  }
   __syncthreads();
-  unsigned* nrm = reinterpret_cast<unsigned*>(lds + (size_t)HPW * RS + (size_t)NCT * S4 * 256) + 2 * hh;
-  head_norms<HD>(kts, qts, nrm, Lp, LS, gw * 64 + lane, 128);
-  if (kt_out != nullptr && b == 0) publish_kv<HD>(vs, kts, LS, kt_out, vt_out, h, L, n_own, gw * 64 + lane, 128);
-
-  __syncthreads();
+  bool bounded = true;
+  if constexpr (!SB) {
+    unsigned* nrm = reinterpret_cast<unsigned*>(lds + (size_t)HPW * RS + (size_t)NCT * S4 * 256) + 2 * hh;
+    head_norms<HD>(kts, qts, nrm, Lp, LS, gw * 64 + lane, 128);
+    if (kt_out != nullptr && b == 0) publish_kv<HD>(vs, kts, LS, kt_out, vt_out, h, L, n_own, gw * 64 + lane, 128);
+
+    __syncthreads();
+    bounded = head_bounded<HD>(nrm);
+  }
   if constexpr (STAMP) st.t[4] = FFD_STAMP_T();
-  attend_qtiles<HD, QG, STAMP, true, LS>((lds_f32*)vs, (lds_f32*)kts, (lds_f32*)qts, LS, gw * QG, 2 * QG, KT, 0, KT,
-                                         head_bounded<HD>(nrm), L, out + (size_t)b * L * D + h * HD, D, st);
+  attend_qtiles<HD, QG, STAMP, true, LS, SB>((lds_f32*)vs, (lds_f32*)kts, (lds_f32*)qts, LS, gw * QG, 2 * QG, KT, 0, KT,
+                                             bounded, L, out + (size_t)b * L * D + h * HD, D, st);
   if constexpr (STAMP) st.write(stamp, NW);
 }
 
@@ -853,19 +880,26 @@
   const int KT = (a.L + 31) / 32;
   const size_t lds = (HPW * HeadDims<HD>::floats(64 * QG + 4) + (size_t)NCT * S4 * 256 + (size_t)HPW * 2) * sizeof(float);
   if (cdiv(2 * KT, 2 * HPW) > 3 || cdiv(KT, 2) > QG) return hipErrorInvalidValue;
+  if (a.static_bound && (QO || a.kt != nullptr)) return hipErrorInvalidValue;
+  auto go = [&](auto kern, unsigned long long* stamp) {
+    hipLaunchKernelGGL(kern, dim3(a.B * (D / HD / HPW)), dim3(128 * HPW), lds, s, a.x, a.pack, a.kt, a.vt, a.kt_out, a.vt_out,
+                       a.out, a.B, a.L, a.n_own, q_only, stamp);
+    return hipGetLastError();
+  };
   if constexpr (D == 72 && HD == 6) {
     if (a.stamp != nullptr) {
-      hipLaunchKernelGGL((k_qkv_attention_mh<D, HD, HPW, QG, NCT, QO, true>), dim3(a.B * (D / HD / HPW)), dim3(128 * HPW), lds,
-                         s, a.x, a.pack, a.kt, a.vt, a.kt_out, a.vt_out, a.out, a.B, a.L, a.n_own, q_only, a.stamp);
-      return hipGetLastError();
+      if constexpr (!QO) {
+        if (a.static_bound) return go(k_qkv_attention_mh<D, HD, HPW, QG, NCT, QO, true, true>, a.stamp);
+      }
+      return go(k_qkv_attention_mh<D, HD, HPW, QG, NCT, QO, true>, a.stamp);
     }
   }
   if (a.stamp != nullptr) return hipErrorInvalidValue;
   if (q_only != (QO ? 1 : 0)) return hipErrorInvalidValue;
-  auto kern = k_qkv_attention_mh<D, HD, HPW, QG, NCT, QO>;
-  hipLaunchKernelGGL(kern, dim3(a.B * (D / HD / HPW)), dim3(128 * HPW), lds, s, a.x, a.pack, a.kt, a.vt, a.kt_out, a.vt_out,
-                     a.out, a.B, a.L, a.n_own, q_only, (unsigned long long*)nullptr);
-  return hipGetLastError();
+  if constexpr (!QO) {
+    if (a.static_bound) return go(k_qkv_attention_mh<D, HD, HPW, QG, NCT, QO, false, true>, nullptr);
+  }
+  return go(k_qkv_attention_mh<D, HD, HPW, QG, NCT, QO>, nullptr);
 }
 
 template <int D, int HD>
@@ -878,37 +912,49 @@
   return hipErrorInvalidValue;
 }
 
-template <int D, int HD, int QG, int NCT>
+template <int D, int HD, int QG, int NCT, bool FULL>
 static hipError_t launch_t(const AttnArgs& a, int q_only, hipStream_t s) {
   const int KT = (a.L + 31) / 32;
   const size_t lds = (HeadDims<HD>::floats(KT * 32 + 4) + (size_t)2 * KT) * sizeof(float);
   int nwaves = cdiv(KT, QG);
   if (nwaves > 4) nwaves = 4;
   if (cdiv(2 * KT, nwaves) > 8) return hipErrorInvalidValue;
+  if (a.static_bound && (!FULL || q_only || a.kt != nullptr)) return hipErrorInvalidValue;
+  auto go = [&](auto kern, unsigned long long* stamp) {
+    hipLaunchKernelGGL(kern, dim3(a.B * (D / HD)), dim3(64 * nwaves), lds, s, a.x, a.pack, a.kt, a.vt, a.kt_out, a.vt_out,
+                       a.out, a.B, a.L, a.n_own, q_only, 1, 1, stamp);
+    return hipGetLastError();
+  };
   if constexpr (D == 72 && HD == 6 && NCT == 2) {
     if (a.stamp != nullptr) {
-      hipLaunchKernelGGL((k_qkv_attention<D, HD, QG, NCT, false, true>), dim3(a.B * (D / HD)), dim3(64 * nwaves), lds, s, a.x,
-                         a.pack, a.kt, a.vt, a.kt_out, a.vt_out, a.out, a.B, a.L, a.n_own, q_only, 1, 1, a.stamp);
-      return hipGetLastError();
+      if (a.static_bound) return go(k_qkv_attention<D, HD, QG, NCT, false, true, false, true>, a.stamp);
+      return go(k_qkv_attention<D, HD, QG, NCT, false, true>, a.stamp);
     }
   }
   if (a.stamp != nullptr) return hipErrorInvalidValue;
-  hipLaunchKernelGGL((k_qkv_attention<D, HD, QG, NCT>), dim3(a.B * (D / HD)), dim3(64 * nwaves), lds, s, a.x, a.pack, a.kt,
-                     a.vt, a.kt_out, a.vt_out, a.out, a.B, a.L, a.n_own, q_only, 1, 1, (unsigned long long*)nullptr);
-  return hipGetLastError();
-}
-
-template <int D, int HD, int NCT, bool KVQ = false>
+  if constexpr (FULL) {
+    if (a.static_bound) return go(k_qkv_attention<D, HD, QG, NCT, false, false, false, true>, nullptr);
+  }
+  return go(k_qkv_attention<D, HD, QG, NCT>, nullptr);
+}
+
+template <int D, int HD, int NCT, bool KVQ = false, bool FULL = false>
 static hipError_t launch_split_t(const AttnArgs& a, int q_only, int kspl, hipStream_t s) {
   const int KT = (a.L + 31) / 32;
   if (cdiv(2 * KT, 4) > 8 || (kspl != 1 && kspl != 2 && kspl != 4)) return hipErrorInvalidValue;
   const int qsplit = cdiv(KT, 4 / kspl);
   const size_t lds =
       (HeadDims<HD>::floats(KT * 32 + 4) + (size_t)4 * 32 * (2 + 2 * HeadDims<HD>::HP) + (size_t)2 * KT) * sizeof(float);
-  hipLaunchKernelGGL((k_qkv_attention<D, HD, 1, NCT, true, false, KVQ>), dim3(a.B * (D / HD) * qsplit), dim3(256), lds, s, a.x,
-                     a.pack, a.kt, a.vt, a.kt_out, a.vt_out, a.out, a.B, a.L, a.n_own, q_only, qsplit, kspl,
-                     (unsigned long long*)nullptr);
-  return hipGetLastError();
+  if (a.static_bound && (!FULL || q_only || a.kt != nullptr)) return hipErrorInvalidValue;
+  auto go = [&](auto kern) {
+    hipLaunchKernelGGL(kern, dim3(a.B * (D / HD) * qsplit), dim3(256), lds, s, a.x, a.pack, a.kt, a.vt, a.kt_out, a.vt_out,
+                       a.out, a.B, a.L, a.n_own, q_only, qsplit, kspl, (unsigned long long*)nullptr);
+    return hipGetLastError();
+  };
+  if constexpr (FULL) {
+    if (a.static_bound) return go(k_qkv_attention<D, HD, 1, NCT, true, false, KVQ, true>);
+  }
+  return go(k_qkv_attention<D, HD, 1, NCT, true, false, KVQ>);
 }
 
 int qkv_attention_small_split(int B, int H, int L) {
@@ -933,14 +979,14 @@
   if (kspl) {
     if (a.stamp != nullptr) return hipErrorInvalidValue;
     if constexpr (2 * HD <= 16 && 3 * HD > 16) {
-      if (q_only == 2) return launch_split_t<D, HD, 2, true>(a, 0, kspl, s);
+      if (q_only == 2) return launch_split_t<D, HD, 2, true, true>(a, 0, kspl, s);
     }
     if (q_only == 2) return hipErrorInvalidValue;
-    return q_only ? launch_split_t<D, HD, 1>(a, 1, kspl, s) : launch_split_t<D, HD, NCTF>(a, 0, kspl, s);
+    return q_only ? launch_split_t<D, HD, 1>(a, 1, kspl, s) : launch_split_t<D, HD, NCTF, false, true>(a, 0, kspl, s);
   }
   if (q_only == 2) return hipErrorInvalidValue;
   if (q_only && a.stamp != nullptr) return hipErrorInvalidValue;
-#define FFD_QG(g, nct) if (qg == g) return launch_t<D, HD, g, nct>(a, q_only, s);
+#define FFD_QG(g, nct) if (qg == g) return launch_t<D, HD, g, nct, false>(a, q_only, s);
   if (q_only) {
     FFD_QG(1, 1) FFD_QG(3, 1)
     if constexpr (HD <= 6) {
@@ -949,6 +995,8 @@
     FFD_QG(2, 1)
     return hipErrorInvalidValue;
   }
+#undef FFD_QG
+#define FFD_QG(g, nct) if (qg == g) return launch_t<D, HD, g, nct, true>(a, q_only, s);
   FFD_QG(2, NCTF) FFD_QG(1, NCTF) FFD_QG(3, NCTF)
   if constexpr (HD <= 6) {
     FFD_QG(4, NCTF)
diff --git a/include/ffd.h b/include/ffd.h
--- a/include/ffd.h
+++ b/include/ffd.h
@@ -64,6 +64,8 @@
 int ffd_host_noise_scaling(int max_len, int fourier_noise_scaling, float* G_out);
 int ffd_host_timesteps(int n, double eps, float* ts_out, float* step_size_out);
 int ffd_host_gate(int step, int max_len, int K, int R);
+int ffd_host_attn_score_bound(const float* in_proj_weight, const float* in_proj_bias, const float* ln_weight,
+                              const float* ln_bias, int d_model, int head_dim, double q_scale, double* bound_out);
 
 
 int ffd_score_forward(ffd_ctx* ctx, const float* x, float t, float* score_out, int B, void* stream);
```
